# ayankele/dune-transformercvn

Measured on AMD Instinct MI355X. Metric: events/sec (fwd+bwd) at batch=32, 8 prongs/event; fraction of MFMA roofline, higher is better.
Workload: dtype bf16; 1 GPU; TransformerCVN DenseNet [3,6,12,6,3] g32, fwd+loss+bwd, batch 32/GPU, 8 prongs/event, 3x400x280 maps, 6-layer encoder, dropout 0.1; global_batch=32, parallelism=dp1, precision=bf16

## Files before the change

### dune-transformercvn_amd/csrc/densenet.hip

```cpp
#include <string>
#include <vector>
#include <cstring>

#include "tcvn_rows.h"
#include <cstdlib>
#include "densenet_plan.h"

using namespace tcvn;

namespace {
constexpr float kEps = 1e-5f, kMom = 0.1f;
}

int DenseNetPlan::add_slot(const std::string& name, long numel, int kind) {
    slots.push_back({name, numel, kind});
    return (int)slots.size() - 1;
}
BnSlots DenseNetPlan::add_bn(const std::string& p, int c) {
    BnSlots s;
    s.w = add_slot(p + ".weight", c, TCVN_SLOT_PARAM);
    s.b = add_slot(p + ".bias", c, TCVN_SLOT_PARAM);
    s.rm = add_slot(p + ".running_mean", c, TCVN_SLOT_BUFFER);
    s.rv = add_slot(p + ".running_var", c, TCVN_SLOT_BUFFER);
    s.nbt = add_slot(p + ".num_batches_tracked", 1, TCVN_SLOT_COUNTER);
// ... 441 lines not shown
    if (stem_path.act_skip &&
        (rc = stem_mark(coords, nnz, n, cfg.H, cfg.W, Hc, Wc, reinterpret_cast<uint32_t*>(s.ws + L.sact), data[s_b0], s.ws + L.zeros + 512, s.st))) return rc;
    a.part = s.train ? s.part : nullptr; a.nblk = conv_fwd_nblk(a);
    if ((rc = conv_fwd(a, s.st))) return rc;
    if ((rc = link(s, n0, a.nblk, cfg.init_ch, 0, cfg.init_ch, bstat0, M0))) return rc;
    const Tab t = tab(s.ws, L, n0);
    Pool0Args p{mode, s.ws + L.c0, n, Hc, Wc, cfg.init_ch, t.sc, t.sh, data[s_a0], s.ws + L.D[0], b0.ld, b0.H, b0.W,
                s.train ? s.part : nullptr, pool0_grid(n, b0.H, b0.W)};
    if ((rc = pool0_fwd(p, s.st))) return rc;
    fr.nblk = p.nblk;
    return 0;
}

LayerPath DenseNetPlan::layer_path(const Step& s, int bi, int l, const ConvFwdArgs& c3, Fwd1x1Args& f1) const {
    const Layout& L = s.L;
    const BlockGeom& bg = blocks[bi];
    const LayerSlots& ls = bg.layers[l];
    const long M = (long)s.n * bg.H * bg.W;
    const bool bf16 = cfg.mode == MODE_BF16, fast1 = L.XA[bi][l] >= 0;
    const Conv3x3Fwd k3 = bf16 ? conv3x3_fwd_kernel(c3) : CONV3X3_FWD_NONE;
    LayerPath p;
    p.fuse_ya = !s.train && fast1 && k3 != CONV3X3_FWD_NONE;
    p.act_fused = bf16 && !p.fuse_ya && conv3x3_act_fusable(c3);
    static const bool no_fuse1 = TCVN_KNOB_SET("TCVN_NO_FWD1_FUSE") || TCVN_KNOB_SET("TCVN_NO_BWD1_FUSE");
    if ((s.train || p.fuse_ya) && fast1 && !no_fuse1 && cfg.bn_size * cfg.growth == 128 && bf16) {
        const WkEntry& e = wk_find(ls.w1, 0, 1);
        const Tab t1 = tab(s.ws, L, ls.n1);
        f1 = Fwd1x1Args{};
        f1.Xin = s.ws + L.D[bi]; f1.ldx = bg.ld; f1.cin = ls.cin; f1.sc = t1.sc; f1.sh = t1.sh; f1.sl = data[ls.a1]; f1.M = M;
        f1.Wfrag = s.ws + L.wk + e.off; f1.Kp = e.Kp; f1.bias = data[ls.b1]; f1.Out = s.ws + L.Y[bi][l]; f1.zeros = s.ws + L.zeros;
        f1.part = s.train ? s.part : nullptr; f1.nblk = fwd1x1_fused_nblk(f1);
        if (!s.train) {
            f1.osc = c3.sc; f1.osh = c3.sh; f1.osl = c3.sl; f1.Out = s.ws + L.YA[bi][l];
        }
        Bwd1x1Args b1;
        p.raw1x1 = fwd1x1_fused_ok(f1) && (!s.train || bwd1x1_fill(bi, l, M, s.ws, L, b1));
    }
    const bool pair = k3 == CONV3X3_FWD_PAIR;
    p.lf2 = p.raw1x1 && s.lf_on && p.act_fused && pair;
    p.out_isum = s.lf_on && pair && cfg.growth <= 32;
    p.keep_stored = s.train && !L.KM[bi].empty() && pair;
    return p;
}

int DenseNetPlan::fwd_layer(const Step& s, int bi, int l, FreshStats& fr) {
    const Layout& L = s.L;
    const BlockGeom& bg = blocks[bi];
    const LayerSlots& ls = bg.layers[l];
    const long M = (long)s.n * bg.H * bg.W;
    const int mid = cfg.bn_size * cfg.growth, g = cfg.growth;
    char* D = s.ws + L.D[bi];
    char* Y = s.ws + L.Y[bi][l];
    double* bstatD = reinterpret_cast<double*>(s.ws + L.bstatD[bi]);
    double* bstatY = reinterpret_cast<double*>(s.ws + L.bstatY[bi][l]);
    long long* isumD = s.lf_on ? reinterpret_cast<long long*>(s.ws + L.isumD[bi]) : nullptr;
    long long* isumY = s.lf_on ? reinterpret_cast<long long*>(s.ws + L.isumY[bi][l]) : nullptr;
    int rc;
    ConvFwdArgs a = conv3_args(s, bi, l);
    Fwd1x1Args f1;
    const LayerPath p = path[bi][l] = layer_path(s, bi, l, a, f1);
    if (p.raw1x1) {
        if (s.lf_on && fr.isum) f1.lf = lf_link(s, ls.n1, isumD + 2 * fr.c0, 2L * bg.ld, fr.c0, fr.n, bstatD, M);
        else if ((rc = link_fresh(s, ls.n1, bi, fr))) return rc;
        f1.isum_out = isumY; f1.isum_stride = 2L * mid;
        if ((rc = fwd1x1_fused(f1, s.st))) return rc;
        if (!p.lf2 && (rc = link(s, ls.n2, f1.nblk, mid, 0, mid, bstatY, M, isumY, 2L * mid))) return rc;
    } else {
        if ((rc = link_fresh(s, ls.n1, bi, fr))) return rc;
        int nblk;
        if (L.XA[bi][l] >= 0) {
            const int cin8 = (int)round_up(ls.cin, 8);
            const Tab t1 = tab(s.ws, L, ls.n1);
            ActArgs act{D, bg.ld, M, ls.cin, t1.sc, t1.sh, data[ls.a1], s.ws + L.XA[bi][l], cin8};
            if ((rc = act_bf16(act, s.st))) return rc;
            const WkEntry& e = wk_find(ls.w1, 0, 1);
            GemmNtArgs ga{};
            ga.epi = EPI_FWD; ga.A = s.ws + L.XA[bi][l]; ga.lda = cin8; ga.K = cin8; ga.M = M; ga.N = mid;
            ga.Wfrag = s.ws + L.wk + e.off; ga.Kp = e.Kp; ga.zeros = s.ws + L.zeros; ga.bias = data[ls.b1];
            ga.Out = Y; ga.ldo = mid; ga.n_off = 0; ga.part = s.train ? s.part : nullptr; ga.nblk = gemm_nt_nblk(ga);
            if (p.fuse_ya) {
                ga.osc = a.sc; ga.osh = a.sh; ga.osl = a.sl; ga.Out = s.ws + L.YA[bi][l];
            }
            if ((rc = gemm_nt_bf16(ga, "k_gemm_nt_bf16<fwd1x1>", s.st))) return rc;
            nblk = ga.nblk;
        } else {
            ConvFwdArgs c1 = conv1_args(s, bi, l);
            c1.part = s.train ? s.part : nullptr; c1.nblk = conv_fwd_nblk(c1);
            if ((rc = conv_fwd(c1, s.st))) return rc;
            nblk = c1.nblk;
        }
        if ((rc = link(s, ls.n2, nblk, mid, 0, mid, bstatY, M))) return rc;
    }
    if (p.act_fused) a.act_fused = 1;
    else if (cfg.mode == MODE_BF16) {
        if (!p.fuse_ya) {
            ActArgs act{Y, mid, M, mid, a.sc, a.sh, a.sl, s.ws + L.YA[bi][l], mid};
            if ((rc = act_bf16(act, s.st))) return rc;
        }
        a.Aact = s.ws + L.YA[bi][l];
    }
    a.part = s.train ? s.part : nullptr;
    a.drop_p = s.train ? cfg.dropout : 0.f; a.seed = s.seed; a.stream_id = (uint32_t)(bi * 64 + l + 1);
    a.nblk = conv_fwd_nblk(a);
    if (p.lf2) {
        if (!a.act_fused) { fprintf(stderr, "tcvn: link-free norm2 without the in-LDS activation\n"); return -17; }
        a.lf = lf_link(s, ls.n2, isumY, 2L * mid, 0, mid, bstatY, M);
    }
    if (p.out_isum) { a.isum_out = isumD + 2 * ls.cin; a.isum_stride = 2L * bg.ld; }
    if (s.train && !L.KM[bi].empty()) a.keep_out = reinterpret_cast<uint32_t*>(s.ws + L.KM[bi][l]);
    if ((rc = conv_fwd(a, s.st))) return rc;
    fr = FreshStats{ls.cin, g, a.nblk, g, p.out_isum};
    return 0;
}

int DenseNetPlan::fwd_transition(const Step& s, int bi, FreshStats& fr) {
    const Layout& L = s.L;
    const BlockGeom& bg = blocks[bi];
    char* D = s.ws + L.D[bi];
    int rc;
    if ((rc = link_fresh(s, bg.has_trans ? bg.tn : nf, bi, fr))) return rc;
    if (!bg.has_trans) {
        const Tab t = tab(s.ws, L, nf);
        HeadPoolArgs a{cfg.mode, D, bg.ld, s.n, bg.H * bg.W, Cf, t.sc, t.sh, data[s_af], reinterpret_cast<float*>(s.ws + L.F)};
        return head_pool_fwd(a, s.st);
    }
    const BlockGeom& nb = blocks[bi + 1];
    fr = FreshStats{0, nb.C0, 0, bg.Ctot / 2, false};
    if (L.XP[bi] >= 0) {
        const Tab t = tab(s.ws, L, bg.tn);
        ActPoolArgs ap{D, bg.ld, s.n, bg.H, bg.W, bg.Ctot, t.sc, t.sh, data[bg.ta], s.ws + L.XP[bi], bg.ldp};
        if ((rc = cfg.mode == MODE_BF16 ? act_pool_bf16(ap, s.st) : act_pool_f32(ap, s.st))) return rc;
    }
    if (L.XP[bi] >= 0 && cfg.mode == MODE_BF16) {
        const WkEntry& ef = wk_find(bg.tw, 0, 1);
        GemmNtArgs ga{};
        ga.epi = EPI_FWD; ga.A = s.ws + L.XP[bi]; ga.lda = bg.ldp; ga.K = bg.ldp; ga.M = (long)s.n * nb.H * nb.W; ga.N = bg.Ctot / 2;
        ga.Wfrag = s.ws + L.wk + ef.off; ga.Kp = ef.Kp; ga.zeros = s.ws + L.zeros; ga.bias = data[bg.tb];
        ga.Out = s.ws + L.D[bi + 1]; ga.ldo = nb.ld; ga.n_off = 0; ga.part = s.train ? s.part : nullptr; ga.nblk = gemm_nt_nblk(ga);
        if ((rc = gemm_nt_bf16(ga, "k_gemm_nt_bf16<fwdtrans>", s.st))) return rc;
        fr.nblk = ga.nblk;
        return 0;
    }
    ConvFwdArgs a = trans_args(s, bi);
    a.part = s.train ? s.part : nullptr; a.nblk = conv_fwd_nblk(a);
    if ((rc = conv_fwd(a, s.st))) return rc;
    fr.nblk = a.nblk;
    return 0;
}

int DenseNetPlan::fwd_output(const Step& s, float* out, long out_ld) const {
    float* F = reinterpret_cast<float*>(s.ws + s.L.F);
    float* Z = reinterpret_cast<float*>(s.ws + s.L.Z);
    int rc;
    if ((rc = linear_fwd(F, Cf, data[s_wl], nullptr, Z, cfg.out_dim, s.n, cfg.out_dim, Cf, s.st))) return rc;
    float* hs = reinterpret_cast<float*>(s.ws + s.L.head_stat);
    RowsBnArgs r{};
    r.X = Z; r.ldx = cfg.out_dim; r.R = s.n; r.C = cfg.out_dim; r.gamma = data[nl.w]; r.beta = data[nl.b]; r.slope = data[s_al];
    r.running_mean = data[nl.rm]; r.running_var = data[nl.rv]; r.Y = out; r.ldy = out_ld;
    r.save_mean = hs; r.save_rstd = hs + cfg.out_dim; r.train = s.train; r.eps = kEps; r.momentum = kMom;
    r.drop_p = s.train ? cfg.dropout : 0.f; r.seed = s.seed; r.stream_id = 0x4000u;
    return rows_bn_fwd(r, s.st);
}

int DenseNetPlan::tap(int n, const char* name, long* off, int* tn, int* th, int* tw, int* tc, int* tld, int* tes) const {
    Layout L;
    layout(n, false, L);
    std::string s(name);
    *tn = n; *tes = esz;
    if ((s == "img" || s == "conv0") && stem_path.sparse && n == last_n) return -1;
    if (s == "img") { *off = L.img; *th = cfg.H; *tw = cfg.W; *tc = cfg.in_ch; *tld = cfg.in_ch; return 0; }
    if (s == "conv0") { *off = L.c0; *th = Hc; *tw = Wc; *tc = cfg.init_ch; *tld = cfg.init_ch; return 0; }
    if (s == "condense") { *off = L.F; *th = 1; *tw = 1; *tc = Cf; *tld = Cf; *tes = 4; return 0; }
    if (s == "raw:wk") { *tn = *th = *tw = 1; *off = L.wk; *tc = *tld = (int)(wk_bytes() / esz); return 0; }
    if (s == "raw:tabs") { *tn = *th = *tw = 1; *off = L.tabs; *tc = *tld = (int)tab_floats(); *tes = 4; return 0; }
    if (s.rfind("raw:ystat", 0) == 0) {
        int b = 0, l = 0;
        if (sscanf(s.c_str(), "raw:ystat%d.%d", &b, &l) != 2) return -1;
        b -= 1;
        if (b < 0 || b >= (int)blocks.size() || l < 0 || l >= blocks[b].L) return -1;
        *tn = *th = *tw = 1; *off = L.bstatY[b][l]; *tc = *tld = 2 * cfg.bn_size * cfg.growth; *tes = 8; return 0;
    }
    if (s.rfind("raw:bstat", 0) == 0) {
        const int b = atoi(s.c_str() + 9) - 1;
        if (b < 0 || b >= (int)blocks.size()) return -1;
        *tn = *th = *tw = 1; *off = L.bstatD[b]; *tc = *tld = blocks[b].ld * 2; *tes = 8; return 0;
    }
    if (s.rfind("dense", 0) == 0) {
        const int b = atoi(s.c_str() + 5) - 1;
        if (b < 0 || b >= (int)blocks.size()) return -1;
        *off = L.D[b]; *th = blocks[b].H; *tw = blocks[b].W; *tc = blocks[b].Ctot; *tld = blocks[b].ld;
        return 0;
    }
    if (s.rfind("bottleneck", 0) == 0) {
        int b = 0, l = 0;
        if (sscanf(s.c_str(), "bottleneck%d.%d", &b, &l) != 2) return -1;
        b -= 1;
        if (b < 0 || b >= (int)blocks.size() || l < 0 || l >= blocks[b].L) return -1;
        for (const auto& pb : path)
            for (const LayerPath& p : pb) if (n == last_n && p.fuse_ya) return -1;
        *off = L.Y[b][l]; *th = blocks[b].H; *tw = blocks[b].W; *tc = cfg.bn_size * cfg.growth; *tld = *tc;
        return 0;
    }
    if (s.rfind("xa", 0) == 0 || s.rfind("ya", 0) == 0) {
        int b = 0, l = 0;
        if (sscanf(s.c_str() + 2, "%d.%d", &b, &l) != 2) return -1;
        b -= 1;
        if (b < 0 || b >= (int)blocks.size() || l < 0 || l >= blocks[b].L) return -1;
        const bool xa = s[0] == 'x';
        if ((xa && (L.XA[b].empty() || L.XA[b][l] < 0)) || (!xa && L.YA[b].empty())) return -1;
        if (n == last_n && (xa ? path[b][l].raw1x1 : path[b][l].act_fused)) return -1;
        *off = xa ? L.XA[b][l] : L.YA[b][l]; *th = blocks[b].H; *tw = blocks[b].W;
        *tc = xa ? blocks[b].layers[l].cin : cfg.bn_size * cfg.growth; *tld = xa ? (int)round_up(*tc, 8) : *tc;
        return 0;
    }
    return -1;
}

struct tcvn_densenet { DenseNetPlan plan; explicit tcvn_densenet(const tcvn_densenet_cfg& c) : plan(c) {} };

extern "C" {

int tcvn_version(void) { return 1; }
void tcvn_backward_overlap(int on) { tcvn::set_backward_overlap(on); }

int tcvn_densenet_create(const tcvn_densenet_cfg* cfg, tcvn_densenet** out) {
    if (!cfg || !out || cfg->n_blocks < 1 || cfg->n_blocks > 8) return -1;
    if (cfg->mode != TCVN_MODE_F32 && cfg->mode != TCVN_MODE_BF16) return -1;
    *out = new tcvn_densenet(*cfg);
    return 0;
}
void tcvn_densenet_destroy(tcvn_densenet* p) { delete p; }
int tcvn_densenet_num_slots(const tcvn_densenet* p) { return (int)p->plan.slots.size(); }
int tcvn_densenet_slot(const tcvn_densenet* p, int i, char* name, int cap, int64_t* numel, int* kind) {
    if (i < 0 || i >= (int)p->plan.slots.size()) return -1;
    const auto& s = p->plan.slots[i];
    if (name && cap > 0) { strncpy(name, s.name.c_str(), cap - 1); name[cap - 1] = 0; }
    if (numel) *numel = s.numel;
    if (kind) *kind = s.kind;
    return 0;
}
int tcvn_densenet_bind(tcvn_densenet* p, void* const* data, void* const* grad) { return p->plan.bind(data, grad); }
int64_t tcvn_densenet_workspace_bytes(const tcvn_densenet* p, int n_img, int with_backward) {
    Layout L;
    p->plan.layout(n_img, with_backward != 0, L);
    return L.total;
}
int tcvn_densenet_forward(tcvn_densenet* p, int n_img, const int32_t* coords, const float* values, int64_t nnz, int log_pixels,
                          float noise_std, float* out, int64_t out_ld, void* ws, int64_t ws_bytes, int train, uint64_t seed,
                          void* stream) {
    return p->plan.forward(n_img, coords, values, nnz, log_pixels, noise_std, out, out_ld, reinterpret_cast<char*>(ws), ws_bytes,
                           train, seed, reinterpret_cast<hipStream_t>(stream));
}
int tcvn_densenet_backward(tcvn_densenet* p, int n_img, const float* d_out, int64_t d_out_ld, void* ws, int64_t ws_bytes,
                           void* stream) {
    return p->plan.backward(n_img, d_out, d_out_ld, reinterpret_cast<char*>(ws), ws_bytes, reinterpret_cast<hipStream_t>(stream));
}
int tcvn_densenet_num_blocks(const tcvn_densenet* p) { return (int)p->plan.blocks.size(); }
int tcvn_densenet_backward_blocks(tcvn_densenet* p, int n_img, const float* d_out, int64_t d_out_ld, void* ws, int64_t ws_bytes,
                                  int block_hi, int block_lo, void* stream) {
    return p->plan.backward(n_img, d_out, d_out_ld, reinterpret_cast<char*>(ws), ws_bytes, reinterpret_cast<hipStream_t>(stream), block_hi,
                            block_lo);
}
int tcvn_densenet_tap(const tcvn_densenet* p, int n_img, const char* name, int64_t* byte_off, int* n, int* h, int* w, int* c,
                      int* ld, int* elem_bytes) {
    long off = 0;
    int rc = p->plan.tap(n_img, name, &off, n, h, w, c, ld, elem_bytes);
    *byte_off = off;
    return rc;
}

}
```

### dune-transformercvn_amd/csrc/densenet_bwd.hip

```cpp
#include <cstring>
#include <vector>

#include <cstdlib>
#include "densenet_plan.h"
#include "tcvn_rows.h"

using namespace tcvn;

static int g_backward_overlap = 0;
bool tcvn::backward_overlap_enabled() { return g_backward_overlap != 0; }
void tcvn::set_backward_overlap(int on) { g_backward_overlap = on; }

namespace {
constexpr float kEps = 1e-5f;
constexpr long kSlabBytes = 48L << 20;
constexpr long kSlab1GemmBytes = 64L << 20;
constexpr long kSlab1Bytes = 68L << 20;
constexpr long kSlabGemmBytes = 44L << 20;
struct Bump {
    long off;
    long take(long bytes) { long o = off; off += round_up(bytes, 256); return o; }
};
}

// ... 3 lines not shown
    L.G.clear(); L.pqD.clear();
    long bpart = (long)std::max(pool0_bwd_grid(n, Hc, Wc), pool0_bwd_vec_grid(n, Hc, Wc)) * cfg.init_ch * 24;
    bpart = std::max(bpart, 1024L * cfg.init_ch * 24);
    bpart = std::max(bpart, (long)head_pool_bwd_grid(n) * Cf * 24);
    for (const auto& bg : blocks) {
        const long M = (long)n * bg.H * bg.W;
        L.G.push_back(b.take(M * bg.ld * esz));
        bpart = std::max(bpart, 512L * std::max(mid, bg.Ctot) * 24);
    }
    for (const auto& bg : blocks) L.pqD.push_back(b.take((long)bg.ld * 8));
    long gw = 0;
    for (const auto& e : wk_list())
        if (!e.transpose && !e.frag) gw += round_up((long)e.N * e.Kp * 4, 256);
    L.gwk = b.take(gw);
    L.zero_end = b.off;
    L.du = b.take(maxY * esz);
    L.ey = b.take(maxY * esz);
    L.ey2 = b.take(maxY * esz);
    L.slab = b.take(kSlabBytes);
    L.slab1 = cfg.mode == MODE_BF16 ? b.take(kSlab1Bytes) : -1;
    L.pqY = b.take((long)mid * 8);
    L.du0 = b.take((long)n * Hc * Wc * cfg.init_ch * esz);
    L.pq0 = b.take((long)cfg.init_ch * 8);
    L.bpart = b.take(bpart);
    L.dF = b.take((long)n * Cf * 4);
    L.dZ = b.take((long)n * cfg.out_dim * 4);
    L.EY3.clear();
    for (const auto& bg : blocks) {
        std::vector<long> eys;
        if (cfg.mode == MODE_BF16 && cfg.growth == 32)
            for (int l = 0; l < bg.L; ++l) eys.push_back(b.take((long)n * bg.H * bg.W * 32 * esz));
        L.EY3.push_back(eys);
    }
    L.total = b.off;
}

bool DenseNetPlan::bwd1x1_fill(int bi, int l, long M, char* ws, const Layout& L, Bwd1x1Args& fa) const {
    static const bool no_fuse1 = TCVN_KNOB_SET("TCVN_NO_BWD1_FUSE");
    const BlockGeom& bg = blocks[bi];
    const LayerSlots& ls = bg.layers[l];
    const int mid = cfg.bn_size * cfg.growth;
    if (no_fuse1 || L.XA[bi][l] < 0 || mid != 128 || L.slab1 < 0 || cfg.mode != MODE_BF16) return false;
    const Tab t1 = tab(ws, L, ls.n1);
    const WkEntry& etf = wk_find(ls.w1, 1, 1);
    fa = Bwd1x1Args{};
    fa.DU = ws + L.du; fa.Y = ws + L.Y[bi][l]; fa.PY = reinterpret_cast<float*>(ws + L.pqY); fa.QY = fa.PY + mid; fa.M = M;
    fa.Xin = ws + L.D[bi]; fa.ldx = bg.ld; fa.cin = ls.cin;
    fa.sc = t1.sc; fa.sh = t1.sh; fa.sl = data[ls.a1]; fa.Gout = ws + L.G[bi]; fa.ldg = bg.ld;
    fa.Wfrag = ws + L.wk + etf.off; fa.Kp = etf.Kp; fa.zeros = ws + L.zeros; fa.part = reinterpret_cast<double*>(ws + L.bpart);
    fa.slab = reinterpret_cast<float*>(ws + L.slab1); fa.slab_bytes = kSlab1GemmBytes; fa.ldc = wk_find(ls.w1, 0).Kp;
    fa.tail = reinterpret_cast<float*>(ws + L.slab1 + kSlab1GemmBytes);
    fa.nblk = bwd1x1_fused_nblk(fa);
    return bwd1x1_fused_ok(fa);
}

float* DenseNetPlan::gw_of(const Step& s, int slot) const {
    long o = 0;
    for (const WkEntry& e : wk_cache) {
        if (e.transpose || e.frag) continue;
        if (e.slot == slot) return reinterpret_cast<float*>(s.ws + s.L.gwk + o);
        o += round_up((long)e.N * e.Kp * 4, 256);
    }
    return nullptr;
}

int DenseNetPlan::bwd_link(const Step& s, const BnSlots& bn, int nblk, const double* bstat, long count, float* P, float* Q, int acc, int a_slot) const {
    BnBwdLinkArgs a{s.part, nblk, bn.C, bstat, count, kEps, data[bn.w], grad[bn.w], grad[bn.b], grad[a_slot], P, Q, acc};
    return bn_bwd_link(a, s.st);
}

int DenseNetPlan::drain(Step& s) const {
    if (s.side_on && s.side_busy) {
        TCVN_CHECK(hipEventRecord(ev_drain, side_st));
        TCVN_CHECK(hipStreamWaitEvent(s.st, ev_drain, 0));
        s.side_busy = false;
    }
    s.seq = 0;
    return 0;
}

int DenseNetPlan::backward(int n, const float* d_out, long d_out_ld, char* ws, long ws_bytes, hipStream_t st, int bi_hi, int bi_lo) {
    if (!bound) return -11;
    if (bi_hi < 0) bi_hi = (int)blocks.size() - 1;
    if (bi_lo < 0 || bi_lo > bi_hi || bi_hi >= (int)blocks.size()) return -1;
    const bool first_part = bi_hi == (int)blocks.size() - 1, last_part = bi_lo == 0;
    if (n <= 0) return 0;
    if (n != last_n) { fprintf(stderr, "tcvn: densenet backward without matching forward\n"); return -13; }
    for (size_t i = 0; i < slots.size(); ++i)
        if (slots[i].kind == TCVN_SLOT_PARAM && grad[i] == nullptr) { fprintf(stderr, "tcvn: grad of %s unbound\n", slots[i].name.c_str()); return -14; }
    Layout L;
    layout(n, true, L);
    if (ws_bytes < L.total) return -12;
    int rc;
    const bool side_on = fast3x3 && backward_overlap_enabled();
    if (side_on && (rc = ensure_side())) return rc;
    Step s{ws, L, st, n, true, last_seed, reinterpret_cast<double*>(ws + L.bpart), false, side_on, 0, false};

    if (undesc_ws != ws || undesc_total != L.total) {
        std::vector<UnpackDesc> ud;
        unpack_first.assign(blocks.size() + 1, 0);
        long o = 0;
        for (const WkEntry& e : wk_cache) {
            if (e.transpose || e.frag) continue;
            for (size_t bi = 0; bi < blocks.size(); ++bi) {
                if (!blocks[bi].layers.empty() && e.slot == blocks[bi].layers[0].w1) unpack_first[bi] = (int)ud.size();
            }
            UnpackDesc d{reinterpret_cast<const float*>(ws + L.gwk + o), grad[e.slot], e.N, e.Cin, e.taps, e.Kp,
                         (fast3x3 && e.taps == 9) ? 1 : 0};
            ud.push_back(d);
            o += round_up((long)e.N * e.Kp * 4, 256);
        }
        n_unpack = (int)ud.size();
        unpack_first[blocks.size()] = n_unpack;
        if (!d_undesc) TCVN_CHECK(hipMalloc(&d_undesc, ud.size() * sizeof(UnpackDesc)));
        h_undesc.assign(reinterpret_cast<char*>(ud.data()), reinterpret_cast<char*>(ud.data()) + ud.size() * sizeof(UnpackDesc));
        TCVN_CHECK(hipMemcpyAsync(d_undesc, h_undesc.data(), h_undesc.size(), hipMemcpyHostToDevice, st));
        undesc_ws = ws; undesc_total = L.total;
    }

    if (first_part) {
        TCVN_CHECK(hipMemsetAsync(ws + L.pqD[0], 0, (size_t)(L.zero_end - L.pqD[0]), st));
        for (size_t bi = 0; bi + 1 < blocks.size(); ++bi) {
            const long bytes = (long)n * blocks[bi].H * blocks[bi].W * blocks[bi].ld * esz;
            if (L.XP[bi] >= 0 && cfg.mode == MODE_BF16) {
                if ((rc = zero_pool_remainder(ws + L.G[bi], blocks[bi].ld, n, blocks[bi].H, blocks[bi].W, blocks[bi + 1].H, blocks[bi + 1].W, st))) return rc;
            } else TCVN_CHECK(hipMemsetAsync(ws + L.G[bi], 0, (size_t)bytes, st));
        }
        if ((rc = bwd_output(s, d_out, d_out_ld))) return rc;
    }
    for (int bi = bi_hi; bi >= bi_lo; --bi) {
        if ((rc = bwd_transition(s, bi))) return rc;
        for (int l = blocks[bi].L - 1; l >= 0; --l)
            if ((rc = bwd_layer(s, bi, l))) return rc;
    }
    if ((rc = drain(s))) return rc;
    if (last_part && (rc = bwd_stem(s))) return rc;
    const int u0 = last_part ? 0 : unpack_first[bi_lo], u1 = unpack_first[bi_hi + 1];
    return unpack_wgrads(reinterpret_cast<const UnpackDesc*>(d_undesc) + u0, u1 - u0, st);
}

int DenseNetPlan::bwd_output(const Step& s, const float* d_out, long d_out_ld) const {
    const Layout& L = s.L;
    float* F = reinterpret_cast<float*>(s.ws + L.F);
    float* Z = reinterpret_cast<float*>(s.ws + L.Z);
    float* dF = reinterpret_cast<float*>(s.ws + L.dF);
    float* dZ = reinterpret_cast<float*>(s.ws + L.dZ);
    float* hs = reinterpret_cast<float*>(s.ws + L.head_stat);
    int rc;
    RowsBnBwdArgs r{};
    r.X = Z; r.ldx = cfg.out_dim; r.dY = d_out; r.lddy = d_out_ld; r.R = s.n; r.C = cfg.out_dim;
    r.gamma = data[nl.w]; r.beta = data[nl.b]; r.slope = data[s_al]; r.save_mean = hs; r.save_rstd = hs + cfg.out_dim;
    r.dX = dZ; r.lddx = cfg.out_dim; r.dgamma = grad[nl.w]; r.dbeta = grad[nl.b]; r.dslope = grad[s_al];
    r.drop_p = cfg.dropout; r.seed = s.seed; r.stream_id = 0x4000u;
    if ((rc = rows_bn_bwd(r, s.st))) return rc;
    if ((rc = linear_bwd_dw(dZ, cfg.out_dim, F, Cf, grad[s_wl], nullptr, s.n, cfg.out_dim, Cf, s.st))) return rc;
    return linear_bwd_dx(dZ, cfg.out_dim, data[s_wl], dF, Cf, s.n, cfg.out_dim, Cf, 0, s.st);
}

int DenseNetPlan::bwd_transition(Step& s, int bi) const {
    const Layout& L = s.L;
    const BlockGeom& bg = blocks[bi];
    const int mode = cfg.mode;
    const long M = (long)s.n * bg.H * bg.W;
    char* D = s.ws + L.D[bi];
    char* G = s.ws + L.G[bi];
    float* P = reinterpret_cast<float*>(s.ws + L.pqD[bi]);
    float* Q = P + bg.ld;
    const double* bstatD = reinterpret_cast<const double*>(s.ws + L.bstatD[bi]);
    int rc;
    if (!bg.has_trans) {
        const Tab t = tab(s.ws, L, nf);
        HeadPoolBwdArgs a{mode, D, bg.ld, s.n, bg.H * bg.W, Cf, t.sc, t.sh, data[s_af], reinterpret_cast<float*>(s.ws + L.dF), G, bg.ld, s.part,
                          head_pool_bwd_grid(s.n)};
        if ((rc = head_pool_bwd(a, s.st))) return rc;
        return bwd_link(s, nf, a.nblk, bstatD, M, P, Q, 1, s_af);
    }
    const BlockGeom& nb = blocks[bi + 1];
    const long Mn = (long)s.n * nb.H * nb.W;
    const int Nt = bg.Ctot / 2;
    float* Pn = reinterpret_cast<float*>(s.ws + L.pqD[bi + 1]);
    float* Qn = Pn + nb.ld;
    const EffSrc e{s.ws + L.G[bi + 1], nb.ld, s.ws + L.D[bi + 1], nb.ld, 0, Nt, Pn, Qn, 0.f, 0, 0};
    const Tab t = tab(s.ws, L, bg.tn);
    const WkEntry& ef = wk_find(bg.tw, 0);
    if ((rc = drain(s))) return rc;
    if (L.XP[bi] >= 0 && mode == MODE_BF16) {
        const int Nt8 = (int)round_up(Nt, 8);
        SlabJob bias_job{};
        EffMatArgs em{e, Mn, s.ws + L.ey, Nt8, grad[bg.tb], reinterpret_cast<float*>(s.ws + L.slab + kSlabGemmBytes), &bias_job};
        if ((rc = eff_materialize_bf16(em, s.st))) return rc;
        GemmTnArgs gt{s.ws + L.ey, Nt8, Nt8, s.ws + L.XP[bi], bg.ldp, bg.ldp, Mn, gw_of(s, bg.tw), ef.Kp, s.ws + L.zeros,
                      reinterpret_cast<float*>(s.ws + L.slab), kSlabGemmBytes, Nt, bias_job};
        if ((rc = gemm_tn_bf16(gt, "k_gemm_tn_bf16<transition>", s.st))) return rc;
        const WkEntry& etf = wk_find(bg.tw, 1, 1);
        GemmNtArgs ga{};
        ga.epi = EPI_DGRAD_POOL; ga.A = s.ws + L.ey; ga.lda = Nt8; ga.K = Nt8; ga.M = Mn; ga.N = bg.Ctot;
        ga.Wfrag = s.ws + L.wk + etf.off; ga.Kp = etf.Kp; ga.zeros = s.ws + L.zeros;
        ga.Xin = D; ga.ldxin = bg.ld; ga.sc = t.sc; ga.sh = t.sh; ga.sl = data[bg.ta];
        ga.Gout = G; ga.ldgo = bg.ld; ga.g_write = 1; ga.H = nb.H; ga.W = nb.W; ga.Hin = bg.H; ga.Win = bg.W;
        ga.part = s.part; ga.nblk = gemm_nt_nblk(ga);
        if ((rc = gemm_nt_bf16(ga, "k_gemm_nt_bf16<dgradtrans>", s.st))) return rc;
        return bwd_link(s, bg.tn, ga.nblk, bstatD, M, P, Q, 1, bg.ta);
    }
    ConvWgradArgs w{};
    w.mode = mode; w.e = e; w.dWk = gw_of(s, bg.tw); w.dbias = grad[bg.tb];
    w.fa = trans_args(s, bi);
    if (L.XP[bi] >= 0) { w.slab = reinterpret_cast<float*>(s.ws + L.slab); w.slab_bytes = kSlabBytes; }
    if ((rc = conv_wgrad(w, s.st))) return rc;
    const WkEntry& et = wk_find(bg.tw, 1);
    ConvDgradArgs d{};
    d.mode = mode; d.dmode = DG_1X1_POOL; d.e = e; d.M = (int)Mn; d.N = bg.Ctot; d.Kp = et.Kp;
    d.H = nb.H; d.W = nb.W; d.Hin = bg.H; d.Win = bg.W; d.Wt = s.ws + L.wk + et.off;
    d.Xin = D; d.ldxin = bg.ld; d.sc = t.sc; d.sh = t.sh; d.sl = data[bg.ta];
    d.Gout = G; d.ldgo = bg.ld; d.accumulate = 1; d.part = s.part; d.nblk = conv_dgrad_nblk(d);
    if ((rc = conv_dgrad(d, s.st))) return rc;
    return bwd_link(s, bg.tn, d.nblk, bstatD, M, P, Q, 1, bg.ta);
}

int DenseNetPlan::bwd_layer(Step& s, int bi, int l) const {
    const Layout& L = s.L;
    const BlockGeom& bg = blocks[bi];
    const LayerSlots& ls = bg.layers[l];
    const LayerPath& p = path[bi][l];
    const int mode = cfg.mode, g = cfg.growth, mid = cfg.bn_size * cfg.growth;
    const long M = (long)s.n * bg.H * bg.W;
    hipStream_t st = s.st;
    char* D = s.ws + L.D[bi];
    char* G = s.ws + L.G[bi];
    float* P = reinterpret_cast<float*>(s.ws + L.pqD[bi]);
    float* Q = P + bg.ld;
    const double* bstatD = reinterpret_cast<const double*>(s.ws + L.bstatD[bi]);
    char* Y = s.ws + L.Y[bi][l];
    char* DU = s.ws + L.du;
    float* PY = reinterpret_cast<float*>(s.ws + L.pqY);
    float* QY = PY + mid;
    int rc;
    ConvWgradArgs w3{};
    w3.fa = conv3_args(s, bi, l);
    EffSrc e2{G, bg.ld, D, bg.ld, ls.cin, g, P + ls.cin, Q + ls.cin, cfg.dropout, s.seed, (uint32_t)(bi * 64 + l + 1)};
    if (p.keep_stored) e2.keep = reinterpret_cast<const uint32_t*>(s.ws + L.KM[bi][l]);
    bool ey_valid = false;
    {
        const WkEntry& et = wk_find(ls.w2, 1);
        ConvDgradArgs d{};
        d.mode = mode; d.dmode = DG_3X3; d.e = e2; d.M = (int)M; d.N = mid; d.Kp = et.Kp; d.H = bg.H; d.W = bg.W;
        d.Wt = s.ws + L.wk + et.off; d.Xin = Y; d.ldxin = mid; d.sc = w3.fa.sc; d.sh = w3.fa.sh; d.sl = w3.fa.sl;
        d.Gout = DU; d.ldgo = mid; d.accumulate = 0; d.part = s.part;
        d.Wfrag = wk_frag(s.ws, L, ls.w2, 1); d.zeros = s.ws + L.zeros;
        ey_valid = fast3x3 && !L.EY3[bi].empty() && conv3x3_dgrad_kernel(d) == CONV3X3_DGRAD_CONSEC;
        if (ey_valid) d.ey_out = s.ws + L.EY3[bi][l];
        d.nblk = conv_dgrad_nblk(d);
        if ((rc = conv_dgrad(d, st))) return rc;
        if ((rc = bwd_link(s, ls.n2, d.nblk, reinterpret_cast<const double*>(s.ws + L.bstatY[bi][l]), M, PY, QY, 0, ls.a2))) return rc;
    }
    Bwd1x1Args fa{};
    const bool fuse1 = bwd1x1_fill(bi, l, M, s.ws, L, fa);
    SlabJob w3jobs[2] = {};
    bool w3_deferred = false;
    {
        w3.mode = mode; w3.e = e2; w3.dWk = gw_of(s, ls.w2); w3.dbias = grad[ls.b2];
        if (ey_valid) w3.e.ey = s.ws + L.EY3[bi][l];
        if (fast3x3) {
            w3.nfast = 1; w3.fa.act_fused = p.act_fused ? 1 : 0;
            if (!p.act_fused) w3.fa.Aact = s.ws + L.YA[bi][l];
            w3.slab = reinterpret_cast<float*>(s.ws + L.slab); w3.slab_bytes = kSlabBytes;
        }
        const bool par = s.side_on && L.XA[bi][l] >= 0;
        if (par) {
            TCVN_CHECK(hipEventRecord(ev_fork_a, st));
            TCVN_CHECK(hipStreamWaitEvent(side_st, ev_fork_a, 0));
            s.side_busy = true;
        }
        if (!par && fuse1 && fast3x3 && conv3x3_wgrad_tile_ok(w3)) { w3.deferred = w3jobs; w3_deferred = true; }
        if ((rc = conv_wgrad(w3, par ? side_st : st))) return rc;
    }
    if (fuse1) {
        if ((rc = bwd1x1_fused_launch(fa, st))) return rc;
        const BnSlots& s1 = ls.n1;
        BnBwdLinkArgs la{s.part, fa.nblk, s1.C, bstatD, M, kEps, data[s1.w], grad[s1.w], grad[s1.b], grad[ls.a1], P, Q, 1};
        return bwd1x1_fused_reduce(fa, gw_of(s, ls.w1), grad[ls.b1], w3_deferred ? w3jobs : nullptr, st, &la);
    }
    if (p.raw1x1) {
        fprintf(stderr, "tcvn: the forward skipped the activated 1x1 input of block %d layer %d but the fused 1x1 backward cannot run\n", bi, l);
        return -15;
    }
    const Tab t1 = tab(s.ws, L, ls.n1);
    const EffSrc e1{DU, mid, Y, mid, 0, mid, PY, QY, 0.f, 0, 0};
    if (L.XA[bi][l] < 0) {
        ConvWgradArgs w{};
        w.mode = mode; w.e = e1; w.dWk = gw_of(s, ls.w1); w.dbias = grad[ls.b1];
        w.fa = conv1_args(s, bi, l);
        if (mode == MODE_F32) { w.slab = reinterpret_cast<float*>(s.ws + L.slab); w.slab_bytes = kSlabBytes; }
        if ((rc = conv_wgrad(w, st))) return rc;
        const WkEntry& et = wk_find(ls.w1, 1);
        ConvDgradArgs d{};
        d.mode = mode; d.dmode = DG_1X1; d.e = e1; d.M = (int)M; d.N = ls.cin; d.Kp = et.Kp; d.H = bg.H; d.W = bg.W;
        d.Wt = s.ws + L.wk + et.off; d.Xin = D; d.ldxin = bg.ld; d.sc = t1.sc; d.sh = t1.sh; d.sl = data[ls.a1];
        d.Gout = G; d.ldgo = bg.ld; d.accumulate = 1; d.part = s.part; d.nblk = conv_dgrad_nblk(d);
        if ((rc = conv_dgrad(d, st))) return rc;
        return bwd_link(s, ls.n1, d.nblk, bstatD, M, P, Q, 1, ls.a1);
    }
    const bool odd = s.side_on && (s.seq & 1);
    char* EY = s.ws + (odd ? L.ey2 : L.ey);
    float* tail = reinterpret_cast<float*>(s.ws + L.slab + kSlabGemmBytes + (odd ? (kSlabBytes - kSlabGemmBytes) / 2 : 0));
    if (s.side_on && s.seq >= 2) TCVN_CHECK(hipStreamWaitEvent(st, ev_done[s.seq & 1], 0));
    SlabJob bias_job{};
    EffMatArgs em{e1, M, EY, mid, grad[ls.b1], tail, &bias_job};
    if ((rc = eff_materialize_bf16(em, st))) return rc;
// ... 66 lines not shown
```

### dune-transformercvn_amd/csrc/encoder.hip

```cpp
#include "tcvn_encoder.h"

namespace tcvn {

namespace {

constexpr float kInvSqrt2 = 0.70710678118654752440f;

__global__ void k_gather_tokens(const float* C, const int* tok_row, float* X, int B, int S, int D) {
    const int t = blockIdx.x;
    const int s = t / B, b = t - s * B;
    const int r = tok_row[b * S + s];
    for (int d = threadIdx.x; d < D; d += blockDim.x) X[(long)t * D + d] = r >= 0 ? C[(long)r * D + d] : 0.f;
}
__global__ void k_scatter_tokens_bwd(const float* dX, const int* tok_row, float* dC, int B, int S, int D) {
    const int t = blockIdx.x;
    const int s = t / B, b = t - s * B;
    const int r = tok_row[b * S + s];
    if (r < 0) return;
    for (int d = threadIdx.x; d < D; d += blockDim.x) dC[(long)r * D + d] = dX[(long)t * D + d];
}
__global__ void k_mask_rows(const float* X, const int* tok_row, float* Y, int B, int S, int D) {
    const int t = blockIdx.x;
    const int s = t / B, b = t - s * B;
    const bool keep = tok_row[b * S + s] >= 0;
// ... 25 lines not shown
    }
    float sum = 0.f;
    for (int j = 0; j < a.S; ++j) { sc[j] = valid[j] ? expf(sc[j] - mx) : 0.f; sum += sc[j]; }
    const float inv = 1.0f / sum;
    float* P = a.probs + (((long)b * a.H + h) * a.S + s) * a.S;
    float ctx[MAXHD];
    for (int e = 0; e < a.hd; ++e) ctx[e] = 0.f;
    for (int j = 0; j < a.S; ++j) {
        float p = sc[j] * inv;
        P[j] = p;
        if (a.drop_p > 0.f) p *= drop_scale(a.drop_p, a.seed, a.stream_id, (((uint64_t)b * a.H + h) * a.S + s) * a.S + j);
        for (int e = 0; e < a.hd; ++e) ctx[e] = fmaf(p, v[j][e], ctx[e]);
    }
    float* o = a.ctx + ((long)s * a.B + b) * D + h * a.hd;
    for (int e = 0; e < a.hd; ++e) o[e] = ctx[e];
}

__global__ __launch_bounds__(64) void k_attn_bwd(const AttnBwdArgs a) {
    __shared__ float q[MAXS][MAXHD + 1], k[MAXS][MAXHD + 1], v[MAXS][MAXHD + 1], dc[MAXS][MAXHD + 1];
    __shared__ float dS[MAXS][MAXS + 1], Pd[MAXS][MAXS + 1];
    const int b = blockIdx.x, h = blockIdx.y, s = threadIdx.x;
    const int D = a.H * a.hd;
    for (int i = threadIdx.x; i < a.S * a.hd; i += 64) {
        const int ss = i / a.hd, d = i - ss * a.hd;
        const float* row = a.qkv + ((long)ss * a.B + b) * 3 * D + h * a.hd + d;
        q[ss][d] = row[0]; k[ss][d] = row[D]; v[ss][d] = row[2 * D];
        dc[ss][d] = a.dctx[((long)ss * a.B + b) * D + h * a.hd + d];
    }
    __syncthreads();
    const float scale = rsqrtf((float)a.hd);
    if (s < a.S) {
        const float* P = a.probs + (((long)b * a.H + h) * a.S + s) * a.S;
        float dot = 0.f;
        float dp[MAXS];
        for (int j = 0; j < a.S; ++j) {
            float g = 0.f;
            for (int e = 0; e < a.hd; ++e) g = fmaf(dc[s][e], v[j][e], g);
            float m = 1.f;
            if (a.drop_p > 0.f) m = drop_scale(a.drop_p, a.seed, a.stream_id, (((uint64_t)b * a.H + h) * a.S + s) * a.S + j);
            Pd[s][j] = P[j] * m;
            dp[j] = g * m;
            dot = fmaf(dp[j], P[j], dot);
        }
        for (int j = 0; j < a.S; ++j) dS[s][j] = P[j] * (dp[j] - dot);
    }
    __syncthreads();
    if (s >= a.S) return;
    float* o = a.dqkv + ((long)s * a.B + b) * 3 * D + h * a.hd;
    for (int e = 0; e < a.hd; ++e) {
        float dq = 0.f, dk = 0.f, dv = 0.f;
        for (int j = 0; j < a.S; ++j) {
            dq = fmaf(dS[s][j], k[j][e], dq);
            dk = fmaf(dS[j][s], q[j][e], dk);
            dv = fmaf(Pd[j][s], dc[j][e], dv);
        }
        o[e] = dq * scale; o[D + e] = dk * scale; o[2 * D + e] = dv;
    }
}

__global__ __launch_bounds__(256) void k_add_ln_fwd(const AddLnArgs a) {
    const int wave = threadIdx.x >> 6, lane = threadIdx.x & 63;
    const int t = blockIdx.x * 4 + wave;
    if (t >= a.T) return;
    float v[8];
    const int per = (a.D + 63) / 64;
    float s = 0.f;
    for (int i = 0; i < per; ++i) {
        const int d = lane + 64 * i;
        float x = 0.f;
        if (d < a.D) {
            float r = a.R[(long)t * a.D + d];
            if (a.drop_p > 0.f) r *= drop_scale(a.drop_p, a.seed, a.stream_id, (uint64_t)t * a.D + d);
            x = a.X[(long)t * a.D + d] + r;
        }
        v[i] = x; s += x;
    }
    const float mean = wave_sum(s) / a.D;
    float q = 0.f;
    for (int i = 0; i < per; ++i) { const int d = lane + 64 * i; if (d < a.D) { const float c = v[i] - mean; q += c * c; } }
    const float rstd = rsqrtf(wave_sum(q) / a.D + a.eps);
    for (int i = 0; i < per; ++i) {
        const int d = lane + 64 * i;
        if (d < a.D) {
            const float xh = (v[i] - mean) * rstd;
            a.XH[(long)t * a.D + d] = xh;
            a.Y[(long)t * a.D + d] = xh * a.gamma[d] + a.beta[d];
        }
    }
    if (lane == 0) a.rstd[t] = rstd;
}
__global__ __launch_bounds__(256) void k_add_ln_bwd(const AddLnBwdArgs a) {
    const int wave = threadIdx.x >> 6, lane = threadIdx.x & 63;
    const int t = blockIdx.x * 4 + wave;
    if (t >= a.T) return;
    const int per = (a.D + 63) / 64;
    float g[8], xh[8];
    float s1 = 0.f, s2 = 0.f;
    for (int i = 0; i < per; ++i) {
        const int d = lane + 64 * i;
        g[i] = 0.f; xh[i] = 0.f;
        if (d < a.D) {
            xh[i] = a.XH[(long)t * a.D + d];
            g[i] = a.dY[(long)t * a.D + d] * a.gamma[d];
            s1 += g[i]; s2 += g[i] * xh[i];
        }
    }
    s1 = wave_sum(s1) / a.D; s2 = wave_sum(s2) / a.D;
    const float rstd = a.rstd[t];
    for (int i = 0; i < per; ++i) {
        const int d = lane + 64 * i;
        if (d < a.D) {
            const float ds = rstd * (g[i] - s1 - xh[i] * s2);
            a.dX[(long)t * a.D + d] = ds;
            float dr = ds;
            if (a.drop_p > 0.f) dr *= drop_scale(a.drop_p, a.seed, a.stream_id, (uint64_t)t * a.D + d);
            a.dR[(long)t * a.D + d] = dr;
        }
    }
}
__global__ __launch_bounds__(256) void k_ln_param_grads(const float* dY, const float* XH, int T, int D, float* dgamma, float* dbeta) {
    __shared__ double sa[16][17], sb[16][17];
    const int cl = threadIdx.x & 15, rl = threadIdx.x >> 4, d = blockIdx.x * 16 + cl;
    double a = 0, b = 0;
    if (d < D)
        for (int t = rl; t < T; t += 16) { const float g = dY[(long)t * D + d]; a += (double)g * XH[(long)t * D + d]; b += g; }
    sa[rl][cl] = a; sb[rl][cl] = b;
    __syncthreads();
    if (threadIdx.x < 16 && d < D) {
        double x = 0, y = 0;
#pragma unroll
        for (int i = 0; i < 16; ++i) { x += sa[i][cl]; y += sb[i][cl]; }
        dgamma[d] += (float)x; dbeta[d] += (float)y;
    }
}

__global__ void k_act_fwd(const float* X, float* Y, long n, int gelu, float drop_p, uint64_t seed, uint32_t stream_id) {
    const long i = (long)blockIdx.x * blockDim.x + threadIdx.x;
    if (i >= n) return;
    const float x = X[i];
    float y = gelu ? 0.5f * x * (1.f + erff(x * kInvSqrt2)) : fmaxf(x, 0.f);
    if (drop_p > 0.f) y *= drop_scale(drop_p, seed, stream_id, (uint64_t)i);
    Y[i] = y;
}
__global__ void k_act_bwd(const float* X, const float* dY, float* dX, long n, int gelu, float drop_p, uint64_t seed, uint32_t stream_id) {
    const long i = (long)blockIdx.x * blockDim.x + threadIdx.x;
    if (i >= n) return;
    const float x = X[i];
    float g = dY[i];
    if (drop_p > 0.f) g *= drop_scale(drop_p, seed, stream_id, (uint64_t)i);
    const float d = gelu ? 0.5f * (1.f + erff(x * kInvSqrt2)) + x * 0.3989422804014327f * expf(-0.5f * x * x) : (x > 0.f ? 1.f : 0.f);
    dX[i] = g * d;
}

template <typename TT>
__global__ __launch_bounds__(256) void k_focal(const float* logits, const TT* targets, int rows, int C, float gamma, float weight,
                                               float* dlogits, float* out) {
    __shared__ double red[256][2];
    __shared__ int cnt_s[256];
    __shared__ int total;
    int cnt = 0;
    for (int r = threadIdx.x; r < rows; r += 256) cnt += targets[r] >= 0;
    cnt_s[threadIdx.x] = cnt;
    __syncthreads();
    if (threadIdx.x == 0) { int c = 0; for (int i = 0; i < 256; ++i) c += cnt_s[i]; total = c; }
    __syncthreads();
    const float invn = total > 0 ? 1.0f / total : 0.f;
    double loss = 0, acc = 0;
    for (int r = threadIdx.x; r < rows; r += 256) {
        const int t = (int)targets[r];
        float* dl = dlogits + (long)r * C;
        if (t < 0) { for (int c = 0; c < C; ++c) dl[c] = 0.f; continue; }
        const float* z = logits + (long)r * C;
        float mx = z[0]; int am = 0;
        for (int c = 1; c < C; ++c) if (z[c] > mx) { mx = z[c]; am = c; }
        float sum = 0.f;
        for (int c = 0; c < C; ++c) sum += expf(z[c] - mx);
        const float logpt = z[t] - mx - logf(sum);
        const float pt = expf(logpt);
        float dldlogpt;
        if (gamma == 0.f) { loss += -logpt; dldlogpt = -1.f; }
        else {
            const float om = fmaxf(1.f - pt, 0.f);
            const float w = powf(om, gamma);
            loss += -logpt * w;
            dldlogpt = -w + (om > 0.f ? logpt * gamma * powf(om, gamma - 1.f) * pt : 0.f);
        }
        acc += am == t;
        for (int c = 0; c < C; ++c) {
            const float p = expf(z[c] - mx) / sum;
            dl[c] = weight * invn * dldlogpt * ((c == t ? 1.f : 0.f) - p);
        }
    }
    red[threadIdx.x][0] = loss; red[threadIdx.x][1] = acc;
    __syncthreads();
    if (threadIdx.x == 0) {
        double l = 0, c = 0;
        for (int i = 0; i < 256; ++i) { l += red[i][0]; c += red[i][1]; }
        out[0] = (float)(l * invn); out[1] = (float)(c * invn);
    }
}

__global__ void k_permute_rows(const float* in, float* out, int B, int P, int C, int to_bm) {
    const int i = blockIdx.x * blockDim.x + threadIdx.x;
    if (i >= B * P * C) return;
    const int c = i % C, r = i / C;
    if (to_bm) { const int b = r / P, p = r - b * P; out[i] = in[((long)p * B + b) * C + c]; }
    else { const int p = r / B, b = r - p * B; out[i] = in[((long)b * P + p) * C + c]; }
}
__global__ void k_add_drop(const float* x, const float* r, float* y, long n, float drop_p, uint64_t seed, uint32_t stream_id) {
    const long i = (long)blockIdx.x * blockDim.x + threadIdx.x;
    if (i >= n) return;
    float v = r[i];
    if (drop_p > 0.f) v *= drop_scale(drop_p, seed, stream_id, (uint64_t)i);
    y[i] = x[i] + v;
}
__global__ void k_mul_drop(const float* dy, float* dr, long n, float drop_p, uint64_t seed, uint32_t stream_id) {
    const long i = (long)blockIdx.x * blockDim.x + threadIdx.x;
    if (i >= n) return;
    float v = dy[i];
    if (drop_p > 0.f) v *= drop_scale(drop_p, seed, stream_id, (uint64_t)i);
    dr[i] = v;
}
__global__ void k_add_inplace(float* dst, const float* src, long n) {
    const long i = (long)blockIdx.x * blockDim.x + threadIdx.x;
    if (i < n) dst[i] += src[i];
}

}

int permute_rows(const float* in, float* out, int B, int P, int C, int to_bm, hipStream_t st) {
    if (B * P * C <= 0) return 0;
    hipLaunchKernelGGL(k_permute_rows, dim3(cdiv((long)B * P * C, 256)), dim3(256), 0, st, in, out, B, P, C, to_bm);
    TCVN_LAUNCH_CHECK(); return 0;
}
int add_drop(const float* x, const float* r, float* y, long n, float drop_p, uint64_t seed, uint32_t sid, hipStream_t st) {
    hipLaunchKernelGGL(k_add_drop, dim3(cdiv(n, 256)), dim3(256), 0, st, x, r, y, n, drop_p, seed, sid);
    TCVN_LAUNCH_CHECK(); return 0;
}
int mul_drop(const float* dy, float* dr, long n, float drop_p, uint64_t seed, uint32_t sid, hipStream_t st) {
    hipLaunchKernelGGL(k_mul_drop, dim3(cdiv(n, 256)), dim3(256), 0, st, dy, dr, n, drop_p, seed, sid);
    TCVN_LAUNCH_CHECK(); return 0;
}
int add_inplace(float* dst, const float* src, long n, hipStream_t st) {
    hipLaunchKernelGGL(k_add_inplace, dim3(cdiv(n, 256)), dim3(256), 0, st, dst, src, n);
    TCVN_LAUNCH_CHECK(); return 0;
}
int gather_tokens(const float* C, const int* tok_row, float* X, int B, int S, int D, hipStream_t st) {
    hipLaunchKernelGGL(k_gather_tokens, dim3(B * S), dim3(128), 0, st, C, tok_row, X, B, S, D);
    TCVN_LAUNCH_CHECK(); return 0;
}
int scatter_tokens_bwd(const float* dX, const int* tok_row, float* dC, int B, int S, int D, hipStream_t st) {
    hipLaunchKernelGGL(k_scatter_tokens_bwd, dim3(B * S), dim3(128), 0, st, dX, tok_row, dC, B, S, D);
    TCVN_LAUNCH_CHECK(); return 0;
}
int mask_rows(const float* X, const int* tok_row, float* Y, int B, int S, int D, hipStream_t st) {
    hipLaunchKernelGGL(k_mask_rows, dim3(B * S), dim3(128), 0, st, X, tok_row, Y, B, S, D);
    TCVN_LAUNCH_CHECK(); return 0;
}
int attn_fwd(const AttnArgs& a, hipStream_t st) {
    if (a.S > MAXS || a.hd > MAXHD) { fprintf(stderr, "tcvn: attention supports S<=%d, head_dim<=%d\n", MAXS, MAXHD); return -2; }
    hipLaunchKernelGGL(k_attn_fwd, dim3(a.B, a.H), dim3(64), 0, st, a);
    TCVN_LAUNCH_CHECK(); return 0;
}
int attn_bwd(const AttnBwdArgs& a, hipStream_t st) {
    if (a.S > MAXS || a.hd > MAXHD) return -2;
    hipLaunchKernelGGL(k_attn_bwd, dim3(a.B, a.H), dim3(64), 0, st, a);
    TCVN_LAUNCH_CHECK(); return 0;
}
int add_ln_fwd(const AddLnArgs& a, hipStream_t st) {
    if (a.D > 512) return -2;
    hipLaunchKernelGGL(k_add_ln_fwd, dim3(cdiv(a.T, 4)), dim3(256), 0, st, a);
    TCVN_LAUNCH_CHECK(); return 0;
}
int add_ln_bwd(const AddLnBwdArgs& a, hipStream_t st) {
    if (a.D > 512) return -2;
    hipLaunchKernelGGL(k_add_ln_bwd, dim3(cdiv(a.T, 4)), dim3(256), 0, st, a);
    TCVN_LAUNCH_CHECK();
    hipLaunchKernelGGL(k_ln_param_grads, dim3(cdiv(a.D, 16)), dim3(256), 0, st, a.dY, a.XH, a.T, a.D, a.dgamma, a.dbeta);
    TCVN_LAUNCH_CHECK(); return 0;
}
int act_fwd(const float* X, float* Y, long n, int gelu, float drop_p, uint64_t seed, uint32_t sid, hipStream_t st) {
    hipLaunchKernelGGL(k_act_fwd, dim3(cdiv(n, 256)), dim3(256), 0, st, X, Y, n, gelu, drop_p, seed, sid);
    TCVN_LAUNCH_CHECK(); return 0;
}
int act_bwd(const float* X, const float* dY, float* dX, long n, int gelu, float drop_p, uint64_t seed, uint32_t sid, hipStream_t st) {
    hipLaunchKernelGGL(k_act_bwd, dim3(cdiv(n, 256)), dim3(256), 0, st, X, dY, dX, n, gelu, drop_p, seed, sid);
    TCVN_LAUNCH_CHECK(); return 0;
}
int focal_i64(const float* logits, const int64_t* targets, int rows, int C, float gamma, float weight, float* dlogits, float* out,
              hipStream_t st) {
    hipLaunchKernelGGL(k_focal<int64_t>, dim3(1), dim3(256), 0, st, logits, targets, rows, C, gamma, weight, dlogits, out);
    TCVN_LAUNCH_CHECK(); return 0;
}
int focal_i8(const float* logits, const int8_t* targets, int rows, int C, float gamma, float weight, float* dlogits, float* out,
             hipStream_t st) {
    hipLaunchKernelGGL(k_focal<int8_t>, dim3(1), dim3(256), 0, st, logits, targets, rows, C, gamma, weight, dlogits, out);
    TCVN_LAUNCH_CHECK(); return 0;
}

}
```

### dune-transformercvn_amd/csrc/head.hip

```cpp
#include <string>
#include <vector>
#include <cstring>

#include "../../include/tcvn_hip.h"
#include "head_plan.h"
#include "tcvn_rows.h"
#include "tcvn_encoder.h"
#include "tcvn_explain.h"
#include "tcvn_occlude.h"
#include "tcvn_shapley.h"

using namespace tcvn;

namespace {
constexpr float kEps = 1e-5f, kMom = 0.1f;
constexpr uint32_t kSidCombined = 0x5000u;
constexpr uint32_t sid_enc(int l, int k) { return 0x6000u + l * 8 + k; }
constexpr uint32_t sid_dec(int i) { return 0x7000u + (uint32_t)i; }

__global__ void k_combine_loss(const float* oe, const float* op, float ew, float* losses, float* accs) {
    losses[0] = ew * oe[0] + (1.f - ew) * op[0];
    losses[1] = oe[0]; losses[2] = op[0];
    accs[0] = oe[1]; accs[1] = op[1];
}
struct Bump {
    long off = 0;
    long take(long bytes) { long o = off; off += round_up(bytes, 256); return o; }
};
}

int HeadPlan::add_slot(const std::string& name, long numel, int kind) {
    slots.push_back({name, numel, kind});
    return (int)slots.size() - 1;
}
HBn HeadPlan::add_bn(const std::string& p, int c) {
    HBn s;
    s.w = add_slot(p + ".weight", c, TCVN_SLOT_PARAM);
    s.b = add_slot(p + ".bias", c, TCVN_SLOT_PARAM);
    s.rm = add_slot(p + ".running_mean", c, TCVN_SLOT_BUFFER);
    s.rv = add_slot(p + ".running_var", c, TCVN_SLOT_BUFFER);
    add_slot(p + ".num_batches_tracked", 1, TCVN_SLOT_COUNTER);
    return s;
}

HeadPlan::HeadPlan(const tcvn_head_cfg& c) : cfg(c) {
    const int D = cfg.hidden_dim;
    const std::string ce = "prong_embedding.combined_embedding";
    const bool bn = !cfg.no_linear_bn, prelu_act = !cfg.linear_relu;
    comb.in = cfg.in_dim; comb.out = D; comb.sid = kSidCombined; comb.drop = true;
    comb.w = add_slot(ce + ".linear.weight", (long)D * cfg.in_dim, TCVN_SLOT_PARAM);
    if (!bn) comb.b = add_slot(ce + ".linear.bias", D, TCVN_SLOT_PARAM);
    if (bn) comb.n = add_bn(ce + ".norm", D);
    if (prelu_act) comb.a = add_slot(ce + ".activation.weight", D, TCVN_SLOT_PARAM);
    for (int l = 0; l < cfg.n_layers; ++l) {
        const std::string p = "encoder.encoder.layers." + std::to_string(l);
        HLayer L;
        L.win = add_slot(p + ".self_attn.in_proj_weight", 3L * D * D, TCVN_SLOT_PARAM);
        L.bin = add_slot(p + ".self_attn.in_proj_bias", 3 * D, TCVN_SLOT_PARAM);
        L.wo = add_slot(p + ".self_attn.out_proj.weight", (long)D * D, TCVN_SLOT_PARAM);
        L.bo = add_slot(p + ".self_attn.out_proj.bias", D, TCVN_SLOT_PARAM);
        L.w1 = add_slot(p + ".linear1.weight", (long)D * D, TCVN_SLOT_PARAM);
        L.b1 = add_slot(p + ".linear1.bias", D, TCVN_SLOT_PARAM);
        L.w2 = add_slot(p + ".linear2.weight", (long)D * D, TCVN_SLOT_PARAM);
        L.b2 = add_slot(p + ".linear2.bias", D, TCVN_SLOT_PARAM);
        L.g1 = add_slot(p + ".norm1.weight", D, TCVN_SLOT_PARAM);
        L.be1 = add_slot(p + ".norm1.bias", D, TCVN_SLOT_PARAM);
        L.g2 = add_slot(p + ".norm2.weight", D, TCVN_SLOT_PARAM);
        L.be2 = add_slot(p + ".norm2.bias", D, TCVN_SLOT_PARAM);
        layers.push_back(L);
    }
    ew = add_slot("event_decoder.hidden_layer.weight", (long)cfg.event_classes * D, TCVN_SLOT_PARAM);
    eb = add_slot("event_decoder.hidden_layer.bias", cfg.event_classes, TCVN_SLOT_PARAM);
    int idx = 0, in = D;
    for (int i = 0; i < cfg.n_dec; ++i) {
        const std::string p = "prong_decoder.hidden_layers.";
        HDec d;
        d.in = in; d.out = cfg.dec_dims[i]; d.sid = sid_dec(i); d.drop = cfg.dropout_modules != 0;
        d.w = add_slot(p + std::to_string(idx) + ".weight", (long)d.out * d.in, TCVN_SLOT_PARAM);
        d.b = add_slot(p + std::to_string(idx) + ".bias", d.out, TCVN_SLOT_PARAM);
        if (bn) d.n = add_bn(p + std::to_string(idx + 1), d.out);
        if (prelu_act) d.a = add_slot(p + std::to_string(idx + 1 + (bn ? 1 : 0)) + ".weight", d.out, TCVN_SLOT_PARAM);
        idx += 2 + (bn ? 1 : 0) + (cfg.dropout_modules ? 1 : 0);
        in = d.out;
        dec.push_back(d);
    }
    dec_width = in;
    ow = add_slot("prong_decoder.output_layer.weight", (long)cfg.prong_classes * cfg.dec_out_in, TCVN_SLOT_PARAM);
    ob = add_slot("prong_decoder.output_layer.bias", cfg.prong_classes, TCVN_SLOT_PARAM);
    data.assign(slots.size(), nullptr);
    grad.assign(slots.size(), nullptr);
}

int HeadPlan::bind(void* const* d, void* const* g) {
    for (size_t i = 0; i < slots.size(); ++i) {
        data[i] = reinterpret_cast<float*>(d[i]);
        grad[i] = g ? reinterpret_cast<float*>(g[i]) : nullptr;
        if (slots[i].kind != TCVN_SLOT_COUNTER && data[i] == nullptr) return -10;
    }
    bound = true;
    return 0;
}

void HeadPlan::layout(int B, int P, int nP, HLayout& L) const {
    Bump b;
    const int D = cfg.hidden_dim, S = 1 + P, T = S * B, R = B + nP, TP = P * B, H = cfg.heads;
    const long td = (long)T * D * 4;
    L.Zc = b.take((long)R * D * 4); L.C = b.take((long)R * D * 4); L.cstat = b.take(2L * D * 4);
    L.X.clear(); L.lay.clear();
    for (int l = 0; l <= cfg.n_layers; ++l) L.X.push_back(b.take(td));
    for (int l = 0; l < cfg.n_layers; ++l) {
        HLayBuf q;
        q.qkv = b.take(3 * td); q.probs = b.take((long)B * H * S * S * 4); q.ctx = b.take(td); q.ao = b.take(td);
        q.xh1 = b.take(td); q.rstd1 = b.take((long)T * 4); q.x1 = b.take(td); q.hpre = b.take(td); q.hact = b.take(td);
        q.f = b.take(td); q.xh2 = b.take(td); q.rstd2 = b.take((long)T * 4);
        q.h1 = cfg.norm_first ? b.take(td) : -1; q.h2 = cfg.norm_first ? b.take(td) : -1;
        L.lay.push_back(q);
    }
    L.HID = b.take(td);
    L.Zd.clear(); L.Ad.clear(); L.dstat.clear();
    for (const auto& d : dec) {
        L.Zd.push_back(b.take((long)TP * d.out * 4)); L.Ad.push_back(b.take((long)TP * d.out * 4));
        L.dstat.push_back(b.take(2L * d.out * 4));
    }
    L.LG = b.take((long)TP * cfg.prong_classes * 4);
    L.dEv = b.take((long)B * cfg.event_classes * 4); L.dPr = b.take((long)B * P * cfg.prong_classes * 4);
    L.lossbuf = b.take(64);
    L.dLG = b.take((long)TP * cfg.prong_classes * 4);
    L.t0 = b.take(3 * td); L.t1 = b.take(3 * td); L.t2 = b.take(td); L.t3 = b.take(td); L.dHID = b.take(td);
    L.dC = b.take((long)R * D * 4); L.dZc = b.take((long)R * D * 4);
    for (int l = 0; l < cfg.n_layers; ++l) {
        HLayBuf& q = L.lay[l];
        q.g_dqkv = b.take(3 * td); q.g_dao = b.take(td); q.g_dhp = b.take(td); q.g_df = b.take(td);
    }
    L.lnp = b.take((long)B * cfg.n_layers * 4 * D * 4);
    L.total = b.off;
}

int HeadPlan::step(int B, int P, int nP, void* ws, long ws_bytes, int train, uint64_t seed, hipStream_t st, HeadStep& s) const {
    if (!bound) return -11;
    if (cfg.dec_out_in != dec_width) { fprintf(stderr, "tcvn: prong decoder width mismatch (reference would fail too)\n"); return -21; }
    if (B <= 0 || P < 0 || nP < 0 || 1 + P > 64) return -1;
    s.B = B; s.P = P; s.nP = nP; s.S = 1 + P; s.T = s.S * B; s.R = B + nP; s.TP = P * B;
    s.ws = reinterpret_cast<char*>(ws); s.train = train; s.seed = seed; s.dp = train ? cfg.dropout : 0.f; s.st = st;
    layout(B, P, nP, s.L);
    return ws_bytes < s.L.total ? -12 : 0;
}

EncPath HeadPlan::enc_path(int S) const {
    if (fused_encoder && encoder_fused_ok(S, cfg.hidden_dim, cfg.heads, cfg.n_layers, cfg.norm_first)) return EncPath::FUSED;
    return cfg.norm_first ? EncPath::PRE_NORM : EncPath::POST_NORM;
}

EncLayerW HeadPlan::enc_w(int l) const {
    const HLayer& W = layers[l];
    return EncLayerW{data[W.win], data[W.bin], data[W.wo], data[W.bo], data[W.w1], data[W.b1], data[W.w2], data[W.b2],
                     data[W.g1], data[W.be1], data[W.g2], data[W.be2]};
}
EncLayerBuf HeadPlan::enc_buf(const HeadStep& s, int l) const {
    const HLayBuf& q = s.L.lay[l];
    return EncLayerBuf{s.F(q.qkv), s.F(q.probs), s.F(q.ctx), s.F(q.xh1), s.F(q.rstd1), s.F(q.x1), s.F(q.hpre), s.F(q.hact), s.F(q.xh2),
                       s.F(q.rstd2), s.F(s.L.X[l + 1])};
}
RowsBnArgs HeadPlan::block_fwd(const HDec& d, const HeadStep& s, long X, long Y, long stat, int rows) const {
    RowsBnArgs r{};
    r.X = s.F(X); r.ldx = d.out; r.R = rows; r.C = d.out; r.slope = d.a >= 0 ? data[d.a] : nullptr; r.no_norm = cfg.no_linear_bn;
    if (!r.no_norm) { r.gamma = data[d.n.w]; r.beta = data[d.n.b]; r.running_mean = data[d.n.rm]; r.running_var = data[d.n.rv]; }
    r.Y = s.F(Y); r.ldy = d.out;
    r.save_mean = s.F(stat); r.save_rstd = s.F(stat) + d.out; r.train = s.train; r.eps = kEps; r.momentum = kMom;
    r.drop_p = d.drop ? s.dp : 0.f; r.seed = s.seed; r.stream_id = d.sid;
    return r;
}
RowsBnBwdArgs HeadPlan::block_bwd(const HDec& d, const HeadStep& s, long X, long dY, long stat, long dX, int rows) const {
    RowsBnBwdArgs r{};
    r.X = s.F(X); r.ldx = d.out; r.dY = s.F(dY); r.lddy = d.out; r.R = rows; r.C = d.out;
    r.no_norm = cfg.no_linear_bn; r.slope = d.a >= 0 ? data[d.a] : nullptr; r.dslope = d.a >= 0 ? grad[d.a] : nullptr;
    if (!r.no_norm) { r.gamma = data[d.n.w]; r.beta = data[d.n.b]; r.dgamma = grad[d.n.w]; r.dbeta = grad[d.n.b]; }
    r.save_mean = s.F(stat); r.save_rstd = s.F(stat) + d.out;
    r.dX = s.F(dX); r.lddx = d.out;
    r.drop_p = d.drop ? s.dp : 0.f; r.seed = s.seed; r.stream_id = d.sid;
    return r;
}
DecIn HeadPlan::dec_in(const HeadStep& s, int i) const {
    const long hid_prongs = (long)s.B * cfg.hidden_dim;
    if (i == 0) return DecIn{s.F(s.L.HID) + hid_prongs, s.F(s.L.dHID) + hid_prongs, cfg.hidden_dim};
    return DecIn{s.F(s.L.Ad[i - 1]), s.F(s.L.t0), dec[i - 1].out};
}

int HeadPlan::embed(const HeadStep& s, const float* rows, const int32_t* tok_row) const {
    const HLayout& L = s.L;
    const int D = cfg.hidden_dim;
    if (int rc = linear_fwd(rows, cfg.in_dim, data[comb.w], comb.b >= 0 ? data[comb.b] : nullptr, s.F(L.Zc), D, s.R, D, cfg.in_dim, s.st)) return rc;
    if (int rc = rows_bn_fwd(block_fwd(comb, s, L.Zc, L.C, L.cstat, s.R), s.st)) return rc;
    return gather_tokens(s.F(L.C), tok_row, s.F(L.X[0]), s.B, s.S, D, s.st);
}

int HeadPlan::encode(const HeadStep& s, const int32_t* tok_row) const {
    switch (enc_path(s.S)) {
    case EncPath::FUSED: {
        EncFusedArgs a{};
        a.X0 = s.F(s.L.X[0]); a.tok_row = tok_row; a.HID = s.F(s.L.HID); a.B = s.B; a.S = s.S; a.H = cfg.heads; a.L = cfg.n_layers;
        a.gelu = cfg.gelu; a.save = 1; a.eps = kEps; a.drop_p = s.dp; a.seed = s.seed;
        for (int l = 0; l < cfg.n_layers; ++l) { a.w[l] = enc_w(l); a.buf[l] = enc_buf(s, l); }
        return encoder_fused_fwd(a, s.st);
    }
    case EncPath::POST_NORM: return encode_post(s, tok_row);
    case EncPath::PRE_NORM: return encode_pre(s, tok_row);
    }
    return -1;
}
int HeadPlan::encode_post(const HeadStep& s, const int32_t* tok_row) const {
    const HLayout& L = s.L;
    const int D = cfg.hidden_dim, T = s.T, H = cfg.heads, hd = D / H;
    for (int l = 0; l < cfg.n_layers; ++l) {
        const HLayer& W = layers[l];
        const HLayBuf& q = L.lay[l];
        if (int rc = linear_fwd(s.F(L.X[l]), D, data[W.win], data[W.bin], s.F(q.qkv), 3 * D, T, 3 * D, D, s.st)) return rc;
        AttnArgs a{s.F(q.qkv), tok_row, s.F(q.probs), s.F(q.ctx), s.B, s.S, H, hd, s.dp, s.seed, sid_enc(l, 0)};
        if (int rc = attn_fwd(a, s.st)) return rc;
        if (int rc = linear_fwd(s.F(q.ctx), D, data[W.wo], data[W.bo], s.F(q.ao), D, T, D, D, s.st)) return rc;
        AddLnArgs n1{s.F(L.X[l]), s.F(q.ao), data[W.g1], data[W.be1], s.F(q.x1), s.F(q.xh1), s.F(q.rstd1), T, D, kEps, s.dp, s.seed, sid_enc(l, 1)};
        if (int rc = add_ln_fwd(n1, s.st)) return rc;
        if (int rc = linear_fwd(s.F(q.x1), D, data[W.w1], data[W.b1], s.F(q.hpre), D, T, D, D, s.st)) return rc;
        if (int rc = act_fwd(s.F(q.hpre), s.F(q.hact), (long)T * D, cfg.gelu, s.dp, s.seed, sid_enc(l, 2), s.st)) return rc;
        if (int rc = linear_fwd(s.F(q.hact), D, data[W.w2], data[W.b2], s.F(q.f), D, T, D, D, s.st)) return rc;
        AddLnArgs n2{s.F(q.x1), s.F(q.f), data[W.g2], data[W.be2], s.F(L.X[l + 1]), s.F(q.xh2), s.F(q.rstd2), T, D, kEps, s.dp, s.seed, sid_enc(l, 3)};
        if (int rc = add_ln_fwd(n2, s.st)) return rc;
    }
    return mask_rows(s.F(L.X[cfg.n_layers]), tok_row, s.F(L.HID), s.B, s.S, D, s.st);
}
int HeadPlan::encode_pre(const HeadStep& s, const int32_t* tok_row) const {
    const HLayout& L = s.L;
    const int D = cfg.hidden_dim, T = s.T, H = cfg.heads, hd = D / H;
    float* zero = s.F(L.t0);
    TCVN_CHECK(hipMemsetAsync(zero, 0, (size_t)T * D * 4, s.st));
    for (int l = 0; l < cfg.n_layers; ++l) {
        const HLayer& W = layers[l];
        const HLayBuf& q = L.lay[l];
        AddLnArgs n1{s.F(L.X[l]), zero, data[W.g1], data[W.be1], s.F(q.h1), s.F(q.xh1), s.F(q.rstd1), T, D, kEps, 0.f, s.seed, sid_enc(l, 1)};
        if (int rc = add_ln_fwd(n1, s.st)) return rc;
        if (int rc = linear_fwd(s.F(q.h1), D, data[W.win], data[W.bin], s.F(q.qkv), 3 * D, T, 3 * D, D, s.st)) return rc;
        AttnArgs a{s.F(q.qkv), tok_row, s.F(q.probs), s.F(q.ctx), s.B, s.S, H, hd, s.dp, s.seed, sid_enc(l, 0)};
        if (int rc = attn_fwd(a, s.st)) return rc;
        if (int rc = linear_fwd(s.F(q.ctx), D, data[W.wo], data[W.bo], s.F(q.ao), D, T, D, D, s.st)) return rc;
        if (int rc = add_drop(s.F(L.X[l]), s.F(q.ao), s.F(q.x1), (long)T * D, s.dp, s.seed, sid_enc(l, 1), s.st)) return rc;
        AddLnArgs n2{s.F(q.x1), zero, data[W.g2], data[W.be2], s.F(q.h2), s.F(q.xh2), s.F(q.rstd2), T, D, kEps, 0.f, s.seed, sid_enc(l, 3)};
        if (int rc = add_ln_fwd(n2, s.st)) return rc;
        if (int rc = linear_fwd(s.F(q.h2), D, data[W.w1], data[W.b1], s.F(q.hpre), D, T, D, D, s.st)) return rc;
        if (int rc = act_fwd(s.F(q.hpre), s.F(q.hact), (long)T * D, cfg.gelu, s.dp, s.seed, sid_enc(l, 2), s.st)) return rc;
        if (int rc = linear_fwd(s.F(q.hact), D, data[W.w2], data[W.b2], s.F(q.f), D, T, D, D, s.st)) return rc;
        if (int rc = add_drop(s.F(q.x1), s.F(q.f), s.F(L.X[l + 1]), (long)T * D, s.dp, s.seed, sid_enc(l, 3), s.st)) return rc;
    }
    return mask_rows(s.F(L.X[cfg.n_layers]), tok_row, s.F(L.HID), s.B, s.S, D, s.st);
}

int HeadPlan::decode(const HeadStep& s, float* ev_logits, float* pr_logits) const {
    const HLayout& L = s.L;
    const int D = cfg.hidden_dim, TP = s.TP, n_dec = (int)dec.size();
    if (ev_logits)
        if (int rc = linear_fwd(s.F(L.HID), D, data[ew], data[eb], ev_logits, cfg.event_classes, s.B, cfg.event_classes, D, s.st)) return rc;
    if (!pr_logits || TP == 0) return 0;
    for (int i = 0; i < n_dec; ++i) {
        const HDec& d = dec[i];
        const DecIn in = dec_in(s, i);
        if (int rc = linear_fwd(in.x, in.w, data[d.w], data[d.b], s.F(L.Zd[i]), d.out, TP, d.out, d.in, s.st)) return rc;
        if (int rc = rows_bn_fwd(block_fwd(d, s, L.Zd[i], L.Ad[i], L.dstat[i], TP), s.st)) return rc;
    }
    const DecIn in = dec_in(s, n_dec);
    if (int rc = linear_fwd(in.x, in.w, data[ow], data[ob], s.F(L.LG), cfg.prong_classes, TP, cfg.prong_classes, cfg.dec_out_in, s.st)) return rc;
    return permute_rows(s.F(L.LG), pr_logits, s.B, s.P, cfg.prong_classes, 1, s.st);
}

int HeadPlan::forward(int B, int P, int nP, const float* rows, const int32_t* tok_row, float* ev_logits, float* pr_logits,
                      void* ws, long ws_bytes, int train, uint64_t seed, hipStream_t st) {
    HeadStep s;
    if (int rc = step(B, P, nP, ws, ws_bytes, train, seed, st, s)) return rc;
    if (int rc = embed(s, rows, tok_row)) return rc;
    if (int rc = encode(s, tok_row)) return rc;
    if (int rc = decode(s, ev_logits, pr_logits)) return rc;
    last_seed = seed;
    return 0;
}

int HeadPlan::loss(int B, int P, const float* ev_logits, const float* pr_logits, const int64_t* et, const int8_t* pt, float* losses,
                   float* accs, float* dEv, float* dPr, hipStream_t st) {
    float* lb = accs + 2;
    if (int rc = focal_i64(ev_logits, et, B, cfg.event_classes, cfg.gamma, cfg.event_weight, dEv, lb, st)) return rc;
    if (int rc = focal_i8(pr_logits, pt, B * P, cfg.prong_classes, cfg.gamma, 1.f - cfg.event_weight, dPr, lb + 2, st)) return rc;
    hipLaunchKernelGGL(k_combine_loss, dim3(1), dim3(1), 0, st, lb, lb + 2, cfg.event_weight, losses, accs);
    TCVN_LAUNCH_CHECK();
    return 0;
}

int HeadPlan::backward(int B, int P, int nP, const float* rows, const int32_t* tok_row, const float* dEv, const float* dPr,
                       float* d_rows, void* ws, long ws_bytes, hipStream_t st) {
    if (bound)
        for (size_t i = 0; i < slots.size(); ++i)
            if (slots[i].kind == TCVN_SLOT_PARAM && grad[i] == nullptr) return -14;
    HeadStep s;
    if (int rc = step(B, P, nP, ws, ws_bytes, 1, last_seed, st, s)) return rc;
    if (int rc = decoders_bwd(s, dEv, dPr)) return rc;
    float* dX = s.F(s.L.t2);
    if (int rc = mask_rows(s.F(s.L.dHID), tok_row, dX, B, s.S, cfg.hidden_dim, st)) return rc;
    int rc = 0;
    switch (enc_path(s.S)) {
    case EncPath::FUSED: rc = encoder_bwd_fused(s, dX, s.F(s.L.t3)); dX = s.F(s.L.t3); break;
    case EncPath::POST_NORM: rc = encoder_bwd_post(s, dX); break;
    case EncPath::PRE_NORM: rc = encoder_bwd_pre(s, dX); break;
    }
    return rc ? rc : embed_bwd(s, dX, rows, tok_row, d_rows);
}

int HeadPlan::decoders_bwd(const HeadStep& s, const float* dEv, const float* dPr) const {
    const HLayout& L = s.L;
    const int D = cfg.hidden_dim, TP = s.TP, Ce = cfg.event_classes, Cp = cfg.prong_classes, n_dec = (int)dec.size();
    if (int rc = permute_rows(dPr, s.F(L.dLG), s.B, s.P, Cp, 0, s.st)) return rc;
    const DecIn last = dec_in(s, n_dec);
    if (int rc = linear_bwd_dw(s.F(L.dLG), Cp, last.x, last.w, grad[ow], grad[ob], TP, Cp, last.w, s.st)) return rc;
    if (int rc = linear_bwd_dx(s.F(L.dLG), Cp, data[ow], last.dx, last.w, TP, Cp, last.w, 0, s.st)) return rc;
    float* dZ = s.F(L.t1);
    for (int i = n_dec - 1; i >= 0; --i) {
        const HDec& d = dec[i];
        const DecIn in = dec_in(s, i);
        if (int rc = rows_bn_bwd(block_bwd(d, s, L.Zd[i], L.t0, L.dstat[i], L.t1, TP), s.st)) return rc;
        if (int rc = linear_bwd_dw(dZ, d.out, in.x, in.w, grad[d.w], grad[d.b], TP, d.out, d.in, s.st)) return rc;
        if (int rc = linear_bwd_dx(dZ, d.out, data[d.w], in.dx, in.w, TP, d.out, d.in, 0, s.st)) return rc;
    }
    if (int rc = linear_bwd_dw(dEv, Ce, s.F(L.HID), D, grad[ew], grad[eb], s.B, Ce, D, s.st)) return rc;
    return linear_bwd_dx(dEv, Ce, data[ew], s.F(L.dHID), D, s.B, Ce, D, 0, s.st);
}

int HeadPlan::encoder_bwd_fused(const HeadStep& s, const float* dY, float* dX) const {
    const HLayout& L = s.L;
    const int D = cfg.hidden_dim;
    EncFusedBwdArgs a{};
    a.dY = dY; a.dX = dX; a.lnp = s.F(L.lnp); a.B = s.B; a.S = s.S; a.H = cfg.heads; a.L = cfg.n_layers; a.gelu = cfg.gelu;
    a.drop_p = s.dp; a.seed = s.seed;
    EncWgradArgs w{};
    w.T = s.T; w.B = s.B; w.L = cfg.n_layers; w.lnp = s.F(L.lnp);
    int nj = 0, nt = 0;
    for (int l = 0; l < cfg.n_layers; ++l) {
        const HLayer& W = layers[l];
        const HLayBuf& q = L.lay[l];
        a.w[l] = enc_w(l); a.buf[l] = enc_buf(s, l);
        a.g[l] = EncLayerGrad{s.F(q.g_dqkv), s.F(q.g_dao), s.F(q.g_dhp), s.F(q.g_df)};
        w.job[nj++] = EncWgradJob{s.F(q.g_dqkv), 3 * D, s.F(L.X[l]), grad[W.win], grad[W.bin], 3 * D / 32};
        w.job[nj++] = EncWgradJob{s.F(q.g_dao), D, s.F(q.ctx), grad[W.wo], grad[W.bo], D / 32};
        w.job[nj++] = EncWgradJob{s.F(q.g_dhp), D, s.F(q.x1), grad[W.w1], grad[W.b1], D / 32};
        w.job[nj++] = EncWgradJob{s.F(q.g_df), D, s.F(q.hact), grad[W.w2], grad[W.b2], D / 32};
        nt += 3 * D / 32 + 3 * (D / 32);
        w.ln_dst[l][0] = grad[W.g1]; w.ln_dst[l][1] = grad[W.be1]; w.ln_dst[l][2] = grad[W.g2]; w.ln_dst[l][3] = grad[W.be2];
    }
    w.n_jobs = nj; w.n_tiles = nt;
    return encoder_fused_bwd(a, w, s.st);
}

int HeadPlan::encoder_bwd_post(const HeadStep& s, float* dX) const {
    const HLayout& L = s.L;
    const int D = cfg.hidden_dim, T = s.T, H = cfg.heads, hd = D / H;
    float *d1 = s.F(L.t3), *dR = s.F(L.t0), *dT = s.F(L.t1);
    for (int l = cfg.n_layers - 1; l >= 0; --l) {
        const HLayer& W = layers[l];
        const HLayBuf& q = L.lay[l];
        AddLnBwdArgs n2{dX, s.F(q.xh2), s.F(q.rstd2), data[W.g2], d1, dR, grad[W.g2], grad[W.be2], T, D, s.dp, s.seed, sid_enc(l, 3)};
        if (int rc = add_ln_bwd(n2, s.st)) return rc;
        if (int rc = linear_bwd_dw(dR, D, s.F(q.hact), D, grad[W.w2], grad[W.b2], T, D, D, s.st)) return rc;
        if (int rc = linear_bwd_dx(dR, D, data[W.w2], dT, D, T, D, D, 0, s.st)) return rc;
        if (int rc = act_bwd(s.F(q.hpre), dT, dR, (long)T * D, cfg.gelu, s.dp, s.seed, sid_enc(l, 2), s.st)) return rc;
        if (int rc = linear_bwd_dw(dR, D, s.F(q.x1), D, grad[W.w1], grad[W.b1], T, D, D, s.st)) return rc;
        if (int rc = linear_bwd_dx(dR, D, data[W.w1], d1, D, T, D, D, 1, s.st)) return rc;
        AddLnBwdArgs n1{d1, s.F(q.xh1), s.F(q.rstd1), data[W.g1], dX, dR, grad[W.g1], grad[W.be1], T, D, s.dp, s.seed, sid_enc(l, 1)};
        if (int rc = add_ln_bwd(n1, s.st)) return rc;
        if (int rc = linear_bwd_dw(dR, D, s.F(q.ctx), D, grad[W.wo], grad[W.bo], T, D, D, s.st)) return rc;
        if (int rc = linear_bwd_dx(dR, D, data[W.wo], dT, D, T, D, D, 0, s.st)) return rc;
        AttnBwdArgs ab{s.F(q.qkv), s.F(q.probs), dT, dR, s.B, s.S, H, hd, s.dp, s.seed, sid_enc(l, 0)};
        if (int rc = attn_bwd(ab, s.st)) return rc;
        if (int rc = linear_bwd_dw(dR, 3 * D, s.F(L.X[l]), D, grad[W.win], grad[W.bin], T, 3 * D, D, s.st)) return rc;
        if (int rc = linear_bwd_dx(dR, 3 * D, data[W.win], dX, D, T, 3 * D, D, 1, s.st)) return rc;
    }
    return 0;
}

int HeadPlan::encoder_bwd_pre(const HeadStep& s, float* dX) const {
    const HLayout& L = s.L;
    const int D = cfg.hidden_dim, T = s.T, H = cfg.heads, hd = D / H;
    const long n = (long)T * D;
    float *d1 = s.F(L.t3), *dR = s.F(L.t0), *dT = s.F(L.t1);
    float* dS = s.F(L.dHID);
    for (int l = cfg.n_layers - 1; l >= 0; --l) {
        const HLayer& W = layers[l];
        const HLayBuf& q = L.lay[l];
        if (int rc = mul_drop(dX, dR, n, s.dp, s.seed, sid_enc(l, 3), s.st)) return rc;
        if (int rc = linear_bwd_dw(dR, D, s.F(q.hact), D, grad[W.w2], grad[W.b2], T, D, D, s.st)) return rc;
        if (int rc = linear_bwd_dx(dR, D, data[W.w2], dT, D, T, D, D, 0, s.st)) return rc;
        if (int rc = act_bwd(s.F(q.hpre), dT, dR, n, cfg.gelu, s.dp, s.seed, sid_enc(l, 2), s.st)) return rc;
        if (int rc = linear_bwd_dw(dR, D, s.F(q.h2), D, grad[W.w1], grad[W.b1], T, D, D, s.st)) return rc;
        if (int rc = linear_bwd_dx(dR, D, data[W.w1], dT, D, T, D, D, 0, s.st)) return rc;
        AddLnBwdArgs n2{dT, s.F(q.xh2), s.F(q.rstd2), data[W.g2], dS, d1, grad[W.g2], grad[W.be2], T, D, 0.f, s.seed, sid_enc(l, 3)};
        if (int rc = add_ln_bwd(n2, s.st)) return rc;
        if (int rc = add_inplace(dX, dS, n, s.st)) return rc;
        if (int rc = mul_drop(dX, dR, n, s.dp, s.seed, sid_enc(l, 1), s.st)) return rc;
        if (int rc = linear_bwd_dw(dR, D, s.F(q.ctx), D, grad[W.wo], grad[W.bo], T, D, D, s.st)) return rc;
        if (int rc = linear_bwd_dx(dR, D, data[W.wo], dT, D, T, D, D, 0, s.st)) return rc;
        AttnBwdArgs ab{s.F(q.qkv), s.F(q.probs), dT, dR, s.B, s.S, H, hd, s.dp, s.seed, sid_enc(l, 0)};
        if (int rc = attn_bwd(ab, s.st)) return rc;
        if (int rc = linear_bwd_dw(dR, 3 * D, s.F(q.h1), D, grad[W.win], grad[W.bin], T, 3 * D, D, s.st)) return rc;
        if (int rc = linear_bwd_dx(dR, 3 * D, data[W.win], dT, D, T, 3 * D, D, 0, s.st)) return rc;
        AddLnBwdArgs n1{dT, s.F(q.xh1), s.F(q.rstd1), data[W.g1], dS, d1, grad[W.g1], grad[W.be1], T, D, 0.f, s.seed, sid_enc(l, 1)};
        if (int rc = add_ln_bwd(n1, s.st)) return rc;
        if (int rc = add_inplace(dX, dS, n, s.st)) return rc;
    }
    return 0;
}

int HeadPlan::embed_bwd(const HeadStep& s, const float* dX0, const float* rows, const int32_t* tok_row, float* d_rows) const {
    const HLayout& L = s.L;
    const int D = cfg.hidden_dim;
    if (int rc = scatter_tokens_bwd(dX0, tok_row, s.F(L.dC), s.B, s.S, D, s.st)) return rc;
    if (int rc = rows_bn_bwd(block_bwd(comb, s, L.Zc, L.dC, L.cstat, L.dZc, s.R), s.st)) return rc;
    if (int rc = linear_bwd_dw(s.F(L.dZc), D, rows, cfg.in_dim, grad[comb.w], comb.b >= 0 ? grad[comb.b] : nullptr, s.R, D, cfg.in_dim, s.st)) return rc;
    return linear_bwd_dx(s.F(L.dZc), D, data[comb.w], d_rows, cfg.in_dim, s.R, D, cfg.in_dim, 0, s.st);
}

struct tcvn_head {
    HeadPlan plan;
    int last_np = 0, last_b = 0, last_p = -1;
    explicit tcvn_head(const tcvn_head_cfg& c) : plan(c) {}
};

namespace {
struct LooLayout { long jobs, src, lg, vrow, head, total; int cap; };
void loo_layout(const HeadPlan& plan, int B, int P, LooLayout& o) {
    Bump b;
    const long slots = (long)B * (1 + P);
    o.cap = (int)(slots < TCVN_LOO_MAX_PASS ? slots : TCVN_LOO_MAX_PASS);
    o.jobs = b.take(slots * 4); o.src = b.take(slots * 4); o.lg = b.take(slots * plan.cfg.event_classes * 4);
    o.vrow = b.take((long)o.cap * (1 + P) * 4);
    HLayout L;
    plan.layout(o.cap, P, 0, L);
    o.head = b.take(L.total);
    o.total = b.off;
}
struct ShapHost { std::vector<int64_t> offsets, vmask; std::vector<int32_t> n, exact; };
bool shap_shape_ok(int batch, int max_prongs, int max_exact, int samples) {
    return batch > 0 && batch <= 65535 && max_prongs >= 0 && max_prongs <= 63 && max_exact >= 0 && max_exact <= TCVN_SHAP_MAX_EXACT &&
           samples >= 1;
}
long shap_jobs(int n, int max_exact, int M) { return n <= max_exact ? 1L << n : 2 + (long)M * (n - 1); }
int shap_read_table(const int32_t* tok_row, int B, int S, int max_exact, int M, hipStream_t st, ShapHost& h) {
    std::vector<int32_t> tr((size_t)B * S);
    TCVN_CHECK(hipMemcpyAsync(tr.data(), tok_row, tr.size() * 4, hipMemcpyDeviceToHost, st));
    TCVN_CHECK(hipStreamSynchronize(st));
    h.offsets.assign(B + 1, 0); h.vmask.assign(B, 0); h.n.assign(B, 0); h.exact.assign(B, 0);
    for (int b = 0; b < B; ++b) {
        for (int s = 1; s < S; ++s)
            if (tr[(size_t)b * S + s] >= 0) { h.vmask[b] |= (int64_t)1 << (s - 1); ++h.n[b]; }
        h.exact[b] = h.n[b] <= max_exact;
        h.offsets[b + 1] = h.offsets[b] + shap_jobs(h.n[b], max_exact, M);
    }
    return 0;
}
struct ShapLayout { long n, vmask, pos, values, vrow, head, total; long cap; };
void shap_layout(const HeadPlan& plan, int B, int P, int max_exact, int M, ShapLayout& o) {
    Bump b;
    long per_event = 1L << (P < max_exact ? P : max_exact);
    if (P > max_exact && shap_jobs(P, max_exact, M) > per_event) per_event = shap_jobs(P, max_exact, M);
    const long jmax = per_event * B;
    o.cap = jmax < TCVN_SHAP_MAX_PASS ? jmax : TCVN_SHAP_MAX_PASS;
    o.n = b.take((long)B * 4); o.vmask = b.take((long)B * 8); o.pos = b.take((long)B * M * (P > 0 ? P : 1) * 4);
    o.values = b.take(jmax * plan.cfg.event_classes * 8);
    o.vrow = b.take(o.cap * (1 + P) * 4);
    HLayout L;
    plan.layout((int)o.cap, P, 0, L);
    o.head = b.take(L.total);
    o.total = b.off;
}
struct OccHeadLayout { long vrows, ident, vrow, head, total; HLayout E; };
void occ_head_layout(const HeadPlan& plan, int P, OccHeadLayout& o) {
    Bump b;
    const long cap = TCVN_OCC_MAX_PASS, D = plan.cfg.hidden_dim;
    o.vrows = b.take(cap * plan.cfg.in_dim * 4); o.ident = b.take(cap * 4); o.vrow = b.take(cap * (1 + P) * 4);
    o.E.Zc = b.take(cap * D * 4); o.E.C = b.take(cap * D * 4); o.E.cstat = b.take(2 * D * 4);
    o.E.X.assign(1, b.take(cap * D * 4));
    HLayout L;
    plan.layout((int)cap, P, 0, L);
    o.head = b.take(L.total);
    o.total = b.off;
}
}


extern "C" {
int tcvn_head_create(const tcvn_head_cfg* cfg, tcvn_head** out) {
    if (!cfg || !out || cfg->n_dec < 0 || cfg->n_dec > 8 || cfg->hidden_dim % cfg->heads != 0) return -1;
    *out = new tcvn_head(*cfg);
    return 0;
}
void tcvn_head_destroy(tcvn_head* p) { delete p; }
int tcvn_head_num_slots(const tcvn_head* p) { return (int)p->plan.slots.size(); }
int tcvn_head_slot(const tcvn_head* p, int i, char* name, int cap, int64_t* numel, int* kind) {
    if (i < 0 || i >= (int)p->plan.slots.size()) return -1;
    const auto& s = p->plan.slots[i];
    if (name && cap > 0) { strncpy(name, s.name.c_str(), cap - 1); name[cap - 1] = 0; }
    if (numel) *numel = s.numel;
    if (kind) *kind = s.kind;
    return 0;
}
int tcvn_head_bind(tcvn_head* p, void* const* data, void* const* grad) { return p->plan.bind(data, grad); }
void tcvn_head_set_fused_encoder(tcvn_head* p, int on) { p->plan.fused_encoder = on != 0; }
int64_t tcvn_head_workspace_bytes(const tcvn_head* p, int batch, int max_prongs, int n_prongs) {
    HLayout L;
    p->plan.layout(batch, max_prongs, n_prongs, L);
    return L.total;
}
int tcvn_head_forward(tcvn_head* p, int batch, int max_prongs, int n_prongs, const float* rows, const int32_t* tok_row,
                      float* event_logits, float* prong_logits, void* ws, int64_t ws_bytes, int train, uint64_t seed, void* stream) {
    p->last_np = n_prongs; p->last_b = batch; p->last_p = max_prongs;
    return p->plan.forward(batch, max_prongs, n_prongs, rows, tok_row, event_logits, prong_logits, ws, ws_bytes, train, seed,
                           reinterpret_cast<hipStream_t>(stream));
}
int tcvn_head_embed(tcvn_head* p, int batch, int max_prongs, int n_prongs, const float* rows, const int32_t* tok_row, float* tokens,
                    void* ws, int64_t ws_bytes, int train, uint64_t seed, void* stream) {
    HeadStep s;
    if (int rc = p->plan.step(batch, max_prongs, n_prongs, ws, ws_bytes, train, seed, reinterpret_cast<hipStream_t>(stream), s)) return rc;
    if (int rc = p->plan.embed(s, rows, tok_row)) return rc;
    return permute_rows(s.F(s.L.X[0]), tokens, batch, s.S, p->plan.cfg.hidden_dim, 1, s.st);
}
int tcvn_head_encode(tcvn_head* p, int batch, int max_prongs, const float* tokens, const int32_t* tok_row, float* hidden, void* ws,
                     int64_t ws_bytes, int train, uint64_t seed, void* stream) {
    HeadStep s;
    if (int rc = p->plan.step(batch, max_prongs, 0, ws, ws_bytes, train, seed, reinterpret_cast<hipStream_t>(stream), s)) return rc;
    const int D = p->plan.cfg.hidden_dim;
    float* X0 = s.F(s.L.X[0]);
    if (int rc = permute_rows(tokens, X0, batch, s.S, D, 0, s.st)) return rc;
    if (int rc = mask_rows(X0, tok_row, X0, batch, s.S, D, s.st)) return rc;
    if (int rc = p->plan.encode(s, tok_row)) return rc;
    p->last_np = 0; p->last_b = batch; p->last_p = max_prongs;
    TCVN_CHECK(hipMemcpyAsync(hidden, s.F(s.L.HID), (size_t)s.T * D * 4, hipMemcpyDeviceToDevice, s.st));
    return 0;
}
int tcvn_head_decode(tcvn_head* p, int batch, int max_prongs, const float* hidden, float* event_logits, float* prong_logits,
                     void* ws, int64_t ws_bytes, int train, uint64_t seed, void* stream) {
    HeadStep s;
    if (int rc = p->plan.step(batch, max_prongs, 0, ws, ws_bytes, train, seed, reinterpret_cast<hipStream_t>(stream), s)) return rc;
    TCVN_CHECK(hipMemcpyAsync(s.F(s.L.HID), hidden, (size_t)s.T * p->plan.cfg.hidden_dim * 4, hipMemcpyDeviceToDevice, s.st));
    return p->plan.decode(s, event_logits, prong_logits);
}

int tcvn_head_attention(tcvn_head* p, int batch, int max_prongs, const int32_t* tok_row, const void* ws, int64_t ws_bytes,
                        float* weights, void* stream) {
    if (!p || !tok_row || !ws || !weights || batch <= 0 || max_prongs < 0 || 1 + max_prongs > 64) {
        fprintf(stderr, "tcvn: head_attention: bad argument (NULL pointer, batch < 1 or more than 64 tokens)\n");
        return -1;
    }
    if (batch != p->last_b || max_prongs != p->last_p) {
        fprintf(stderr, "tcvn: head_attention: no forward / encode of shape (batch %d, max_prongs %d) precedes this call\n", batch, max_prongs);
        return -15;
    }
    HLayout L;
    p->plan.layout(batch, max_prongs, p->last_np, L);
    if (ws_bytes < L.total) {
        fprintf(stderr, "tcvn: head_attention: workspace of %lld bytes, the forward's has %ld\n", (long long)ws_bytes, L.total);
        return -12;
    }
    const int nl = p->plan.cfg.n_layers;
    if (nl < 1) { fprintf(stderr, "tcvn: head_attention: the encoder has no layer\n"); return -1; }
    const long stride = nl > 1 ? L.lay[1].probs - L.lay[0].probs : 0;
    for (int l = 1; l < nl; ++l)
        if (L.lay[l].probs - L.lay[l - 1].probs != stride) return -16;
    return attn_export(reinterpret_cast<const char*>(ws), L.lay[0].probs, stride, tok_row, weights, nl, batch, p->plan.cfg.heads,
                       1 + max_prongs, reinterpret_cast<hipStream_t>(stream));
}
int64_t tcvn_head_leave_one_out_workspace_bytes(const tcvn_head* p, int batch, int max_prongs) {
    if (!p || batch <= 0 || max_prongs < 0 || 1 + max_prongs > 64) return -1;
    LooLayout o;
    loo_layout(p->plan, batch, max_prongs, o);
    return o.total;
}
int tcvn_head_leave_one_out(tcvn_head* p, int batch, int max_prongs, const float* tokens, const int32_t* tok_row, float* event_logits,
                            float* loo, void* ws, int64_t ws_bytes, void* stream) {
    if (!p || !tokens || !tok_row || !event_logits || !ws || (max_prongs > 0 && !loo) || batch <= 0 || max_prongs < 0 ||
        1 + max_prongs > 64) {
        fprintf(stderr, "tcvn: head_leave_one_out: bad argument (NULL pointer, batch < 1 or more than 64 tokens)\n");
        return -1;
    }
    LooLayout o;
    loo_layout(p->plan, batch, max_prongs, o);
    if (ws_bytes < o.total) {
        fprintf(stderr, "tcvn: head_leave_one_out: workspace of %lld bytes, %ld needed\n", (long long)ws_bytes, o.total);
        return -12;
    }
    if (!p->plan.bound) { fprintf(stderr, "tcvn: head_leave_one_out: parameters are not bound\n"); return -11; }
    hipStream_t st = reinterpret_cast<hipStream_t>(stream);
    const int B = batch, P = max_prongs, S = 1 + P, D = p->plan.cfg.hidden_dim, Ce = p->plan.cfg.event_classes;
    char* w = reinterpret_cast<char*>(ws);
    std::vector<int32_t> tr((size_t)B * S), jobs, src((size_t)B * S);
    TCVN_CHECK(hipMemcpyAsync(tr.data(), tok_row, tr.size() * 4, hipMemcpyDeviceToHost, st));
    TCVN_CHECK(hipStreamSynchronize(st));
    for (int b = 0; b < B; ++b) { jobs.push_back(b * S); src[(size_t)b * S] = b; }
    for (int b = 0; b < B; ++b)
        for (int s = 1; s < S; ++s) {
            const bool valid = tr[(size_t)b * S + s] >= 0;
            src[(size_t)b * S + s] = valid ? (int32_t)jobs.size() : b;
            if (valid) jobs.push_back(b * S + s);
        }
    const int J = (int)jobs.size();
    int* d_jobs = reinterpret_cast<int*>(w + o.jobs);
    int* d_src = reinterpret_cast<int*>(w + o.src);
    int* d_vrow = reinterpret_cast<int*>(w + o.vrow);
    float* lg = reinterpret_cast<float*>(w + o.lg);
    TCVN_CHECK(hipMemcpyAsync(d_jobs, jobs.data(), (size_t)J * 4, hipMemcpyHostToDevice, st));
    TCVN_CHECK(hipMemcpyAsync(d_src, src.data(), src.size() * 4, hipMemcpyHostToDevice, st));
    TCVN_CHECK(hipStreamSynchronize(st));
    for (int off = 0; off < J; off += o.cap) {
        const int n = J - off < o.cap ? J - off : o.cap;
        HeadStep s;
        if (int rc = p->plan.step(n, P, 0, w + o.head, ws_bytes - o.head, 0, 0, st, s)) return rc;
        if (int rc = loo_gather(tokens, tok_row, d_jobs + off, s.F(s.L.X[0]), d_vrow, n, S, D, st)) return rc;
        if (int rc = p->plan.encode(s, d_vrow)) return rc;
        if (int rc = p->plan.decode(s, lg + (long)off * Ce, nullptr)) return rc;
    }
    return loo_scatter(lg, d_src, event_logits, loo, B, S, Ce, st);
}

int64_t tcvn_head_shapley_workspace_bytes(const tcvn_head* p, int batch, int max_prongs, int max_exact, int samples) {
    if (!p || !shap_shape_ok(batch, max_prongs, max_exact, samples)) return -1;
    ShapLayout o;
    shap_layout(p->plan, batch, max_prongs, max_exact, samples, o);
    return o.total;
}
int64_t tcvn_head_shapley_count(int batch, int max_prongs, const int32_t* tok_row, int max_exact, int samples, void* stream) {
    if (!tok_row || !shap_shape_ok(batch, max_prongs, max_exact, samples)) {
        fprintf(stderr, "tcvn: head_shapley_count: bad argument (NULL pointer, batch outside 1..65535, max_prongs outside 0..63, max_exact outside 0..%d or samples < 1)\n",
                TCVN_SHAP_MAX_EXACT);
        return -1;
    }
    ShapHost h;
    if (shap_read_table(tok_row, batch, 1 + max_prongs, max_exact, samples, reinterpret_cast<hipStream_t>(stream), h)) return -2;
    return h.offsets[batch];
}
int tcvn_head_shapley(tcvn_head* p, int batch, int max_prongs, const float* tokens, const int32_t* tok_row, int max_exact, int samples,
                      uint64_t seed, int value_kind, float* event_logits, float* phi, float* std_error, float* interaction,
                      int32_t* exact, int64_t* offsets, int64_t* masks, int32_t* event, float* coalition_logits, int64_t n_coalitions,
                      int32_t* permutations, void* ws, int64_t ws_bytes, void* stream) {
    const bool prongs = max_prongs > 0;
    if (!p || !tokens || !tok_row || !event_logits || !exact || !offsets || !masks || !event || !coalition_logits || !ws ||
        (prongs && (!phi || !std_error || !interaction || !permutations)) || !shap_shape_ok(batch, max_prongs, max_exact, samples) ||
        (value_kind != TCVN_SHAP_VALUE_PROB && value_kind != TCVN_SHAP_VALUE_LOGIT) || n_coalitions < batch) {
        fprintf(stderr, "tcvn: head_shapley: bad argument (NULL pointer, batch outside 1..65535, max_prongs outside 0..63, max_exact outside 0..%d, samples < 1, unknown value kind or fewer coalitions than events)\n",
                TCVN_SHAP_MAX_EXACT);
        return -1;
    }
    ShapLayout o;
    shap_layout(p->plan, batch, max_prongs, max_exact, samples, o);
    if (ws_bytes < o.total) {
        fprintf(stderr, "tcvn: head_shapley: workspace of %lld bytes, %ld needed\n", (long long)ws_bytes, o.total);
        return -12;
    }
    if (!p->plan.bound) { fprintf(stderr, "tcvn: head_shapley: parameters are not bound\n"); return -11; }
    hipStream_t st = reinterpret_cast<hipStream_t>(stream);
    const int B = batch, P = max_prongs, S = 1 + P, M = samples, D = p->plan.cfg.hidden_dim, Ce = p->plan.cfg.event_classes;
    char* w = reinterpret_cast<char*>(ws);
    ShapHost h;
    if (int rc = shap_read_table(tok_row, B, S, max_exact, M, st, h)) return rc;
    const long J = h.offsets[B];
    if (J != n_coalitions) {
        fprintf(stderr, "tcvn: head_shapley: outputs sized for %lld coalitions, this mask has %ld (tcvn_head_shapley_count)\n",
                (long long)n_coalitions, J);
        return -13;
    }
    int32_t* d_n = reinterpret_cast<int32_t*>(w + o.n);
    int64_t* d_vmask = reinterpret_cast<int64_t*>(w + o.vmask);
    double* values = reinterpret_cast<double*>(w + o.values);
    int* d_vrow = reinterpret_cast<int*>(w + o.vrow);
    TCVN_CHECK(hipMemcpyAsync(offsets, h.offsets.data(), (size_t)(B + 1) * 8, hipMemcpyHostToDevice, st));
    TCVN_CHECK(hipMemcpyAsync(exact, h.exact.data(), (size_t)B * 4, hipMemcpyHostToDevice, st));
    TCVN_CHECK(hipMemcpyAsync(d_n, h.n.data(), (size_t)B * 4, hipMemcpyHostToDevice, st));
    TCVN_CHECK(hipMemcpyAsync(d_vmask, h.vmask.data(), (size_t)B * 8, hipMemcpyHostToDevice, st));
    TCVN_CHECK(hipStreamSynchronize(st));
    const ShapTable t{offsets, d_n, d_vmask, exact};
    int32_t* d_pos = reinterpret_cast<int32_t*>(w + o.pos);
    if (int rc = shap_perm(tok_row, permutations, d_pos, B, M, P, seed, st)) return rc;
    for (long off = 0; off < J; off += o.cap) {
        const int n = (int)(J - off < o.cap ? J - off : o.cap);
        HeadStep s;
        if (int rc = p->plan.step(n, P, 0, w + o.head, ws_bytes - o.head, 0, 0, st, s)) return rc;
        if (int rc = shap_gather(tokens, tok_row, t, permutations, off, n, B, M, S, D, s.F(s.L.X[0]), d_vrow, masks, event, st)) return rc;
        if (int rc = p->plan.encode(s, d_vrow)) return rc;
        if (int rc = p->plan.decode(s, coalition_logits + off * Ce, nullptr)) return rc;
    }
    if (int rc = shap_full_rows(coalition_logits, t, event_logits, B, Ce, st)) return rc;
    if (int rc = shap_values(coalition_logits, values, J, Ce, value_kind == TCVN_SHAP_VALUE_PROB, st)) return rc;
    if (int rc = shap_exact(values, t, phi, std_error, B, P, Ce, st)) return rc;
    if (int rc = shap_pairs(values, t, interaction, B, P, Ce, st)) return rc;
    return shap_sampled(values, t, d_pos, phi, std_error, B, M, P, Ce, st);
}

int64_t tcvn_head_occlusion_workspace_bytes(const tcvn_head* p, int max_prongs) {
    if (!p || max_prongs < 0 || 1 + max_prongs > 64) return -1;
    OccHeadLayout o;
    occ_head_layout(p->plan, max_prongs, o);
    return o.total;
}
int tcvn_head_occlusion(tcvn_head* p, int batch, int max_prongs, int n_prongs, const float* rows, const float* tokens,
                        const int32_t* tok_row, int n, const int32_t* vimg, const int32_t* index, int row_base, const float* emb,
                        int64_t emb_ld, int col0, int width, float* occluded_event_logits, float* occluded_prong_logits, void* ws,
                        int64_t ws_bytes, void* stream) {
    if (!p || !rows || !tokens || !tok_row || !vimg || !index || !emb || !occluded_event_logits || !ws ||
        (max_prongs > 0 && !occluded_prong_logits) || batch <= 0 || max_prongs < 0 || 1 + max_prongs > 64 || n_prongs < 0 || n < 1 ||
        n > TCVN_OCC_MAX_PASS || row_base < 0 || row_base > batch + n_prongs || col0 < 0 || width < 1 ||
        col0 + width > p->plan.cfg.in_dim || emb_ld < width) {
        fprintf(stderr, "tcvn: head_occlusion: bad argument (NULL pointer, batch < 1, more than 64 tokens, n outside 1..%d or columns outside the row)\n",
                TCVN_OCC_MAX_PASS);
        return -1;
    }
    OccHeadLayout o{};
    occ_head_layout(p->plan, max_prongs, o);
    if (ws_bytes < o.total) {
        fprintf(stderr, "tcvn: head_occlusion: workspace of %lld bytes, %ld needed\n", (long long)ws_bytes, o.total);
        return -12;
    }
    if (!p->plan.bound) { fprintf(stderr, "tcvn: head_occlusion: parameters are not bound\n"); return -11; }
    hipStream_t st = reinterpret_cast<hipStream_t>(stream);
    const int P = max_prongs, S = 1 + P, D = p->plan.cfg.hidden_dim;
    char* w = reinterpret_cast<char*>(ws);
    float* vrows = reinterpret_cast<float*>(w + o.vrows);
    int* ident = reinterpret_cast<int*>(w + o.ident);
    int* d_vrow = reinterpret_cast<int*>(w + o.vrow);
    if (int rc = occ_rows(rows, vimg, row_base, emb, emb_ld, col0, width, vrows, ident, n, p->plan.cfg.in_dim, batch + n_prongs, st)) return rc;
    HeadStep e, s;
    if (int rc = p->plan.step(n, 0, 0, w, ws_bytes, 0, 0, st, e)) return rc;
    e.L = o.E;
    if (int rc = p->plan.embed(e, vrows, ident)) return rc;
    if (int rc = p->plan.step(n, P, 0, w + o.head, ws_bytes - o.head, 0, 0, st, s)) return rc;
    if (int rc = occ_gather(tokens, tok_row, index, e.F(o.E.X[0]), s.F(s.L.X[0]), d_vrow, n, batch, S, D, st)) return rc;
    if (int rc = p->plan.encode(s, d_vrow)) return rc;
    return p->plan.decode(s, occluded_event_logits, occluded_prong_logits);
}

int tcvn_head_loss(tcvn_head* p, int batch, int max_prongs, const float* event_logits, const float* prong_logits,
                   const int64_t* event_targets, const int8_t* prong_targets, float* losses, float* accs, float* d_event_logits,
                   float* d_prong_logits, void* stream) {
    return p->plan.loss(batch, max_prongs, event_logits, prong_logits, event_targets, prong_targets, losses, accs, d_event_logits,
                        d_prong_logits, reinterpret_cast<hipStream_t>(stream));
}
int tcvn_head_backward(tcvn_head* p, int batch, int max_prongs, int n_prongs, const float* rows, const int32_t* tok_row,
                       const float* d_event_logits, const float* d_prong_logits, float* d_rows, void* ws, int64_t ws_bytes,
                       void* stream) {
    return p->plan.backward(batch, max_prongs, n_prongs, rows, tok_row, d_event_logits, d_prong_logits, d_rows, ws, ws_bytes,
                            reinterpret_cast<hipStream_t>(stream));
}
}

extern "C" int tcvn_linear_forward(const float* x, int64_t ldx, const float* weight, const float* bias, float* y, int64_t ldy,
                                   int rows, int n_out, int n_in, void* stream) {
    if (!x || !weight || !y || rows < 0 || n_out <= 0 || n_in <= 0) return -1;
    if (rows == 0) return 0;
    return linear_fwd(x, ldx, weight, bias, y, ldy, rows, n_out, n_in, reinterpret_cast<hipStream_t>(stream));
}
extern "C" int tcvn_rows_bn_prelu_forward(const float* x, int64_t ldx, int rows, int channels, const float* gamma, const float* beta,
                                          const float* slope, float* running_mean, float* running_var, float* y, int64_t ldy,
                                          float* save_mean_rstd, int train, float drop_p, uint64_t seed, uint32_t stream_id,
                                          void* stream) {
    const bool no_norm = !gamma && !beta && !running_mean && !running_var;
    if (!x || !y || rows <= 0 || channels <= 0) return -1;
    if (!no_norm && (!gamma || !beta || !running_mean || !running_var || !save_mean_rstd)) return -1;
    RowsBnArgs r{};
    r.no_norm = no_norm ? 1 : 0;
    r.X = x; r.ldx = ldx; r.R = rows; r.C = channels; r.gamma = gamma; r.beta = beta; r.slope = slope;
    r.running_mean = running_mean; r.running_var = running_var; r.Y = y; r.ldy = ldy;
    r.save_mean = save_mean_rstd; r.save_rstd = save_mean_rstd ? save_mean_rstd + channels : nullptr; r.train = train; r.eps = kEps; r.momentum = kMom;
    r.drop_p = train ? drop_p : 0.f; r.seed = seed; r.stream_id = stream_id;
    return rows_bn_fwd(r, reinterpret_cast<hipStream_t>(stream));
}

extern "C" int tcvn_linear_backward(const float* dy, int64_t lddy, const float* x, int64_t ldx, const float* weight, float* dx, int64_t lddx,
                                    float* dweight, float* dbias, int rows, int n_out, int n_in, void* stream) {
    if (!dy || !x || !weight || rows <= 0 || n_out <= 0 || n_in <= 0) return -1;
    hipStream_t st = reinterpret_cast<hipStream_t>(stream);
    int rc;
    if (dweight && (rc = linear_bwd_dw(dy, lddy, x, ldx, dweight, dbias, rows, n_out, n_in, st))) return rc;
    if (dx && (rc = linear_bwd_dx(dy, lddy, weight, dx, lddx, rows, n_out, n_in, 0, st))) return rc;
    return 0;
}
extern "C" int tcvn_rows_bn_prelu_backward(const float* x, int64_t ldx, const float* dy, int64_t lddy, int rows, int channels,
                                           const float* gamma, const float* beta, const float* slope, const float* save_mean_rstd,
                                           float* dx, int64_t lddx, float* dgamma, float* dbeta, float* dslope, float drop_p,
                                           uint64_t seed, uint32_t stream_id, void* stream) {
    const bool no_norm = !gamma && !beta && !dgamma && !dbeta;
    if (!x || !dy || !dx || rows <= 0 || channels <= 0 || (slope != nullptr) != (dslope != nullptr)) return -1;
    if (!no_norm && (!gamma || !beta || !save_mean_rstd || !dgamma || !dbeta)) return -1;
    RowsBnBwdArgs r{};
    r.no_norm = no_norm ? 1 : 0;
    r.X = x; r.ldx = ldx; r.dY = dy; r.lddy = lddy; r.R = rows; r.C = channels; r.gamma = gamma; r.beta = beta; r.slope = slope;
    r.save_mean = save_mean_rstd; r.save_rstd = save_mean_rstd ? save_mean_rstd + channels : nullptr; r.dX = dx; r.lddx = lddx;
    r.dgamma = dgamma; r.dbeta = dbeta; r.dslope = dslope; r.drop_p = drop_p; r.seed = seed; r.stream_id = stream_id;
    return rows_bn_bwd(r, reinterpret_cast<hipStream_t>(stream));
}

extern "C" int tcvn_focal_loss(const float* logits, const int64_t* targets, int rows, int classes, float gamma, float weight,
                               float* d_logits, float* out2, void* stream) {
    return focal_i64(logits, targets, rows, classes, gamma, weight, d_logits, out2, reinterpret_cast<hipStream_t>(stream));
}
```

### dune-transformercvn_amd/csrc/head_plan.h

```cpp
#pragma once
#include <string>
#include <vector>

#include "../../include/tcvn_hip.h"
#include "tcvn_common.h"
#include "tcvn_rows.h"
#include "tcvn_encoder.h"

namespace tcvn {

struct HBn { int w = -1, b = -1, rm = -1, rv = -1; };
struct HLayer { int win, bin, wo, bo, w1, b1, w2, b2, g1, be1, g2, be2; };
struct HDec { int w, b = -1, a = -1, in, out; HBn n; uint32_t sid = 0; bool drop = false; };
struct HLayBuf { long qkv, probs, ctx, ao, xh1, rstd1, x1, hpre, hact, f, xh2, rstd2, g_dqkv, g_dao, g_dhp, g_df,
                 h1, h2; };
struct HLayout {
    long Zc, C, cstat, HID, LG, dEv, dPr, lossbuf, dLG, t0, t1, t2, t3, dHID, dC, dZc, lnp, total;
    std::vector<long> X, Zd, Ad, dstat;
    std::vector<HLayBuf> lay;
};

struct HeadStep {
    int B, P, nP, S, T, R, TP;
    char* ws; HLayout L;
    int train; uint64_t seed; float dp; hipStream_t st;
    float* F(long off) const { return reinterpret_cast<float*>(ws + off); }
};
enum class EncPath { FUSED, POST_NORM, PRE_NORM };
struct DecIn { const float* x; float* dx; int w; };

struct HeadPlan {
    tcvn_head_cfg cfg;
    std::vector<Slot> slots;
    std::vector<float*> data, grad;
    HDec comb;
    int ew, eb, ow, ob, dec_width;
    std::vector<HLayer> layers;
    std::vector<HDec> dec;
    bool bound = false;
    bool fused_encoder = true;
    uint64_t last_seed = 0;

    explicit HeadPlan(const tcvn_head_cfg& c);
    int add_slot(const std::string& name, long numel, int kind);
    HBn add_bn(const std::string& p, int c);
    int bind(void* const* d, void* const* g);
    void layout(int B, int P, int nP, HLayout& L) const;
    int step(int B, int P, int nP, void* ws, long ws_bytes, int train, uint64_t seed, hipStream_t st, HeadStep& s) const;
    EncPath enc_path(int S) const;
    EncLayerW enc_w(int l) const;  EncLayerBuf enc_buf(const HeadStep& s, int l) const;
    RowsBnArgs block_fwd(const HDec& d, const HeadStep& s, long X, long Y, long stat, int rows) const;
    RowsBnBwdArgs block_bwd(const HDec& d, const HeadStep& s, long X, long dY, long stat, long dX, int rows) const;
    DecIn dec_in(const HeadStep& s, int i) const;
    int embed(const HeadStep& s, const float* rows, const int32_t* tok_row) const;
    int encode(const HeadStep& s, const int32_t* tok_row) const, encode_post(const HeadStep& s, const int32_t* tok_row) const,
        encode_pre(const HeadStep& s, const int32_t* tok_row) const;
    int decode(const HeadStep& s, float* ev_logits, float* pr_logits) const;
    int forward(int B, int P, int nP, const float* rows, const int32_t* tok_row, float* ev_logits, float* pr_logits, void* ws,
                long ws_bytes, int train, uint64_t seed, hipStream_t st);
    int loss(int B, int P, const float* ev_logits, const float* pr_logits, const int64_t* et, const int8_t* pt, float* losses,
             float* accs, float* dEv, float* dPr, hipStream_t st);
    int backward(int B, int P, int nP, const float* rows, const int32_t* tok_row, const float* dEv, const float* dPr, float* d_rows,
                 void* ws, long ws_bytes, hipStream_t st);
    int decoders_bwd(const HeadStep& s, const float* dEv, const float* dPr) const;
    int encoder_bwd_fused(const HeadStep& s, const float* dY, float* dX) const;
    int encoder_bwd_post(const HeadStep& s, float* dX) const, encoder_bwd_pre(const HeadStep& s, float* dX) const;
    int embed_bwd(const HeadStep& s, const float* dX0, const float* rows, const int32_t* tok_row, float* d_rows) const;
};

}
```

### dune-transformercvn_amd/csrc/rows.hip

```cpp
#include "tcvn_rows.h"

namespace tcvn {

namespace {

__global__ __launch_bounds__(256) void k_sgemm(const SgemmArgs a) {
    constexpr int KP = 128;
    __shared__ float As[16][KP + 1], Bs[16][KP + 1];
    const int tx = threadIdx.x & 15, ty = threadIdx.x >> 4;
    const int i = blockIdx.y * 16 + ty, j = blockIdx.x * 16 + tx;
    const int jb = blockIdx.x * 16 + ty;
    float acc = 0.f;
    for (int k0 = 0; k0 < a.K; k0 += KP) {
        float va[KP / 16], vb[KP / 16];
#pragma unroll
        for (int q = 0; q < KP / 16; ++q) {
            const int k = k0 + tx + 16 * q;
            va[q] = (i < a.M && k < a.K) ? a.A[(long)i * a.sai + (long)k * a.sak] : 0.f;
            vb[q] = (jb < a.N && k < a.K) ? a.B[(long)jb * a.sbj + (long)k * a.sbk] : 0.f;
        }
#pragma unroll
        for (int q = 0; q < KP / 16; ++q) { As[ty][tx + 16 * q] = va[q]; Bs[ty][tx + 16 * q] = vb[q]; }
        __syncthreads();
        const int kn = a.K - k0 < KP ? a.K - k0 : KP;
        if (kn == KP) {
#pragma unroll 16
            for (int k = 0; k < KP; ++k) acc = fmaf(As[ty][k], Bs[tx][k], acc);
        } else {
            for (int k = 0; k < kn; ++k) acc = fmaf(As[ty][k], Bs[tx][k], acc);
        }
        __syncthreads();
    }
    if (i < a.M && j < a.N) {
        float v = a.alpha * acc + (a.bias ? a.bias[j] : 0.f);
        float* c = a.C + (long)i * a.ldc + j;
        *c = a.accumulate ? *c + v : v;
    }
}

__global__ __launch_bounds__(256) void k_rows_bn_fwd(const RowsBnArgs a) {
    __shared__ double red[16][16][2];
    __shared__ float s_mean[16], s_rstd[16];
    const int cl = threadIdx.x & 15, rg = threadIdx.x >> 4;
    const int c = blockIdx.x * 16 + cl;
    const bool ok = c < a.C;
    if (a.no_norm) {
        if (!ok) return;
        const float sl = a.slope ? a.slope[c] : 0.f;
        for (int r = rg; r < a.R; r += 16) {
            float z = prelu(a.X[(long)r * a.ldx + c], sl);
            if (a.train && a.drop_p > 0.f) z *= drop_scale(a.drop_p, a.seed, a.stream_id, (uint64_t)r * a.C + c);
            a.Y[(long)r * a.ldy + c] = z;
        }
        return;
    }
    if (a.train) {
        double s1 = 0, s2 = 0;
        if (ok)
            for (int r = rg; r < a.R; r += 16) { const double v = a.X[(long)r * a.ldx + c]; s1 += v; s2 += v * v; }
        red[rg][cl][0] = s1; red[rg][cl][1] = s2;
        __syncthreads();
        if (rg == 0 && ok) {
            double x = 0, y = 0;
            for (int g = 0; g < 16; ++g) { x += red[g][cl][0]; y += red[g][cl][1]; }
            const double mean = x / a.R;
            double var = y / a.R - mean * mean;
            if (var < 0) var = 0;
            s_mean[cl] = (float)mean;
            s_rstd[cl] = (float)(1.0 / sqrt(var + (double)a.eps));
            if (a.save_mean) { a.save_mean[c] = s_mean[cl]; a.save_rstd[c] = s_rstd[cl]; }
            if (a.running_mean) {
                const double unb = a.R > 1 ? var * a.R / (double)(a.R - 1) : var;
                a.running_mean[c] = (1.f - a.momentum) * a.running_mean[c] + a.momentum * (float)mean;
                a.running_var[c] = (1.f - a.momentum) * a.running_var[c] + a.momentum * (float)unb;
            }
        }
        __syncthreads();
    } else if (rg == 0 && ok) {
        s_mean[cl] = a.running_mean[c];
        s_rstd[cl] = 1.0f / sqrtf(a.running_var[c] + a.eps);
    }
    if (!a.train) __syncthreads();
    if (!ok) return;
    const float mean = s_mean[cl], rstd = s_rstd[cl];
    const float g = a.gamma ? a.gamma[c] : 1.f, b = a.beta ? a.beta[c] : 0.f;
    const float sl = a.slope ? a.slope[c] : 0.f;
    for (int r = rg; r < a.R; r += 16) {
        const float u = (a.X[(long)r * a.ldx + c] - mean) * rstd * g + b;
        float z = prelu(u, sl);
        if (a.train && a.drop_p > 0.f) z *= drop_scale(a.drop_p, a.seed, a.stream_id, (uint64_t)r * a.C + c);
        a.Y[(long)r * a.ldy + c] = z;
    }
}

__global__ __launch_bounds__(256) void k_rows_bn_bwd(const RowsBnBwdArgs a) {
    __shared__ double red[16][16][3];
    __shared__ float s_db[16], s_dg[16];
    const int cl = threadIdx.x & 15, rg = threadIdx.x >> 4;
    const int c = blockIdx.x * 16 + cl;
    const bool ok = c < a.C;
    if (a.no_norm) {
        const float sl = (ok && a.slope) ? a.slope[c] : 0.f;
        double s3 = 0;
        if (ok)
            for (int r = rg; r < a.R; r += 16) {
                const float u = a.X[(long)r * a.ldx + c];
                float dz = a.dY[(long)r * a.lddy + c];
                if (a.drop_p > 0.f) dz *= drop_scale(a.drop_p, a.seed, a.stream_id, (uint64_t)r * a.C + c);
                if (a.dX) a.dX[(long)r * a.lddx + c] = u > 0.f ? dz : sl * dz;
                s3 += u > 0.f ? 0.f : dz * u;
            }
        red[rg][cl][0] = s3;
        __syncthreads();
        if (rg == 0 && ok && a.dslope) {
            double z = 0;
            for (int q = 0; q < 16; ++q) z += red[q][cl][0];
            a.dslope[c] += (float)z;
        }
        return;
    }
    const float mean = ok ? a.save_mean[c] : 0.f, rstd = ok ? a.save_rstd[c] : 0.f;
    const float g = (ok && a.gamma) ? a.gamma[c] : 1.f, b = (ok && a.beta) ? a.beta[c] : 0.f;
    const float sl = (ok && a.slope) ? a.slope[c] : 0.f;
    double s1 = 0, s2 = 0, s3 = 0;
    if (ok)
        for (int r = rg; r < a.R; r += 16) {
            const float xh = (a.X[(long)r * a.ldx + c] - mean) * rstd;
            const float u = xh * g + b;
            float dz = a.dY[(long)r * a.lddy + c];
            if (a.drop_p > 0.f) dz *= drop_scale(a.drop_p, a.seed, a.stream_id, (uint64_t)r * a.C + c);
            const float du = u > 0.f ? dz : sl * dz;
            s1 += du; s2 += (double)du * xh; s3 += u > 0.f ? 0.f : dz * u;
        }
    red[rg][cl][0] = s1; red[rg][cl][1] = s2; red[rg][cl][2] = s3;
    __syncthreads();
    if (rg == 0 && ok) {
        double x = 0, y = 0, z = 0;
        for (int q = 0; q < 16; ++q) { x += red[q][cl][0]; y += red[q][cl][1]; z += red[q][cl][2]; }
        s_db[cl] = (float)x; s_dg[cl] = (float)y;
        if (a.dbeta) a.dbeta[c] += (float)x;
        if (a.dgamma) a.dgamma[c] += (float)y;
        if (a.dslope) a.dslope[c] += (float)z;
    }
    __syncthreads();
    if (!ok || a.dX == nullptr) return;
    const float db = s_db[cl] / a.R, dg = s_dg[cl] / a.R;
    for (int r = rg; r < a.R; r += 16) {
        const float xh = (a.X[(long)r * a.ldx + c] - mean) * rstd;
        const float u = xh * g + b;
        float dz = a.dY[(long)r * a.lddy + c];
        if (a.drop_p > 0.f) dz *= drop_scale(a.drop_p, a.seed, a.stream_id, (uint64_t)r * a.C + c);
        const float du = u > 0.f ? dz : sl * dz;
        a.dX[(long)r * a.lddx + c] = g * rstd * (du - db - xh * dg);
    }
}

__global__ __launch_bounds__(256) void k_colsum_acc(const float* dY, long lddy, int R, int N, float* db) {
    __shared__ double sa[16][17];
    const int cl = threadIdx.x & 15, rl = threadIdx.x >> 4, n = blockIdx.x * 16 + cl;
    double s = 0;
    if (n < N)
        for (int r = rl; r < R; r += 16) s += dY[(long)r * lddy + n];
    sa[rl][cl] = s;
    __syncthreads();
    if (threadIdx.x < 16 && n < N) {
        double x = 0;
#pragma unroll
        for (int i = 0; i < 16; ++i) x += sa[i][cl];
        db[n] += (float)x;
    }
}

}

int linear_bwd_dw(const float* dY, long lddy, const float* X, long ldx, float* dW, float* db, int R, int N, int K, hipStream_t st) {
    if (R <= 0) return 0;
    SgemmArgs a{dY, 1, lddy, X, 1, ldx, dW, (long)K, N, K, R, nullptr, 1.f, 1};
    int rc = sgemm(a, st);
    if (rc) return rc;
    if (db) {
        hipLaunchKernelGGL(k_colsum_acc, dim3(cdiv(N, 16)), dim3(256), 0, st, dY, lddy, R, N, db);
        TCVN_LAUNCH_CHECK();
    }
    return 0;
}

int sgemm(const SgemmArgs& a, hipStream_t st) {
    if (a.M <= 0 || a.N <= 0) return 0;
    hipLaunchKernelGGL(k_sgemm, dim3(cdiv(a.N, 16), cdiv(a.M, 16)), dim3(256), 0, st, a);
    TCVN_LAUNCH_CHECK();
    return 0;
}
int rows_bn_fwd(const RowsBnArgs& a, hipStream_t st) {
    if (a.R <= 0) return 0;
    hipLaunchKernelGGL(k_rows_bn_fwd, dim3(cdiv(a.C, 16)), dim3(256), 0, st, a);
    TCVN_LAUNCH_CHECK();
    return 0;
}
int rows_bn_bwd(const RowsBnBwdArgs& a, hipStream_t st) {
    if (a.R <= 0) return 0;
    hipLaunchKernelGGL(k_rows_bn_bwd, dim3(cdiv(a.C, 16)), dim3(256), 0, st, a);
    TCVN_LAUNCH_CHECK();
    return 0;
}

}
```

### dune-transformercvn_amd/csrc/tcvn_encoder.h

```cpp
#pragma once
#include "tcvn_common.h"

namespace tcvn {

int gather_tokens(const float* C, const int* tok_row, float* X, int B, int S, int D, hipStream_t st);
int scatter_tokens_bwd(const float* dX, const int* tok_row, float* dC, int B, int S, int D, hipStream_t st);
int mask_rows(const float* X, const int* tok_row, float* Y, int B, int S, int D, hipStream_t st);
int permute_rows(const float* in, float* out, int B, int P, int C, int to_batch_major, hipStream_t st);

struct AttnArgs {
    const float* qkv; const int* tok_row; float* probs; float* ctx;
    int B, S, H, hd; float drop_p; uint64_t seed; uint32_t stream_id;
};
int attn_fwd(const AttnArgs& a, hipStream_t st);
struct AttnBwdArgs {
    const float* qkv; const float* probs; const float* dctx; float* dqkv;
    int B, S, H, hd; float drop_p; uint64_t seed; uint32_t stream_id;
};
int attn_bwd(const AttnBwdArgs& a, hipStream_t st);

struct AddLnArgs {
    const float* X; const float* R; const float *gamma, *beta; float* Y; float* XH; float* rstd;
    int T, D; float eps; float drop_p; uint64_t seed; uint32_t stream_id;
};
int add_ln_fwd(const AddLnArgs& a, hipStream_t st);
struct AddLnBwdArgs {
    const float* dY; const float* XH; const float* rstd; const float* gamma; float* dX; float* dR; float *dgamma, *dbeta;
    int T, D; float drop_p; uint64_t seed; uint32_t stream_id;
};
int add_ln_bwd(const AddLnBwdArgs& a, hipStream_t st);

int act_fwd(const float* X, float* Y, long n, int gelu, float drop_p, uint64_t seed, uint32_t sid, hipStream_t st);
int act_bwd(const float* X, const float* dY, float* dX, long n, int gelu, float drop_p, uint64_t seed, uint32_t sid, hipStream_t st);
int add_inplace(float* dst, const float* src, long n, hipStream_t st);
int add_drop(const float* x, const float* r, float* y, long n, float drop_p, uint64_t seed, uint32_t sid, hipStream_t st);
int mul_drop(const float* dy, float* dr, long n, float drop_p, uint64_t seed, uint32_t sid, hipStream_t st);

constexpr int ENC_MAX_LAYERS = 8;
struct EncLayerW { const float *win, *bin, *wo, *bo, *w1, *b1, *w2, *b2, *g1, *be1, *g2, *be2; };
struct EncLayerBuf { float *qkv, *probs, *ctx, *xh1, *rstd1, *x1, *hpre, *hact, *xh2, *rstd2, *xnext; };
struct EncFusedArgs {
    const float* X0; const int* tok_row; float* HID;
    int B, S, H, L, gelu, save; float eps, drop_p; uint64_t seed;
    EncLayerW w[ENC_MAX_LAYERS]; EncLayerBuf buf[ENC_MAX_LAYERS];
};
bool encoder_fused_ok(int S, int D, int H, int L, int norm_first);
int encoder_fused_fwd(const EncFusedArgs& a, hipStream_t st);
struct EncLayerGrad { float *dqkv, *dao, *dhp, *df; };
struct EncFusedBwdArgs {
    const float* dY; float* dX; float* lnp;
    int B, S, H, L, gelu; float drop_p; uint64_t seed;
    EncLayerW w[ENC_MAX_LAYERS]; EncLayerBuf buf[ENC_MAX_LAYERS]; EncLayerGrad g[ENC_MAX_LAYERS];
};
struct EncWgradJob { const float* dY; int ldy; const float* X; float* dW; float* db; int tiles; };
struct EncWgradArgs {
    int T, B, L, n_jobs, n_tiles; const float* lnp;
    float* ln_dst[ENC_MAX_LAYERS][4];
    EncWgradJob job[4 * ENC_MAX_LAYERS];
};
int encoder_fused_bwd(const EncFusedBwdArgs& a, const EncWgradArgs& w, hipStream_t st);

int focal_i64(const float* logits, const int64_t* targets, int rows, int C, float gamma, float weight, float* dlogits, float* out,
              hipStream_t st);
int focal_i8(const float* logits, const int8_t* targets, int rows, int C, float gamma, float weight, float* dlogits, float* out,
             hipStream_t st);

}
```

### dune-transformercvn_amd/csrc/tcvn_rows.h

```cpp
#pragma once
#include "tcvn_common.h"

namespace tcvn {

struct SgemmArgs {
    const float* A; long sai, sak;
    const float* B; long sbj, sbk;
    float* C; long ldc;
    int M, N, K;
    const float* bias; float alpha; int accumulate;
};
int sgemm(const SgemmArgs& a, hipStream_t st);

static inline int linear_fwd(const float* X, long ldx, const float* W, const float* b, float* Y, long ldy, int R, int N, int K,
                             hipStream_t st) {
    SgemmArgs a{X, ldx, 1, W, (long)K, 1, Y, ldy, R, N, K, b, 1.f, 0};
    return sgemm(a, st);
}
static inline int linear_bwd_dx(const float* dY, long lddy, const float* W, float* dX, long lddx, int R, int N, int K,
                                int accumulate, hipStream_t st) {
    SgemmArgs a{dY, lddy, 1, W, 1, (long)K, dX, lddx, R, K, N, nullptr, 1.f, accumulate};
    return sgemm(a, st);
}
int linear_bwd_dw(const float* dY, long lddy, const float* X, long ldx, float* dW, float* db, int R, int N, int K, hipStream_t st);

struct RowsBnArgs {
    const float* X; long ldx; int R, C;
    const float *gamma, *beta, *slope;
    float *running_mean, *running_var;
    float* Y; long ldy;
    float *save_mean, *save_rstd;
    int train; float eps, momentum;
    float drop_p; uint64_t seed; uint32_t stream_id;
    int no_norm;
};
int rows_bn_fwd(const RowsBnArgs& a, hipStream_t st);

struct RowsBnBwdArgs {
    const float* X; long ldx; const float* dY; long lddy; int R, C;
    const float *gamma, *beta, *slope;
    const float *save_mean, *save_rstd;
    float* dX; long lddx;
    float *dgamma, *dbeta, *dslope;
    float drop_p; uint64_t seed; uint32_t stream_id;
    int no_norm;
};
int rows_bn_bwd(const RowsBnBwdArgs& a, hipStream_t st);

}
```

### dune-transformercvn_amd/transformercvn/hip/_lib.py

```python
from __future__ import annotations

import ctypes as C
import os

import torch

from . import _libselect

_HERE = os.path.dirname(os.path.abspath(__file__))
LIB_PATH = os.path.normpath(os.path.join(_HERE, "..", "..", "lib", _libselect.NAME))
_libselect._bound = True

MODE_F32, MODE_BF16 = 0, 1
SLOT_PARAM, SLOT_BUFFER, SLOT_COUNTER = 0, 1, 2
FUSE_MEAN, FUSE_MAX = 0, 1
LOO_MAX_PASS = 256
SHAP_MAX_PASS = 1024
SHAP_MAX_EXACT = 16
SHAP_VALUE_PROB, SHAP_VALUE_LOGIT = 0, 1
OCC_MAX_PASS = 256
OCC_TARGET_EVENT, OCC_TARGET_PRONG = 0, 1
OCC_GROUP_EVENT, OCC_GROUP_MAP = 0, 1
OCC_MAX_LEVELS = 16
CURVE_MAX_STEPS, CURVE_MAX_TILES = 64, 4096
CURVE_DELETION, CURVE_INSERTION = 0, 1


class DenseNetCfg(C.Structure):
    _fields_ = [("in_ch", C.c_int), ("out_dim", C.c_int), ("init_ch", C.c_int), ("growth", C.c_int), ("bn_size", C.c_int),
                ("n_blocks", C.c_int), ("layers", C.c_int * 8), ("H", C.c_int), ("W", C.c_int), ("dropout", C.c_float),
                ("mode", C.c_int)]


class SdxlCfg(C.Structure):
    _fields_ = [("in_ch", C.c_int), ("out_dim", C.c_int), ("init_ch", C.c_int), ("repeat", C.c_int), ("num_blocks", C.c_int),
                ("H", C.c_int), ("W", C.c_int), ("mode", C.c_int)]


class HeadCfg(C.Structure):
    _fields_ = [("hidden_dim", C.c_int), ("heads", C.c_int), ("n_layers", C.c_int), ("in_dim", C.c_int),
                ("event_classes", C.c_int), ("prong_classes", C.c_int), ("n_dec", C.c_int), ("dec_dims", C.c_int * 8),
                ("dec_out_in", C.c_int), ("gelu", C.c_int), ("norm_first", C.c_int), ("dropout_modules", C.c_int),
                ("dropout", C.c_float), ("gamma", C.c_float), ("event_weight", C.c_float),
                ("no_linear_bn", C.c_int), ("linear_relu", C.c_int)]


def _load():
    if not os.path.exists(LIB_PATH):
        raise ImportError(
            f"libtcvn_hip.so not found at {LIB_PATH}: build it with `make -C dune-transformercvn_amd/csrc -j8` "
            "(hipcc, --offload-arch=gfx950). There is no CPU fallback for the TransformerCVN hot path.")
    lib = C.CDLL(LIB_PATH)
    vp, i32, i64, u64, f32 = C.c_void_p, C.c_int, C.c_int64, C.c_uint64, C.c_float
    P = C.POINTER

    def sig(name, res, *args):
        fn = getattr(lib, name)
        fn.restype = res
        fn.argtypes = list(args)
        return fn

    sig("tcvn_version", i32)
    sig("tcvn_densenet_create", i32, P(DenseNetCfg), P(vp))
    sig("tcvn_densenet_destroy", None, vp)
    sig("tcvn_densenet_num_slots", i32, vp)
    sig("tcvn_densenet_slot", i32, vp, i32, C.c_char_p, i32, P(i64), P(i32))
    sig("tcvn_densenet_bind", i32, vp, P(vp), P(vp))
    sig("tcvn_densenet_workspace_bytes", i64, vp, i32, i32)
    sig("tcvn_densenet_forward", i32, vp, i32, vp, vp, i64, i32, f32, vp, i64, vp, i64, i32, u64, vp)
    sig("tcvn_densenet_backward", i32, vp, i32, vp, i64, vp, i64, vp)
    sig("tcvn_densenet_num_blocks", i32, vp)
    sig("tcvn_densenet_backward_blocks", i32, vp, i32, vp, i64, vp, i64, i32, i32, vp)
    sig("tcvn_densenet_tap", i32, vp, i32, C.c_char_p, P(i64), P(i32), P(i32), P(i32), P(i32), P(i32), P(i32))
    sig("tcvn_sdxl_create", i32, P(SdxlCfg), P(vp))
    sig("tcvn_sdxl_destroy", None, vp)
    sig("tcvn_sdxl_num_slots", i32, vp)
    sig("tcvn_sdxl_slot", i32, vp, i32, C.c_char_p, i32, P(i64), P(i32))
    sig("tcvn_sdxl_bind", i32, vp, P(vp), P(vp))
    sig("tcvn_sdxl_workspace_bytes", i64, vp, i32, i32)
    sig("tcvn_sdxl_forward", i32, vp, i32, vp, vp, i64, i32, f32, vp, i64, vp, i64, i32, u64, vp)
    sig("tcvn_sdxl_backward", i32, vp, i32, vp, i64, vp, i64, vp)
    sig("tcvn_sdxl_tap", i32, vp, i32, C.c_char_p, P(i64), P(i32), P(i32), P(i32), P(i32), P(i32), P(i32))
    sig("tcvn_head_create", i32, P(HeadCfg), P(vp))
    sig("tcvn_head_destroy", None, vp)
    sig("tcvn_head_num_slots", i32, vp)
    sig("tcvn_head_slot", i32, vp, i32, C.c_char_p, i32, P(i64), P(i32))
    sig("tcvn_head_bind", i32, vp, P(vp), P(vp))
    sig("tcvn_head_workspace_bytes", i64, vp, i32, i32, i32)
    sig("tcvn_head_forward", i32, vp, i32, i32, i32, vp, vp, vp, vp, vp, i64, i32, u64, vp)
    sig("tcvn_head_loss", i32, vp, i32, i32, vp, vp, vp, vp, vp, vp, vp, vp, vp)
    sig("tcvn_head_backward", i32, vp, i32, i32, i32, vp, vp, vp, vp, vp, vp, i64, vp)
    sig("tcvn_head_set_fused_encoder", None, vp, i32)
    sig("tcvn_head_embed", i32, vp, i32, i32, i32, vp, vp, vp, vp, i64, i32, u64, vp)
    sig("tcvn_head_encode", i32, vp, i32, i32, vp, vp, vp, vp, i64, i32, u64, vp)
    sig("tcvn_head_decode", i32, vp, i32, i32, vp, vp, vp, vp, i64, i32, u64, vp)
    sig("tcvn_head_attention", i32, vp, i32, i32, vp, vp, i64, vp, vp)
    sig("tcvn_attention_rollout", i32, vp, vp, i32, i32, i32, i32, i32, vp, vp)
    sig("tcvn_head_leave_one_out_workspace_bytes", i64, vp, i32, i32)
    sig("tcvn_head_leave_one_out", i32, vp, i32, i32, vp, vp, vp, vp, vp, i64, vp)
    sig("tcvn_head_shapley_workspace_bytes", i64, vp, i32, i32, i32, i32)
    sig("tcvn_head_shapley_count", i64, i32, i32, vp, i32, i32, vp)
    sig("tcvn_head_shapley", i32, vp, i32, i32, vp, vp, i32, i32, u64, i32, vp, vp, vp, vp, vp, vp, vp, vp, vp, i64, vp, vp, i64, vp)
    sig("tcvn_occlusion_workspace_bytes", i64, i32, i32, i32, i32, i32, i32)
    sig("tcvn_occlusion_variants", i32, vp, i64, i32, i32, i32, i32, i32, vp, i32, vp, vp, vp, i64, P(i64), i64, vp)
    sig("tcvn_occlusion_build_pass", i32, vp, vp, i64, i32, i32, i32, i32, i32, i32, i32, vp, vp, i64, i32, i32, vp, vp, i64, vp)
    sig("tcvn_head_occlusion_workspace_bytes", i64, vp, i32)
    sig("tcvn_head_occlusion", i32, vp, i32, i32, i32, vp, vp, vp, i32, vp, vp, i32, vp, i64, i32, i32, vp, vp, vp, i64, vp)
    sig("tcvn_occlusion_heatmap", i32, vp, vp, vp, vp, vp, i64, i32, i32, i32, i32, i32, i32, i32, vp, vp, vp)
    sig("tcvn_occlusion_select", i32, vp, vp, i64, i32, i32, i32, i32, i32, f32, vp, vp, vp)
    sig("tcvn_occlusion_refine_variants", i32, vp, i64, i32, i32, i32, i32, i32, vp, vp, i32, i32, i32, i32, i32, vp, vp, vp, i64, P(i64),
        i64, vp)
    sig("tcvn_occlusion_mark", i32, vp, i64, i32, i32, i32, i32, vp, vp)
    sig("tcvn_occlusion_occupancy", i32, vp, i64, i32, i32, i32, i32, i32, vp, i32, i32, vp, vp)
    sig("tcvn_occlusion_paint", i32, i32, P(vp), P(vp), P(i32), P(i32), vp, i32, i32, vp, vp)
    sig("tcvn_occlusion_curve_workspace_bytes", i64, i32, i32, i32, i32, i32, i32, i32)
    sig("tcvn_occlusion_curve_variants", i32, vp, i64, i32, i32, i32, i32, i32, vp, vp, i32, i32, i32, i32, vp, i32, vp, vp, vp, i64, P(i64),
        i64, vp)
    sig("tcvn_occlusion_curve_build_pass", i32, vp, vp, i64, i32, i32, i32, i32, i32, i32, i32, i32, i32, vp, vp, i64, i32, i32, vp, vp, i64,
        vp)
    sig("tcvn_occlusion_curve", i32, vp, vp, vp, vp, vp, i64, i32, i32, i32, i32, i32, i32, vp, vp, vp, vp)
    sig("tcvn_linear_forward", i32, vp, i64, vp, vp, vp, i64, i32, i32, i32, vp)
    sig("tcvn_rows_bn_prelu_forward", i32, vp, i64, i32, i32, vp, vp, vp, vp, vp, vp, i64, vp, i32, f32, u64, C.c_uint32, vp)
    sig("tcvn_linear_backward", i32, vp, i64, vp, i64, vp, vp, i64, vp, vp, i32, i32, i32, vp)
    sig("tcvn_rows_bn_prelu_backward", i32, vp, i64, vp, i64, i32, i32, vp, vp, vp, vp, vp, i64, vp, vp, vp, f32, u64, C.c_uint32, vp)
    sig("tcvn_focal_loss", i32, vp, vp, i32, i32, f32, f32, vp, vp, vp)
    sig("tcvn_grad_sumsq", i32, vp, i64, vp, i32, vp, vp)
    sig("tcvn_adamw_step", i32, vp, vp, vp, vp, vp, i64, f32, f32, f32, f32, i64, vp, f32, vp)
    sig("tcvn_dropout_keep", i32, i32, f32, u64, C.c_uint32, i64, i32, vp, vp)
    sig("tcvn_backward_overlap", None, i32)
    sig("tcvn_profile_enable", None, i32)
    sig("tcvn_profile_filter", None, C.c_char_p)
    sig("tcvn_profile_reset", None)
    sig("tcvn_profile_count", i32)
    sig("tcvn_profile_get", i32, i32, C.c_char_p, i32, P(f32), P(C.c_double), P(C.c_double))
    return lib


def profile_records():
    out = []
    buf = C.create_string_buffer(128)
    ms, fl, by = C.c_float(), C.c_double(), C.c_double()
    for i in range(lib.tcvn_profile_count()):
        check(lib.tcvn_profile_get(i, buf, 128, C.byref(ms), C.byref(fl), C.byref(by)), "profile_get")
        out.append((buf.value.decode(), ms.value, fl.value, by.value))
    return out


EXPORTS = [
    "tcvn_grad_sumsq", "tcvn_adamw_step", "tcvn_backward_overlap", "tcvn_profile_enable", "tcvn_profile_filter", "tcvn_profile_reset", "tcvn_profile_count", "tcvn_profile_get",
    "tcvn_focal_loss", "tcvn_dropout_keep", "tcvn_head_set_fused_encoder", "tcvn_head_embed", "tcvn_head_encode", "tcvn_head_decode", "tcvn_linear_forward",
    "tcvn_rows_bn_prelu_forward", "tcvn_linear_backward", "tcvn_rows_bn_prelu_backward", "tcvn_sdxl_create", "tcvn_sdxl_destroy", "tcvn_sdxl_num_slots", "tcvn_sdxl_slot", "tcvn_sdxl_bind",
    "tcvn_sdxl_workspace_bytes", "tcvn_sdxl_forward", "tcvn_sdxl_backward", "tcvn_sdxl_tap",
    "tcvn_version", "tcvn_densenet_create", "tcvn_densenet_destroy", "tcvn_densenet_num_slots", "tcvn_densenet_slot",
    "tcvn_densenet_bind", "tcvn_densenet_workspace_bytes", "tcvn_densenet_forward", "tcvn_densenet_backward",
    "tcvn_densenet_tap", "tcvn_densenet_num_blocks", "tcvn_densenet_backward_blocks", "tcvn_head_create", "tcvn_head_destroy", "tcvn_head_num_slots", "tcvn_head_slot", "tcvn_head_bind",
    "tcvn_head_workspace_bytes", "tcvn_head_forward", "tcvn_head_loss", "tcvn_head_backward",
    "tcvn_head_attention", "tcvn_attention_rollout", "tcvn_head_leave_one_out_workspace_bytes", "tcvn_head_leave_one_out",
    "tcvn_occlusion_workspace_bytes", "tcvn_occlusion_variants", "tcvn_occlusion_build_pass", "tcvn_head_occlusion_workspace_bytes",
    "tcvn_head_occlusion", "tcvn_occlusion_heatmap",
    "tcvn_occlusion_select", "tcvn_occlusion_refine_variants", "tcvn_occlusion_mark", "tcvn_occlusion_occupancy", "tcvn_occlusion_paint",
    "tcvn_occlusion_curve_workspace_bytes", "tcvn_occlusion_curve_variants", "tcvn_occlusion_curve_build_pass", "tcvn_occlusion_curve",
    "tcvn_head_shapley_workspace_bytes", "tcvn_head_shapley_count", "tcvn_head_shapley",
]

lib = _load()


def check(rc: int, what: str):
    if rc != 0:
        raise RuntimeError(f"libtcvn_hip: {what} failed with code {rc}")
```

### include/tcvn_hip.h

```cpp
#ifndef TCVN_HIP_H
#define TCVN_HIP_H

#include <stdint.h>

#ifdef __cplusplus
extern "C" {
#endif

#define TCVN_MODE_F32 0
#define TCVN_MODE_BF16 1

#define TCVN_SLOT_PARAM 0
#define TCVN_SLOT_BUFFER 1
#define TCVN_SLOT_COUNTER 2

int tcvn_version(void);

typedef struct tcvn_densenet_cfg {
    int in_ch;
    int out_dim;
    int init_ch;
    int growth;
    int bn_size;
    int n_blocks;
    int layers[8];
    int H, W;
    float dropout;
    int mode;
} tcvn_densenet_cfg;

typedef struct tcvn_densenet tcvn_densenet;

int tcvn_densenet_create(const tcvn_densenet_cfg* cfg, tcvn_densenet** out);
void tcvn_densenet_destroy(tcvn_densenet* p);

int tcvn_densenet_num_slots(const tcvn_densenet* p);
int tcvn_densenet_slot(const tcvn_densenet* p, int i, char* name, int name_cap, int64_t* numel, int* kind);
int tcvn_densenet_bind(tcvn_densenet* p, void* const* data, void* const* grad);

int64_t tcvn_densenet_workspace_bytes(const tcvn_densenet* p, int n_img, int with_backward);

int tcvn_densenet_forward(tcvn_densenet* p, int n_img, const int32_t* coords, const float* values, int64_t nnz,
                          int log_pixels, float noise_std, float* out, int64_t out_ld, void* workspace,
                          int64_t workspace_bytes, int train, uint64_t seed, void* stream);

int tcvn_densenet_backward(tcvn_densenet* p, int n_img, const float* d_out, int64_t d_out_ld, void* workspace,
                           int64_t workspace_bytes, void* stream);

int tcvn_densenet_num_blocks(const tcvn_densenet* p);
int tcvn_densenet_backward_blocks(tcvn_densenet* p, int n_img, const float* d_out, int64_t d_out_ld, void* workspace,
                                  int64_t workspace_bytes, int block_hi, int block_lo, void* stream);

int tcvn_densenet_tap(const tcvn_densenet* p, int n_img, const char* name, int64_t* byte_off, int* n, int* h, int* w,
                      int* c, int* ld, int* elem_bytes);

typedef struct tcvn_sdxl_cfg {
    int in_ch;
    int out_dim;
    int init_ch;
    int repeat;
    int num_blocks;
    int H, W;
    int mode;
} tcvn_sdxl_cfg;
typedef struct tcvn_sdxl tcvn_sdxl;
int tcvn_sdxl_create(const tcvn_sdxl_cfg* cfg, tcvn_sdxl** out);
void tcvn_sdxl_destroy(tcvn_sdxl* p);
int tcvn_sdxl_num_slots(const tcvn_sdxl* p);
int tcvn_sdxl_slot(const tcvn_sdxl* p, int i, char* name, int name_cap, int64_t* numel, int* kind);
int tcvn_sdxl_bind(tcvn_sdxl* p, void* const* data, void* const* grad);
int64_t tcvn_sdxl_workspace_bytes(const tcvn_sdxl* p, int n_img, int with_backward);
int tcvn_sdxl_forward(tcvn_sdxl* p, int n_img, const int32_t* coords, const float* values, int64_t nnz, int log_pixels,
                      float noise_std, float* out, int64_t out_ld, void* workspace, int64_t workspace_bytes, int train,
                      uint64_t seed, void* stream);
int tcvn_sdxl_backward(tcvn_sdxl* p, int n_img, const float* d_out, int64_t d_out_ld, void* workspace, int64_t workspace_bytes,
                       void* stream);
int tcvn_sdxl_tap(const tcvn_sdxl* p, int n_img, const char* name, int64_t* byte_off, int* n, int* h, int* w, int* c, int* ld,
                  int* elem_bytes);

typedef struct tcvn_head_cfg {
    int hidden_dim, heads, n_layers;
    int in_dim;
    int event_classes, prong_classes;
    int n_dec; int dec_dims[8];
    int dec_out_in;
    int gelu;
    int norm_first;
    int dropout_modules;
    float dropout; float gamma; float event_weight;
    int no_linear_bn;
    int linear_relu;
} tcvn_head_cfg;

typedef struct tcvn_head tcvn_head;
int tcvn_head_create(const tcvn_head_cfg* cfg, tcvn_head** out);
void tcvn_head_destroy(tcvn_head* p);
int tcvn_head_num_slots(const tcvn_head* p);
int tcvn_head_slot(const tcvn_head* p, int i, char* name, int name_cap, int64_t* numel, int* kind);
int tcvn_head_bind(tcvn_head* p, void* const* data, void* const* grad);
int64_t tcvn_head_workspace_bytes(const tcvn_head* p, int batch, int max_prongs, int n_prongs);
void tcvn_head_set_fused_encoder(tcvn_head* p, int on);

int tcvn_head_forward(tcvn_head* p, int batch, int max_prongs, int n_prongs, const float* rows, const int32_t* tok_row,
                      float* event_logits, float* prong_logits, void* workspace, int64_t workspace_bytes, int train,
                      uint64_t seed, void* stream);
int tcvn_head_embed(tcvn_head* p, int batch, int max_prongs, int n_prongs, const float* rows, const int32_t* tok_row, float* tokens,
                    void* workspace, int64_t workspace_bytes, int train, uint64_t seed, void* stream);
int tcvn_head_encode(tcvn_head* p, int batch, int max_prongs, const float* tokens, const int32_t* tok_row, float* hidden,
                     void* workspace, int64_t workspace_bytes, int train, uint64_t seed, void* stream);
int tcvn_head_decode(tcvn_head* p, int batch, int max_prongs, const float* hidden, float* event_logits, float* prong_logits,
                     void* workspace, int64_t workspace_bytes, int train, uint64_t seed, void* stream);

#define TCVN_FUSE_MEAN 0
#define TCVN_FUSE_MAX 1
#define TCVN_LOO_MAX_PASS 256
int tcvn_head_attention(tcvn_head* p, int batch, int max_prongs, const int32_t* tok_row, const void* workspace,
                        int64_t workspace_bytes, float* weights, void* stream);
int tcvn_attention_rollout(const float* weights, const int32_t* tok_row, int layers, int batch, int heads, int seq, int head_fusion,
                           float* rollout, void* stream);
int64_t tcvn_head_leave_one_out_workspace_bytes(const tcvn_head* p, int batch, int max_prongs);
int tcvn_head_leave_one_out(tcvn_head* p, int batch, int max_prongs, const float* tokens, const int32_t* tok_row,
                            float* event_logits, float* loo_event_logits, void* workspace, int64_t workspace_bytes, void* stream);

#define TCVN_SHAP_MAX_PASS 1024
#define TCVN_SHAP_MAX_EXACT 16
#define TCVN_SHAP_VALUE_PROB 0
#define TCVN_SHAP_VALUE_LOGIT 1
int64_t tcvn_head_shapley_workspace_bytes(const tcvn_head* p, int batch, int max_prongs, int max_exact, int samples);
int64_t tcvn_head_shapley_count(int batch, int max_prongs, const int32_t* tok_row, int max_exact, int samples, void* stream);
int tcvn_head_shapley(tcvn_head* p, int batch, int max_prongs, const float* tokens, const int32_t* tok_row, int max_exact, int samples,
                      uint64_t seed, int value_kind, float* event_logits, float* phi, float* std_error, float* interaction,
                      int32_t* exact, int64_t* offsets, int64_t* masks, int32_t* event, float* coalition_logits, int64_t n_coalitions,
                      int32_t* permutations, void* workspace, int64_t workspace_bytes, void* stream);

#define TCVN_OCC_MAX_PASS 256
#define TCVN_OCC_TARGET_EVENT 0
#define TCVN_OCC_TARGET_PRONG 1
int64_t tcvn_occlusion_workspace_bytes(int n_img, int height, int width, int tile_h, int tile_w, int max_pass);
int tcvn_occlusion_variants(const int32_t* coords, int64_t nnz, int n_img, int height, int width, int tile_h, int tile_w,
                            const int32_t* img_bs, int max_pass, int32_t* vimg, int32_t* index, void* workspace,
                            int64_t workspace_bytes, int64_t* host_out, int64_t host_cap, void* stream);
int tcvn_occlusion_build_pass(const int32_t* coords, const float* values, int64_t nnz, int channels, int n_img, int height, int width,
                              int tile_h, int tile_w, int max_pass, const int32_t* vimg, const void* workspace, int64_t workspace_bytes,
                              int first, int count, int32_t* out_coords, float* out_values, int64_t out_rows, void* stream);
int64_t tcvn_head_occlusion_workspace_bytes(const tcvn_head* p, int max_prongs);
int tcvn_head_occlusion(tcvn_head* p, int batch, int max_prongs, int n_prongs, const float* rows, const float* tokens,
                        const int32_t* tok_row, int n, const int32_t* vimg, const int32_t* index, int row_base, const float* emb,
                        int64_t emb_ld, int col0, int width, float* occluded_event_logits, float* occluded_prong_logits,
                        void* workspace, int64_t workspace_bytes, void* stream);
int tcvn_occlusion_heatmap(const float* event_logits, const float* prong_logits, const float* occluded_event_logits,
                           const float* occluded_prong_logits, const int32_t* index, int64_t n_variants, int batch, int max_prongs,
                           int event_classes, int prong_classes, int grid_h, int grid_w, int target, const int32_t* classes,
                           float* heatmap, void* stream);

#define TCVN_OCC_GROUP_EVENT 0
#define TCVN_OCC_GROUP_MAP 1
#define TCVN_OCC_MAX_LEVELS 16
int tcvn_occlusion_select(const float* heat, const int32_t* index, int64_t n_variants, int batch, int max_prongs, int grid_h,
                          int grid_w, int group, float keep, uint32_t* group_max, uint8_t* keep_map, void* stream);
int tcvn_occlusion_refine_variants(const int32_t* coords, int64_t nnz, int n_img, int height, int width, int tile_h, int tile_w,
                                   const int32_t* img_bs, const uint8_t* keep_map, int batch, int max_prongs, int parent_grid_h,
                                   int parent_grid_w, int max_pass, int32_t* vimg, int32_t* index, void* workspace,
                                   int64_t workspace_bytes, int64_t* host_out, int64_t host_cap, void* stream);
int tcvn_occlusion_mark(const int32_t* index, int64_t n_variants, int batch, int max_prongs, int grid_h, int grid_w, uint8_t* evaluated,
                        void* stream);
int tcvn_occlusion_occupancy(const int32_t* coords, int64_t nnz, int n_img, int height, int width, int tile_h, int tile_w,
                             const int32_t* img_bs, int batch, int max_prongs, uint8_t* occupied, void* stream);
int tcvn_occlusion_paint(int levels, const float* const* heat, const uint8_t* const* evaluated, const int32_t* grid_h,
                         const int32_t* grid_w, const uint8_t* occupied, int batch, int max_prongs, float* out, void* stream);

#define TCVN_CURVE_MAX_STEPS 64
#define TCVN_CURVE_MAX_TILES 4096
#define TCVN_CURVE_DELETION 0
#define TCVN_CURVE_INSERTION 1
int64_t tcvn_occlusion_curve_workspace_bytes(int n_img, int height, int width, int tile_h, int tile_w, int steps, int max_pass);
int tcvn_occlusion_curve_variants(const int32_t* coords, int64_t nnz, int n_img, int height, int width, int tile_h, int tile_w,
                                  const int32_t* img_bs, const float* relevance, int batch, int max_prongs, int steps, int mode,
                                  int32_t* rank, int max_pass, int32_t* vimg, int32_t* index, void* workspace,
                                  int64_t workspace_bytes, int64_t* host_out, int64_t host_cap, void* stream);
int tcvn_occlusion_curve_build_pass(const int32_t* coords, const float* values, int64_t nnz, int channels, int n_img, int height,
                                    int width, int tile_h, int tile_w, int steps, int mode, int max_pass, const int32_t* vimg,
                                    const void* workspace, int64_t workspace_bytes, int first, int count, int32_t* out_coords,
                                    float* out_values, int64_t out_rows, void* stream);
int tcvn_occlusion_curve(const float* event_logits, const float* prong_logits, const float* step_event_logits,
                         const float* step_prong_logits, const int32_t* index, int64_t n_variants, int batch, int max_prongs,
                         int event_classes, int prong_classes, int steps, int target, const int32_t* classes, float* curve, float* auc,
                         void* stream);

int tcvn_linear_forward(const float* x, int64_t ldx, const float* weight, const float* bias, float* y, int64_t ldy, int rows,
                        int n_out, int n_in, void* stream);
int tcvn_rows_bn_prelu_forward(const float* x, int64_t ldx, int rows, int channels, const float* gamma, const float* beta,
                               const float* slope, float* running_mean, float* running_var, float* y, int64_t ldy,
                               float* save_mean_rstd, int train, float drop_p, uint64_t seed, uint32_t stream_id, void* stream);

int tcvn_linear_backward(const float* dy, int64_t lddy, const float* x, int64_t ldx, const float* weight, float* dx, int64_t lddx,
                         float* dweight, float* dbias, int rows, int n_out, int n_in, void* stream);
int tcvn_rows_bn_prelu_backward(const float* x, int64_t ldx, const float* dy, int64_t lddy, int rows, int channels, const float* gamma,
                                const float* beta, const float* slope, const float* save_mean_rstd, float* dx, int64_t lddx,
                                float* dgamma, float* dbeta, float* dslope, float drop_p, uint64_t seed, uint32_t stream_id, void* stream);

int tcvn_head_loss(tcvn_head* p, int batch, int max_prongs, const float* event_logits, const float* prong_logits,
                   const int64_t* event_targets, const int8_t* prong_targets, float* losses, float* accs,
                   float* d_event_logits, float* d_prong_logits, void* stream);
int tcvn_head_backward(tcvn_head* p, int batch, int max_prongs, int n_prongs, const float* rows, const int32_t* tok_row,
                       const float* d_event_logits, const float* d_prong_logits, float* d_rows, void* workspace,
                       int64_t workspace_bytes, void* stream);

int tcvn_focal_loss(const float* logits, const int64_t* targets, int rows, int classes, float gamma, float weight,
                    float* d_logits, float* out2, void* stream);

int tcvn_grad_sumsq(const float* x, int64_t n, double* partials, int n_partials, float* out, void* stream);
int tcvn_adamw_step(float* param, const float* grad, float* exp_avg, float* exp_avg_sq, const float* weight_decay, int64_t n,
                    float lr, float beta1, float beta2, float eps, int64_t step, const float* grad_sumsq, float clip, void* stream);

int tcvn_dropout_keep(int kind, float p, uint64_t seed, uint32_t stream_id, int64_t rows, int cols, float* out, void* stream);

void tcvn_backward_overlap(int on);
void tcvn_profile_enable(int on);
void tcvn_profile_filter(const char* label_substring);
void tcvn_profile_reset(void);
int tcvn_profile_count(void);
int tcvn_profile_get(int i, char* name, int name_cap, float* ms, double* flops, double* bytes);

#ifdef __cplusplus
}
#endif
#endif
```

Baseline: 1768 events/s.

## Fuse small linear+BN+PReLU blocks and head loss into single kernels

Adds fused kernels that compute a small-row linear layer together with the following batch-norm/PReLU/dropout in one launch, forward and backward (including weight/bias gradients and chaining the next layer's dx). These replace separate linear and rows-BN launches in the DenseNet output head and the transformer head's combine/decoder layers. The event and prong focal losses are also merged into one kernel. The aim is to cut kernel launch overhead and intermediate round-trips on tiny tensors, at the risk of lower parallelism since each fused kernel runs only a few blocks.

```diff
diff --git a/dune-transformercvn_amd/csrc/densenet.hip b/dune-transformercvn_amd/csrc/densenet.hip
--- a/dune-transformercvn_amd/csrc/densenet.hip
+++ b/dune-transformercvn_amd/csrc/densenet.hip
@@ -617,13 +617,16 @@
     float* F = reinterpret_cast<float*>(s.ws + s.L.F);
     float* Z = reinterpret_cast<float*>(s.ws + s.L.Z);
     int rc;
-    if ((rc = linear_fwd(F, Cf, data[s_wl], nullptr, Z, cfg.out_dim, s.n, cfg.out_dim, Cf, s.st))) return rc;
+    static const bool no_fuse = TCVN_KNOB_SET("TCVN_NO_BLOCK_FUSE");
+    const bool fuse = !no_fuse && block_fused_ok(s.n);
+    if (!fuse && (rc = linear_fwd(F, Cf, data[s_wl], nullptr, Z, cfg.out_dim, s.n, cfg.out_dim, Cf, s.st))) return rc;
     float* hs = reinterpret_cast<float*>(s.ws + s.L.head_stat);
     RowsBnArgs r{};
     r.X = Z; r.ldx = cfg.out_dim; r.R = s.n; r.C = cfg.out_dim; r.gamma = data[nl.w]; r.beta = data[nl.b]; r.slope = data[s_al];
     r.running_mean = data[nl.rm]; r.running_var = data[nl.rv]; r.Y = out; r.ldy = out_ld;
     r.save_mean = hs; r.save_rstd = hs + cfg.out_dim; r.train = s.train; r.eps = kEps; r.momentum = kMom;
     r.drop_p = s.train ? cfg.dropout : 0.f; r.seed = s.seed; r.stream_id = 0x4000u;
+    if (fuse) return fused_block_fwd(BlockFwdArgs{F, Cf, data[s_wl], nullptr, Cf, Z, cfg.out_dim, r}, s.st);
     return rows_bn_fwd(r, s.st);
 }
 
diff --git a/dune-transformercvn_amd/csrc/densenet_bwd.hip b/dune-transformercvn_amd/csrc/densenet_bwd.hip
--- a/dune-transformercvn_amd/csrc/densenet_bwd.hip
+++ b/dune-transformercvn_amd/csrc/densenet_bwd.hip
@@ -179,8 +179,15 @@
     r.gamma = data[nl.w]; r.beta = data[nl.b]; r.slope = data[s_al]; r.save_mean = hs; r.save_rstd = hs + cfg.out_dim;
     r.dX = dZ; r.lddx = cfg.out_dim; r.dgamma = grad[nl.w]; r.dbeta = grad[nl.b]; r.dslope = grad[s_al];
     r.drop_p = cfg.dropout; r.seed = s.seed; r.stream_id = 0x4000u;
-    if ((rc = rows_bn_bwd(r, s.st))) return rc;
-    if ((rc = linear_bwd_dw(dZ, cfg.out_dim, F, Cf, grad[s_wl], nullptr, s.n, cfg.out_dim, Cf, s.st))) return rc;
+    static const bool no_fuse = TCVN_KNOB_SET("TCVN_NO_BLOCK_FUSE");
+    if (!no_fuse && block_fused_ok(s.n)) {
+        BlockBwdArgs g{};
+        g.b = r; g.A = F; g.lda = Cf; g.K = Cf; g.dW = grad[s_wl];
+        if ((rc = fused_block_bwd(g, s.st))) return rc;
+    } else {
+        if ((rc = rows_bn_bwd(r, s.st))) return rc;
+        if ((rc = linear_bwd_dw(dZ, cfg.out_dim, F, Cf, grad[s_wl], nullptr, s.n, cfg.out_dim, Cf, s.st))) return rc;
+    }
     return linear_bwd_dx(dZ, cfg.out_dim, data[s_wl], dF, Cf, s.n, cfg.out_dim, Cf, 0, s.st);
 }
 
diff --git a/dune-transformercvn_amd/csrc/encoder.hip b/dune-transformercvn_amd/csrc/encoder.hip
--- a/dune-transformercvn_amd/csrc/encoder.hip
+++ b/dune-transformercvn_amd/csrc/encoder.hip
@@ -201,12 +201,13 @@
     dX[i] = g * d;
 }
 
+struct FocalSmem { alignas(16) double red[256][2]; int cnt_s[256]; int total; };
 template <typename TT>
-__global__ __launch_bounds__(256) void k_focal(const float* logits, const TT* targets, int rows, int C, float gamma, float weight,
-                                               float* dlogits, float* out) {
-    __shared__ double red[256][2];
-    __shared__ int cnt_s[256];
-    __shared__ int total;
+__device__ __forceinline__ void focal_rows(FocalSmem& sm, const float* logits, const TT* targets, int rows, int C, float gamma, float weight,
+                                           float* dlogits, float* out) {
+    double (&red)[256][2] = sm.red;
+    int (&cnt_s)[256] = sm.cnt_s;
+    int& total = sm.total;
     int cnt = 0;
     for (int r = threadIdx.x; r < rows; r += 256) cnt += targets[r] >= 0;
     cnt_s[threadIdx.x] = cnt;
@@ -248,6 +249,24 @@
         out[0] = (float)(l * invn); out[1] = (float)(c * invn);
     }
 }
+template <typename TT>
+__global__ __launch_bounds__(256) void k_focal(const float* logits, const TT* targets, int rows, int C, float gamma, float weight,
+                                               float* dlogits, float* out) {
+    __shared__ FocalSmem sm;
+    focal_rows(sm, logits, targets, rows, C, gamma, weight, dlogits, out);
+}
+__global__ __launch_bounds__(256) void k_head_loss(const HeadLossArgs a) {
+    __shared__ FocalSmem sm;
+    focal_rows(sm, a.ev_logits, a.ev_targets, a.B, a.Ce, a.gamma, a.ew, a.dEv, a.lb);
+    __syncthreads();
+    focal_rows(sm, a.pr_logits, a.pr_targets, a.B * a.P, a.Cp, a.gamma, 1.f - a.ew, a.dPr, a.lb + 2);
+    if (threadIdx.x == 0) {
+        const float oe = a.lb[0], op = a.lb[2];
+        a.losses[0] = a.ew * oe + (1.f - a.ew) * op;
+        a.losses[1] = oe; a.losses[2] = op;
+        a.accs[0] = a.lb[1]; a.accs[1] = a.lb[3];
+    }
+}
 
 __global__ void k_permute_rows(const float* in, float* out, int B, int P, int C, int to_bm) {
     const int i = blockIdx.x * blockDim.x + threadIdx.x;
@@ -341,6 +360,10 @@
     hipLaunchKernelGGL(k_focal<int64_t>, dim3(1), dim3(256), 0, st, logits, targets, rows, C, gamma, weight, dlogits, out);
     TCVN_LAUNCH_CHECK(); return 0;
 }
+int head_loss(const HeadLossArgs& a, hipStream_t st) {
+    hipLaunchKernelGGL(k_head_loss, dim3(1), dim3(256), 0, st, a);
+    TCVN_LAUNCH_CHECK(); return 0;
+}
 int focal_i8(const float* logits, const int8_t* targets, int rows, int C, float gamma, float weight, float* dlogits, float* out,
              hipStream_t st) {
     hipLaunchKernelGGL(k_focal<int8_t>, dim3(1), dim3(256), 0, st, logits, targets, rows, C, gamma, weight, dlogits, out);
diff --git a/dune-transformercvn_amd/csrc/head.hip b/dune-transformercvn_amd/csrc/head.hip
--- a/dune-transformercvn_amd/csrc/head.hip
+++ b/dune-transformercvn_amd/csrc/head.hip
@@ -128,6 +128,8 @@
     L.dLG = b.take((long)TP * cfg.prong_classes * 4);
     L.t0 = b.take(3 * td); L.t1 = b.take(3 * td); L.t2 = b.take(td); L.t3 = b.take(td); L.dHID = b.take(td);
     L.dC = b.take((long)R * D * 4); L.dZc = b.take((long)R * D * 4);
+    L.dZd.clear();
+    for (const auto& d : dec) L.dZd.push_back(b.take((long)TP * d.out * 4));
     for (int l = 0; l < cfg.n_layers; ++l) {
         HLayBuf& q = L.lay[l];
         q.g_dqkv = b.take(3 * td); q.g_dao = b.take(td); q.g_dhp = b.take(td); q.g_df = b.take(td);
@@ -180,6 +182,15 @@
     r.drop_p = d.drop ? s.dp : 0.f; r.seed = s.seed; r.stream_id = d.sid;
     return r;
 }
+int HeadPlan::linear_block_fwd(const HDec& d, const HeadStep& s, const float* A, long lda, long Z, long Y, long stat, int rows) const {
+    const float* bias = d.b >= 0 ? data[d.b] : nullptr;
+    if (blocks_fused(rows)) {
+        BlockFwdArgs f{A, lda, data[d.w], bias, d.in, s.F(Z), d.out, block_fwd(d, s, Z, Y, stat, rows)};
+        return fused_block_fwd(f, s.st);
+    }
+    if (int rc = linear_fwd(A, lda, data[d.w], bias, s.F(Z), d.out, rows, d.out, d.in, s.st)) return rc;
+    return rows_bn_fwd(block_fwd(d, s, Z, Y, stat, rows), s.st);
+}
 DecIn HeadPlan::dec_in(const HeadStep& s, int i) const {
     const long hid_prongs = (long)s.B * cfg.hidden_dim;
     if (i == 0) return DecIn{s.F(s.L.HID) + hid_prongs, s.F(s.L.dHID) + hid_prongs, cfg.hidden_dim};
@@ -189,8 +200,7 @@
 int HeadPlan::embed(const HeadStep& s, const float* rows, const int32_t* tok_row) const {
     const HLayout& L = s.L;
     const int D = cfg.hidden_dim;
-    if (int rc = linear_fwd(rows, cfg.in_dim, data[comb.w], comb.b >= 0 ? data[comb.b] : nullptr, s.F(L.Zc), D, s.R, D, cfg.in_dim, s.st)) return rc;
-    if (int rc = rows_bn_fwd(block_fwd(comb, s, L.Zc, L.C, L.cstat, s.R), s.st)) return rc;
+    if (int rc = linear_block_fwd(comb, s, rows, cfg.in_dim, L.Zc, L.C, L.cstat, s.R)) return rc;
     return gather_tokens(s.F(L.C), tok_row, s.F(L.X[0]), s.B, s.S, D, s.st);
 }
 
@@ -262,8 +272,7 @@
     for (int i = 0; i < n_dec; ++i) {
         const HDec& d = dec[i];
         const DecIn in = dec_in(s, i);
-        if (int rc = linear_fwd(in.x, in.w, data[d.w], data[d.b], s.F(L.Zd[i]), d.out, TP, d.out, d.in, s.st)) return rc;
-        if (int rc = rows_bn_fwd(block_fwd(d, s, L.Zd[i], L.Ad[i], L.dstat[i], TP), s.st)) return rc;
+        if (int rc = linear_block_fwd(d, s, in.x, in.w, L.Zd[i], L.Ad[i], L.dstat[i], TP)) return rc;
     }
     const DecIn in = dec_in(s, n_dec);
     if (int rc = linear_fwd(in.x, in.w, data[ow], data[ob], s.F(L.LG), cfg.prong_classes, TP, cfg.prong_classes, cfg.dec_out_in, s.st)) return rc;
@@ -284,6 +293,11 @@
 int HeadPlan::loss(int B, int P, const float* ev_logits, const float* pr_logits, const int64_t* et, const int8_t* pt, float* losses,
                    float* accs, float* dEv, float* dPr, hipStream_t st) {
     float* lb = accs + 2;
+    if (fused_blocks) {
+        HeadLossArgs a{ev_logits, et, pr_logits, pt, B, P, cfg.event_classes, cfg.prong_classes, cfg.gamma, cfg.event_weight,
+                       dEv, dPr, lb, losses, accs};
+        return head_loss(a, st);
+    }
     if (int rc = focal_i64(ev_logits, et, B, cfg.event_classes, cfg.gamma, cfg.event_weight, dEv, lb, st)) return rc;
     if (int rc = focal_i8(pr_logits, pt, B * P, cfg.prong_classes, cfg.gamma, 1.f - cfg.event_weight, dPr, lb + 2, st)) return rc;
     hipLaunchKernelGGL(k_combine_loss, dim3(1), dim3(1), 0, st, lb, lb + 2, cfg.event_weight, losses, accs);
@@ -315,6 +329,32 @@
     const int D = cfg.hidden_dim, TP = s.TP, Ce = cfg.event_classes, Cp = cfg.prong_classes, n_dec = (int)dec.size();
     if (int rc = permute_rows(dPr, s.F(L.dLG), s.B, s.P, Cp, 0, s.st)) return rc;
     const DecIn last = dec_in(s, n_dec);
+    if (blocks_fused(TP) && blocks_fused(s.B)) {
+        BlockBwdArgs o{};
+        o.linear_only = 1; o.b.dY = s.F(L.dLG); o.b.lddy = Cp; o.b.R = TP; o.b.C = Cp;
+        o.A = last.x; o.lda = last.w; o.K = last.w; o.dW = grad[ow]; o.db = grad[ob];
+        if (n_dec == 0) { o.W = data[ow]; o.dA = last.dx; o.ldda = last.w; }
+        if (int rc = fused_block_bwd(o, s.st)) return rc;
+        for (int i = n_dec - 1; i >= 0; --i) {
+            const HDec& d = dec[i];
+            const DecIn in = dec_in(s, i);
+            BlockBwdArgs g{};
+            g.b = block_bwd(d, s, L.Zd[i], L.t0, L.dstat[i], L.dZd[i], TP);
+            g.dYf = s.F(L.t0);
+            if (i == n_dec - 1) { g.dZn = s.F(L.dLG); g.lddzn = Cp; g.Wn = data[ow]; g.Nn = Cp; }
+            else { g.dZn = s.F(L.dZd[i + 1]); g.lddzn = dec[i + 1].out; g.Wn = data[dec[i + 1].w]; g.Nn = dec[i + 1].out; }
+            g.A = in.x; g.lda = in.w; g.K = d.in; g.dW = grad[d.w]; g.db = grad[d.b];
+            if (int rc = fused_block_bwd(g, s.st)) return rc;
+        }
+        if (n_dec > 0) {
+            const DecIn in = dec_in(s, 0);
+            if (int rc = linear_bwd_dx(s.F(L.dZd[0]), dec[0].out, data[dec[0].w], in.dx, in.w, TP, dec[0].out, dec[0].in, 0, s.st)) return rc;
+        }
+        BlockBwdArgs e{};
+        e.linear_only = 1; e.b.dY = dEv; e.b.lddy = Ce; e.b.R = s.B; e.b.C = Ce;
+        e.A = s.F(L.HID); e.lda = D; e.K = D; e.dW = grad[ew]; e.db = grad[eb]; e.W = data[ew]; e.dA = s.F(L.dHID); e.ldda = D;
+        return fused_block_bwd(e, s.st);
+    }
     if (int rc = linear_bwd_dw(s.F(L.dLG), Cp, last.x, last.w, grad[ow], grad[ob], TP, Cp, last.w, s.st)) return rc;
     if (int rc = linear_bwd_dx(s.F(L.dLG), Cp, data[ow], last.dx, last.w, TP, Cp, last.w, 0, s.st)) return rc;
     float* dZ = s.F(L.t1);
@@ -416,6 +456,13 @@
     const HLayout& L = s.L;
     const int D = cfg.hidden_dim;
     if (int rc = scatter_tokens_bwd(dX0, tok_row, s.F(L.dC), s.B, s.S, D, s.st)) return rc;
+    if (blocks_fused(s.R)) {
+        BlockBwdArgs g{};
+        g.b = block_bwd(comb, s, L.Zc, L.dC, L.cstat, L.dZc, s.R);
+        g.A = rows; g.lda = cfg.in_dim; g.K = cfg.in_dim; g.dW = grad[comb.w]; g.db = comb.b >= 0 ? grad[comb.b] : nullptr;
+        if (int rc = fused_block_bwd(g, s.st)) return rc;
+        return linear_bwd_dx(s.F(L.dZc), D, data[comb.w], d_rows, cfg.in_dim, s.R, D, cfg.in_dim, 0, s.st);
+    }
     if (int rc = rows_bn_bwd(block_bwd(comb, s, L.Zc, L.dC, L.cstat, L.dZc, s.R), s.st)) return rc;
     if (int rc = linear_bwd_dw(s.F(L.dZc), D, rows, cfg.in_dim, grad[comb.w], comb.b >= 0 ? grad[comb.b] : nullptr, s.R, D, cfg.in_dim, s.st)) return rc;
     return linear_bwd_dx(s.F(L.dZc), D, data[comb.w], d_rows, cfg.in_dim, s.R, D, cfg.in_dim, 0, s.st);
@@ -507,6 +554,7 @@
 }
 int tcvn_head_bind(tcvn_head* p, void* const* data, void* const* grad) { return p->plan.bind(data, grad); }
 void tcvn_head_set_fused_encoder(tcvn_head* p, int on) { p->plan.fused_encoder = on != 0; }
+void tcvn_head_set_fused_blocks(tcvn_head* p, int on) { p->plan.fused_blocks = on != 0; }
 int64_t tcvn_head_workspace_bytes(const tcvn_head* p, int batch, int max_prongs, int n_prongs) {
     HLayout L;
     p->plan.layout(batch, max_prongs, n_prongs, L);
@@ -797,6 +845,67 @@
     return rows_bn_bwd(r, reinterpret_cast<hipStream_t>(stream));
 }
 
+extern "C" int tcvn_linear_block_forward(const float* x, int64_t ldx, const float* weight, const float* bias, int rows, int n_out, int n_in,
+                                         const float* gamma, const float* beta, const float* slope, float* running_mean,
+                                         float* running_var, float* z, int64_t ldz, float* y, int64_t ldy, float* save_mean_rstd,
+                                         int train, float drop_p, uint64_t seed, uint32_t stream_id, void* stream) {
+    if (!x || !weight || !z || rows <= 0 || n_out <= 0 || n_in <= 0) return -1;
+    if (!block_fused_ok(rows)) {
+        if (int rc = tcvn_linear_forward(x, ldx, weight, bias, z, ldz, rows, n_out, n_in, stream)) return rc;
+        return tcvn_rows_bn_prelu_forward(z, ldz, rows, n_out, gamma, beta, slope, running_mean, running_var, y, ldy, save_mean_rstd,
+                                          train, drop_p, seed, stream_id, stream);
+    }
+    const bool no_norm = !gamma && !beta && !running_mean && !running_var;
+    if (!y || (!no_norm && (!gamma || !beta || !running_mean || !running_var || !save_mean_rstd))) return -1;
+    BlockFwdArgs f{};
+    f.A = x; f.lda = ldx; f.W = weight; f.bias = bias; f.K = n_in; f.Z = z; f.ldz = ldz;
+    RowsBnArgs& r = f.n;
+    r.no_norm = no_norm ? 1 : 0;
+    r.X = z; r.ldx = ldz; r.R = rows; r.C = n_out; r.gamma = gamma; r.beta = beta; r.slope = slope;
+    r.running_mean = running_mean; r.running_var = running_var; r.Y = y; r.ldy = ldy;
+    r.save_mean = save_mean_rstd; r.save_rstd = save_mean_rstd ? save_mean_rstd + n_out : nullptr; r.train = train; r.eps = kEps; r.momentum = kMom;
+    r.drop_p = train ? drop_p : 0.f; r.seed = seed; r.stream_id = stream_id;
+    return fused_block_fwd(f, reinterpret_cast<hipStream_t>(stream));
+}
+extern "C" int tcvn_linear_block_backward(const float* x, int64_t ldx, const float* weight, const float* z, int64_t ldz, float* dy,
+                                          int64_t lddy, const float* dz_next, int64_t lddz_next, const float* weight_next, int n_next,
+                                          int rows, int n_out, int n_in, const float* gamma, const float* beta, const float* slope,
+                                          const float* save_mean_rstd, float* dz, int64_t lddz, float* dx, int64_t lddx, float* dweight,
+                                          float* dbias, float* dgamma, float* dbeta, float* dslope, float drop_p, uint64_t seed,
+                                          uint32_t stream_id, void* stream) {
+    const bool no_norm = !gamma && !beta && !dgamma && !dbeta;
+    if (!x || !weight || !z || !dy || !dz || rows <= 0 || n_out <= 0 || n_in <= 0 || (slope != nullptr) != (dslope != nullptr)) return -1;
+    if (!no_norm && (!gamma || !beta || !save_mean_rstd || !dgamma || !dbeta)) return -1;
+    if (dz_next && (!weight_next || n_next <= 0)) return -1;
+    hipStream_t st = reinterpret_cast<hipStream_t>(stream);
+    if (!block_fused_ok(rows)) {
+        if (dz_next)
+            if (int rc = linear_bwd_dx(dz_next, lddz_next, weight_next, dy, lddy, rows, n_next, n_out, 0, st)) return rc;
+        if (int rc = tcvn_rows_bn_prelu_backward(z, ldz, dy, lddy, rows, n_out, gamma, beta, slope, save_mean_rstd, dz, lddz, dgamma, dbeta,
+                                                 dslope, drop_p, seed, stream_id, stream)) return rc;
+        return tcvn_linear_backward(dz, lddz, x, ldx, weight, dx, lddx, dweight, dbias, rows, n_out, n_in, stream);
+    }
+    BlockBwdArgs g{};
+    g.dZn = dz_next; g.lddzn = lddz_next; g.Wn = weight_next; g.Nn = n_next; g.dYf = dy;
+    RowsBnBwdArgs& r = g.b;
+    r.no_norm = no_norm ? 1 : 0;
+    r.X = z; r.ldx = ldz; r.dY = dy; r.lddy = lddy; r.R = rows; r.C = n_out; r.gamma = gamma; r.beta = beta; r.slope = slope;
+    r.save_mean = save_mean_rstd; r.save_rstd = save_mean_rstd ? save_mean_rstd + n_out : nullptr; r.dX = dz; r.lddx = lddz;
+    r.dgamma = dgamma; r.dbeta = dbeta; r.dslope = dslope; r.drop_p = drop_p; r.seed = seed; r.stream_id = stream_id;
+    g.A = x; g.lda = ldx; g.K = n_in; g.dW = dweight; g.db = dweight ? dbias : nullptr;
+    if (int rc = fused_block_bwd(g, st)) return rc;
+    return dx ? linear_bwd_dx(dz, lddz, weight, dx, lddx, rows, n_out, n_in, 0, st) : 0;
+}
+extern "C" int tcvn_linear_backward_fused(const float* dy, int64_t lddy, const float* x, int64_t ldx, const float* weight, float* dx,
+                                          int64_t lddx, float* dweight, float* dbias, int rows, int n_out, int n_in, void* stream) {
+    if (!dy || !x || !weight || rows <= 0 || n_out <= 0 || n_in <= 0) return -1;
+    if (!block_fused_ok(rows)) return tcvn_linear_backward(dy, lddy, x, ldx, weight, dx, lddx, dweight, dbias, rows, n_out, n_in, stream);
+    BlockBwdArgs g{};
+    g.linear_only = 1; g.b.dY = dy; g.b.lddy = lddy; g.b.R = rows; g.b.C = n_out;
+    g.A = x; g.lda = ldx; g.K = n_in; g.dW = dweight; g.db = dweight ? dbias : nullptr; g.W = weight; g.dA = dx; g.ldda = lddx;
+    return fused_block_bwd(g, reinterpret_cast<hipStream_t>(stream));
+}
+
 extern "C" int tcvn_focal_loss(const float* logits, const int64_t* targets, int rows, int classes, float gamma, float weight,
                                float* d_logits, float* out2, void* stream) {
     return focal_i64(logits, targets, rows, classes, gamma, weight, d_logits, out2, reinterpret_cast<hipStream_t>(stream));
diff --git a/dune-transformercvn_amd/csrc/head_plan.h b/dune-transformercvn_amd/csrc/head_plan.h
--- a/dune-transformercvn_amd/csrc/head_plan.h
+++ b/dune-transformercvn_amd/csrc/head_plan.h
@@ -16,7 +16,7 @@
                  h1, h2; };
 struct HLayout {
     long Zc, C, cstat, HID, LG, dEv, dPr, lossbuf, dLG, t0, t1, t2, t3, dHID, dC, dZc, lnp, total;
-    std::vector<long> X, Zd, Ad, dstat;
+    std::vector<long> X, Zd, Ad, dstat, dZd;
     std::vector<HLayBuf> lay;
 };
 
@@ -39,6 +39,7 @@
     std::vector<HDec> dec;
     bool bound = false;
     bool fused_encoder = true;
+    bool fused_blocks = true;
     uint64_t last_seed = 0;
 
     explicit HeadPlan(const tcvn_head_cfg& c);
@@ -52,6 +53,8 @@
     RowsBnArgs block_fwd(const HDec& d, const HeadStep& s, long X, long Y, long stat, int rows) const;
     RowsBnBwdArgs block_bwd(const HDec& d, const HeadStep& s, long X, long dY, long stat, long dX, int rows) const;
     DecIn dec_in(const HeadStep& s, int i) const;
+    bool blocks_fused(int rows) const { return fused_blocks && block_fused_ok(rows); }
+    int linear_block_fwd(const HDec& d, const HeadStep& s, const float* A, long lda, long Z, long Y, long stat, int rows) const;
     int embed(const HeadStep& s, const float* rows, const int32_t* tok_row) const;
     int encode(const HeadStep& s, const int32_t* tok_row) const, encode_post(const HeadStep& s, const int32_t* tok_row) const,
         encode_pre(const HeadStep& s, const int32_t* tok_row) const;
diff --git a/dune-transformercvn_amd/csrc/rows.hip b/dune-transformercvn_amd/csrc/rows.hip
--- a/dune-transformercvn_amd/csrc/rows.hip
+++ b/dune-transformercvn_amd/csrc/rows.hip
@@ -171,6 +171,240 @@
     }
 }
 
+constexpr int BT_RB = 64, BT_KP = 128;
+struct BlockTile { float As[BT_RB][BT_KP + 1], Bs[BLOCK_CT][BT_KP + 1]; };
+
+template <bool A_ALONG_ROWS, class Store>
+__device__ __forceinline__ void block_tile_gemm(BlockTile& sm, const float* __restrict__ A, long sai, long sak, const float* __restrict__ B,
+                                                long sbj, long sbk, int M, int N, int K, int j0, Store store) {
+    static_assert(BLOCK_CT == 4 && BT_RB * BLOCK_CT == 256, "thread maps below");
+    const int tid = threadIdx.x, tx = tid & 3, ty = tid >> 2;
+    const int npan = (K + BT_KP - 1) / BT_KP, nit = npan * ((M + BT_RB - 1) / BT_RB);
+    constexpr int NA = BT_RB * BT_KP / 256, NB = BLOCK_CT * BT_KP / 256;
+    const int a_r = A_ALONG_ROWS ? (tid & 63) : (tid >> 7), a_k = A_ALONG_ROWS ? (tid >> 6) : (tid & 127);
+    constexpr int a_dr = A_ALONG_ROWS ? 0 : 2, a_dk = A_ALONG_ROWS ? 4 : 0;
+    float va[NA], vb[NB];
+    auto load = [&](int it) {
+        const int i0 = (it / npan) * BT_RB, k0 = (it % npan) * BT_KP;
+#pragma unroll
+        for (int q = 0; q < NA; ++q) {
+            const int i = i0 + a_r + a_dr * q, k = k0 + a_k + a_dk * q;
+            va[q] = (i < M && k < K) ? A[(long)i * sai + (long)k * sak] : 0.f;
+        }
+#pragma unroll
+        for (int q = 0; q < NB; ++q) {
+            const int e = tid + 256 * q, j = j0 + (e >> 7), k = k0 + (e & 127);
+            vb[q] = (j < N && k < K) ? B[(long)j * sbj + (long)k * sbk] : 0.f;
+        }
+    };
+    load(0);
+    float acc = 0.f;
+    for (int it = 0; it < nit; ++it) {
+#pragma unroll
+        for (int q = 0; q < NA; ++q) sm.As[a_r + a_dr * q][a_k + a_dk * q] = va[q];
+#pragma unroll
+        for (int q = 0; q < NB; ++q) { const int e = tid + 256 * q; sm.Bs[e >> 7][e & 127] = vb[q]; }
+        __syncthreads();
+        if (it + 1 < nit) load(it + 1);
+        const int p = it % npan, k0 = p * BT_KP;
+        const int kn = K - k0 < BT_KP ? K - k0 : BT_KP;
+        if (p == 0) acc = 0.f;
+        if (kn == BT_KP) {
+#pragma unroll 16
+            for (int k = 0; k < BT_KP; ++k) acc = fmaf(sm.As[ty][k], sm.Bs[tx][k], acc);
+        } else {
+            for (int k = 0; k < kn; ++k) acc = fmaf(sm.As[ty][k], sm.Bs[tx][k], acc);
+        }
+        if (p == npan - 1) {
+            const int i = (it / npan) * BT_RB + ty, j = j0 + tx;
+            if (i < M && j < N) store(i, j, acc);
+        }
+        __syncthreads();
+    }
+}
+
+__global__ __launch_bounds__(256) void k_block_fwd(const BlockFwdArgs f) {
+    __shared__ BlockTile sm;
+    __shared__ double red[16][BLOCK_CT][2];
+    __shared__ float s_mean[BLOCK_CT], s_rstd[BLOCK_CT];
+    const RowsBnArgs& a = f.n;
+    const int c0 = blockIdx.x * BLOCK_CT;
+    {
+        const float* bias = f.bias; float* Z = f.Z; const long ldz = f.ldz;
+        block_tile_gemm<false>(sm, f.A, f.lda, 1, f.W, (long)f.K, 1, a.R, a.C, f.K, c0,
+                               [=](int i, int j, float acc) { Z[(long)i * ldz + j] = acc + (bias ? bias[j] : 0.f); });
+    }
+    const int cl = threadIdx.x & (BLOCK_CT - 1), rg = threadIdx.x >> 2;
+    const int c = c0 + cl;
+    const bool ok = c < a.C, stat = threadIdx.x < 16 * BLOCK_CT;
+    if (!a.no_norm) {
+        if (a.train) {
+            if (stat) {
+                double s1 = 0, s2 = 0;
+                if (ok)
+                    for (int r = rg; r < a.R; r += 16) { const double v = a.X[(long)r * a.ldx + c]; s1 += v; s2 += v * v; }
+                red[rg][cl][0] = s1; red[rg][cl][1] = s2;
+            }
+            __syncthreads();
+            if (stat && rg == 0 && ok) {
+                double x = 0, y = 0;
+                for (int g = 0; g < 16; ++g) { x += red[g][cl][0]; y += red[g][cl][1]; }
+                const double mean = x / a.R;
+                double var = y / a.R - mean * mean;
+                if (var < 0) var = 0;
+                s_mean[cl] = (float)mean;
+                s_rstd[cl] = (float)(1.0 / sqrt(var + (double)a.eps));
+                if (a.save_mean) { a.save_mean[c] = s_mean[cl]; a.save_rstd[c] = s_rstd[cl]; }
+                if (a.running_mean) {
+                    const double unb = a.R > 1 ? var * a.R / (double)(a.R - 1) : var;
+                    a.running_mean[c] = (1.f - a.momentum) * a.running_mean[c] + a.momentum * (float)mean;
+                    a.running_var[c] = (1.f - a.momentum) * a.running_var[c] + a.momentum * (float)unb;
+                }
+            }
+        } else if (stat && rg == 0 && ok) {
+            s_mean[cl] = a.running_mean[c];
+            s_rstd[cl] = 1.0f / sqrtf(a.running_var[c] + a.eps);
+        }
+        __syncthreads();
+    }
+    if (!ok) return;
+    const float mean = a.no_norm ? 0.f : s_mean[cl], rstd = a.no_norm ? 1.f : s_rstd[cl];
+    const float g = a.gamma ? a.gamma[c] : 1.f, b = a.beta ? a.beta[c] : 0.f;
+    const float sl = a.slope ? a.slope[c] : 0.f;
+    for (int r = threadIdx.x >> 2; r < a.R; r += 256 / BLOCK_CT) {
+        const float x = a.X[(long)r * a.ldx + c];
+        float z;
+        if (a.no_norm) z = prelu(x, sl);
+        else {
+            const float u = (x - mean) * rstd * g + b;
+            z = prelu(u, sl);
+        }
+        if (a.train && a.drop_p > 0.f) z *= drop_scale(a.drop_p, a.seed, a.stream_id, (uint64_t)r * a.C + c);
+        a.Y[(long)r * a.ldy + c] = z;
+    }
+}
+
+__global__ __launch_bounds__(256) void k_block_bwd(const BlockBwdArgs f, int tiles) {
+    __shared__ BlockTile sm;
+    __shared__ double red[16][BLOCK_CT][3];
+    __shared__ float s_db[BLOCK_CT], s_dg[BLOCK_CT];
+    const RowsBnBwdArgs& a = f.b;
+    if ((int)blockIdx.x >= tiles) {
+        float* dA = f.dA; const long ldda = f.ldda;
+        block_tile_gemm<false>(sm, a.dY, a.lddy, 1, f.W, 1, (long)f.K, a.R, f.K, a.C, ((int)blockIdx.x - tiles) * BLOCK_CT,
+                               [=](int i, int j, float acc) { dA[(long)i * ldda + j] = acc + 0.f; });
+        return;
+    }
+    const int c0 = blockIdx.x * BLOCK_CT;
+    const float* dY = a.dY;
+    if (f.dZn) {
+        float* o = f.dYf; const long ldo = a.lddy;
+        block_tile_gemm<false>(sm, f.dZn, f.lddzn, 1, f.Wn, 1, (long)a.C, a.R, a.C, f.Nn, c0,
+                               [=](int i, int j, float acc) { o[(long)i * ldo + j] = acc + 0.f; });
+        dY = f.dYf;
+    }
+    const int cl = threadIdx.x & (BLOCK_CT - 1), rg = threadIdx.x >> 2;
+    const int c = c0 + cl;
+    const bool ok = c < a.C, stat = threadIdx.x < 16 * BLOCK_CT;
+    const float* dZ = dY; long lddz = a.lddy;
+    if (!f.linear_only) {
+        dZ = a.dX; lddz = a.lddx;
+        const float sl = (ok && a.slope) ? a.slope[c] : 0.f;
+        if (a.no_norm) {
+            if (stat) {
+                double s3 = 0;
+                if (ok)
+                    for (int r = rg; r < a.R; r += 16) {
+                        const float u = a.X[(long)r * a.ldx + c];
+                        float dz = dY[(long)r * a.lddy + c];
+                        if (a.drop_p > 0.f) dz *= drop_scale(a.drop_p, a.seed, a.stream_id, (uint64_t)r * a.C + c);
+                        a.dX[(long)r * a.lddx + c] = u > 0.f ? dz : sl * dz;
+                        s3 += u > 0.f ? 0.f : dz * u;
+                    }
+                red[rg][cl][0] = s3;
+            }
+            __syncthreads();
+            if (stat && rg == 0 && ok && a.dslope) {
+                double z = 0;
+                for (int q = 0; q < 16; ++q) z += red[q][cl][0];
+                a.dslope[c] += (float)z;
+            }
+        } else {
+            const float mean = ok ? a.save_mean[c] : 0.f, rstd = ok ? a.save_rstd[c] : 0.f;
+            const float g = (ok && a.gamma) ? a.gamma[c] : 1.f, b = (ok && a.beta) ? a.beta[c] : 0.f;
+            if (stat) {
+                double s1 = 0, s2 = 0, s3 = 0;
+                if (ok)
+                    for (int r = rg; r < a.R; r += 16) {
+                        const float xh = (a.X[(long)r * a.ldx + c] - mean) * rstd;
+                        const float u = xh * g + b;
+                        float dz = dY[(long)r * a.lddy + c];
+                        if (a.drop_p > 0.f) dz *= drop_scale(a.drop_p, a.seed, a.stream_id, (uint64_t)r * a.C + c);
+                        const float du = u > 0.f ? dz : sl * dz;
+                        s1 += du; s2 += (double)du * xh; s3 += u > 0.f ? 0.f : dz * u;
+                    }
+                red[rg][cl][0] = s1; red[rg][cl][1] = s2; red[rg][cl][2] = s3;
+            }
+            __syncthreads();
+            if (stat && rg == 0 && ok) {
+                double x = 0, y = 0, z = 0;
+                for (int q = 0; q < 16; ++q) { x += red[q][cl][0]; y += red[q][cl][1]; z += red[q][cl][2]; }
+                s_db[cl] = (float)x; s_dg[cl] = (float)y;
+                if (a.dbeta) a.dbeta[c] += (float)x;
+                if (a.dgamma) a.dgamma[c] += (float)y;
+                if (a.dslope) a.dslope[c] += (float)z;
+            }
+            __syncthreads();
+            if (ok) {
+                const float db = s_db[cl] / a.R, dg = s_dg[cl] / a.R;
+                for (int r = threadIdx.x >> 2; r < a.R; r += 256 / BLOCK_CT) {
+                    const float xh = (a.X[(long)r * a.ldx + c] - mean) * rstd;
+                    const float u = xh * g + b;
+                    float dz = dY[(long)r * a.lddy + c];
+                    if (a.drop_p > 0.f) dz *= drop_scale(a.drop_p, a.seed, a.stream_id, (uint64_t)r * a.C + c);
+                    const float du = u > 0.f ? dz : sl * dz;
+                    a.dX[(long)r * a.lddx + c] = g * rstd * (du - db - xh * dg);
+                }
+            }
+        }
+        __syncthreads();
+    }
+    if (f.db) {
+        if (stat) {
+            double s = 0;
+            if (ok)
+                for (int r = rg; r < a.R; r += 16) s += dZ[(long)r * lddz + c];
+            red[rg][cl][0] = s;
+        }
+        __syncthreads();
+        if (stat && rg == 0 && ok) {
+            double x = 0;
+            for (int q = 0; q < 16; ++q) x += red[q][cl][0];
+            f.db[c] += (float)x;
+        }
+    }
+    if (f.dW) {
+        float* dW = f.dW; const int K = f.K;
+        block_tile_gemm<true>(sm, f.A, 1, f.lda, dZ, 1, lddz, f.K, a.C, a.R, c0,
+                              [=](int k, int n, float acc) { float* w = dW + (long)n * K + k; *w = *w + (acc + 0.f); });
+    }
+}
+
+}
+
+int fused_block_fwd(const BlockFwdArgs& a, hipStream_t st) {
+    if (a.n.R <= 0) return 0;
+    if (a.n.X != a.Z || a.n.ldx != a.ldz) return -1;
+    hipLaunchKernelGGL(k_block_fwd, dim3(cdiv(a.n.C, BLOCK_CT)), dim3(256), 0, st, a);
+    TCVN_LAUNCH_CHECK();
+    return 0;
+}
+int fused_block_bwd(const BlockBwdArgs& a, hipStream_t st) {
+    if (a.b.R <= 0) return 0;
+    const int tiles = cdiv(a.b.C, BLOCK_CT), dx_tiles = (a.linear_only && a.dA) ? cdiv(a.K, BLOCK_CT) : 0;
+    hipLaunchKernelGGL(k_block_bwd, dim3(tiles + dx_tiles), dim3(256), 0, st, a, tiles);
+    TCVN_LAUNCH_CHECK();
+    return 0;
 }
 
 int linear_bwd_dw(const float* dY, long lddy, const float* X, long ldx, float* dW, float* db, int R, int N, int K, hipStream_t st) {
diff --git a/dune-transformercvn_amd/csrc/tcvn_encoder.h b/dune-transformercvn_amd/csrc/tcvn_encoder.h
--- a/dune-transformercvn_amd/csrc/tcvn_encoder.h
+++ b/dune-transformercvn_amd/csrc/tcvn_encoder.h
@@ -64,5 +64,11 @@
               hipStream_t st);
 int focal_i8(const float* logits, const int8_t* targets, int rows, int C, float gamma, float weight, float* dlogits, float* out,
              hipStream_t st);
+struct HeadLossArgs {
+    const float* ev_logits; const int64_t* ev_targets; const float* pr_logits; const int8_t* pr_targets;
+    int B, P, Ce, Cp; float gamma, ew;
+    float *dEv, *dPr, *lb, *losses, *accs;
+};
+int head_loss(const HeadLossArgs& a, hipStream_t st);
 
 }
diff --git a/dune-transformercvn_amd/csrc/tcvn_rows.h b/dune-transformercvn_amd/csrc/tcvn_rows.h
--- a/dune-transformercvn_amd/csrc/tcvn_rows.h
+++ b/dune-transformercvn_amd/csrc/tcvn_rows.h
@@ -47,4 +47,22 @@
 };
 int rows_bn_bwd(const RowsBnBwdArgs& a, hipStream_t st);
 
+constexpr int BLOCK_CT = 4, BLOCK_MAX_ROWS = 1024;
+static inline bool block_fused_ok(int rows) { return rows <= BLOCK_MAX_ROWS; }
+
+struct BlockFwdArgs {
+    const float* A; long lda; const float* W; const float* bias; int K;
+    float* Z; long ldz;
+    RowsBnArgs n;
+};
+int fused_block_fwd(const BlockFwdArgs& a, hipStream_t st);
+
+struct BlockBwdArgs {
+    const float* dZn; long lddzn; const float* Wn; int Nn; float* dYf;
+    RowsBnBwdArgs b; int linear_only;
+    const float* A; long lda; int K; float* dW; float* db;
+    const float* W; float* dA; long ldda;
+};
+int fused_block_bwd(const BlockBwdArgs& a, hipStream_t st);
+
 }
diff --git a/dune-transformercvn_amd/transformercvn/hip/_lib.py b/dune-transformercvn_amd/transformercvn/hip/_lib.py
--- a/dune-transformercvn_amd/transformercvn/hip/_lib.py
+++ b/dune-transformercvn_amd/transformercvn/hip/_lib.py
@@ -123,6 +123,11 @@
     sig("tcvn_rows_bn_prelu_forward", i32, vp, i64, i32, i32, vp, vp, vp, vp, vp, vp, i64, vp, i32, f32, u64, C.c_uint32, vp)
     sig("tcvn_linear_backward", i32, vp, i64, vp, i64, vp, vp, i64, vp, vp, i32, i32, i32, vp)
     sig("tcvn_rows_bn_prelu_backward", i32, vp, i64, vp, i64, i32, i32, vp, vp, vp, vp, vp, i64, vp, vp, vp, f32, u64, C.c_uint32, vp)
+    sig("tcvn_linear_block_forward", i32, vp, i64, vp, vp, i32, i32, i32, vp, vp, vp, vp, vp, vp, i64, vp, i64, vp, i32, f32, u64, C.c_uint32, vp)
+    sig("tcvn_linear_block_backward", i32, vp, i64, vp, vp, i64, vp, i64, vp, i64, vp, i32, i32, i32, i32, vp, vp, vp, vp, vp, i64, vp, i64,
+        vp, vp, vp, vp, vp, f32, u64, C.c_uint32, vp)
+    sig("tcvn_linear_backward_fused", i32, vp, i64, vp, i64, vp, vp, i64, vp, vp, i32, i32, i32, vp)
+    sig("tcvn_head_set_fused_blocks", None, vp, i32)
     sig("tcvn_focal_loss", i32, vp, vp, i32, i32, f32, f32, vp, vp, vp)
     sig("tcvn_grad_sumsq", i32, vp, i64, vp, i32, vp, vp)
     sig("tcvn_adamw_step", i32, vp, vp, vp, vp, vp, i64, f32, f32, f32, f32, i64, vp, f32, vp)
@@ -161,6 +166,7 @@
     "tcvn_occlusion_select", "tcvn_occlusion_refine_variants", "tcvn_occlusion_mark", "tcvn_occlusion_occupancy", "tcvn_occlusion_paint",
     "tcvn_occlusion_curve_workspace_bytes", "tcvn_occlusion_curve_variants", "tcvn_occlusion_curve_build_pass", "tcvn_occlusion_curve",
     "tcvn_head_shapley_workspace_bytes", "tcvn_head_shapley_count", "tcvn_head_shapley",
+    "tcvn_head_set_fused_blocks", "tcvn_linear_block_forward", "tcvn_linear_block_backward", "tcvn_linear_backward_fused",
 ]
 
 lib = _load()
diff --git a/include/tcvn_hip.h b/include/tcvn_hip.h
--- a/include/tcvn_hip.h
+++ b/include/tcvn_hip.h
@@ -100,6 +100,7 @@
 int tcvn_head_bind(tcvn_head* p, void* const* data, void* const* grad);
 int64_t tcvn_head_workspace_bytes(const tcvn_head* p, int batch, int max_prongs, int n_prongs);
 void tcvn_head_set_fused_encoder(tcvn_head* p, int on);
+void tcvn_head_set_fused_blocks(tcvn_head* p, int on);
 
 int tcvn_head_forward(tcvn_head* p, int batch, int max_prongs, int n_prongs, const float* rows, const int32_t* tok_row,
                       float* event_logits, float* prong_logits, void* workspace, int64_t workspace_bytes, int train,
@@ -199,6 +200,18 @@
                                 const float* beta, const float* slope, const float* save_mean_rstd, float* dx, int64_t lddx,
                                 float* dgamma, float* dbeta, float* dslope, float drop_p, uint64_t seed, uint32_t stream_id, void* stream);
 
+int tcvn_linear_block_forward(const float* x, int64_t ldx, const float* weight, const float* bias, int rows, int n_out, int n_in,
+                              const float* gamma, const float* beta, const float* slope, float* running_mean, float* running_var,
+                              float* z, int64_t ldz, float* y, int64_t ldy, float* save_mean_rstd, int train, float drop_p,
+                              uint64_t seed, uint32_t stream_id, void* stream);
+int tcvn_linear_block_backward(const float* x, int64_t ldx, const float* weight, const float* z, int64_t ldz, float* dy, int64_t lddy,
+                               const float* dz_next, int64_t lddz_next, const float* weight_next, int n_next, int rows, int n_out,
+                               int n_in, const float* gamma, const float* beta, const float* slope, const float* save_mean_rstd,
+                               float* dz, int64_t lddz, float* dx, int64_t lddx, float* dweight, float* dbias, float* dgamma,
+                               float* dbeta, float* dslope, float drop_p, uint64_t seed, uint32_t stream_id, void* stream);
+int tcvn_linear_backward_fused(const float* dy, int64_t lddy, const float* x, int64_t ldx, const float* weight, float* dx, int64_t lddx,
+                               float* dweight, float* dbias, int rows, int n_out, int n_in, void* stream);
+
 int tcvn_head_loss(tcvn_head* p, int batch, int max_prongs, const float* event_logits, const float* prong_logits,
                    const int64_t* event_targets, const int8_t* prong_targets, float* losses, float* accs,
                    float* d_event_logits, float* d_prong_logits, void* stream);
```

Result: slower. 1745 events/s (-1.3%).
